# chsakell/aca-dotnet-workshop

Measured on AMD Instinct MI355X. Metric: tasks_e2e_per_sec, higher is better.
Workload: dtype n/a (JSON over HTTP)

## Files before the change

aca_dotnet_workshop_amd/native/build.py:

```python
from __future__ import annotations

import contextlib
import fcntl
import os
import subprocess
import sys
import sysconfig
from pathlib import Path

HERE = Path(__file__).resolve().parent
SRC = HERE / "src"


def ext_path(name: str) -> Path:
    suffix = sysconfig.get_config_var("EXT_SUFFIX") or ".so"
    return HERE / f"{name}{suffix}"


@contextlib.contextmanager
def build_lock(name: str):
    lock_dir = HERE / "bin"
    lock_dir.mkdir(exist_ok=True)
    with open(lock_dir / f".{name}.lock", "w") as fh:
        fcntl.flock(fh, fcntl.LOCK_EX)
        try:
            yield
        finally:
            fcntl.flock(fh, fcntl.LOCK_UN)


def _stale(target: Path, sources: list[Path]) -> bool:
    if not target.exists():
        return True
    t = target.stat().st_mtime
    return any(s.exists() and s.stat().st_mtime > t for s in sources)


def _newest(sources: list[Path]) -> float:
    return max((s.stat().st_mtime for s in sources if s.exists()), default=0.0)


def _install(tmp: Path, target: Path, stamp: float) -> None:
    os.replace(tmp, target)
    if stamp > 0:
        os.utime(target, (stamp, stamp))


def _run_compiler(cmd: list[str], tmp: Path) -> None:
    try:
        subprocess.run(cmd, check=True)
    except BaseException:
        tmp.unlink(missing_ok=True)
        raise


EXE_ONLY_HEADERS: set[str] = set()


def build_native(force: bool = False, verbose: bool = False) -> Path:
    target = ext_path("_ttnative")
    sources = sorted(h for h in SRC.glob("*.hpp") if h.name not in EXE_ONLY_HEADERS) + [SRC / "module.cpp"]
    if not force and not _stale(target, sources):
        return target
    with build_lock("ttnative"):
        if force or _stale(target, sources):
            _compile_native(target, verbose, _newest(sources))
    return target


def _compile_native(target: Path, verbose: bool, stamp: float = 0.0) -> None:
    import pybind11
    cxx = os.environ.get("CXX", "g++")
    tmp = target.with_suffix(f".tmp{os.getpid()}.so")
    cmd = [cxx, "-O3", "-std=c++17", "-shared", "-fPIC", "-Wall", "-Wno-unused-function", "-Wno-attributes",
           f"-I{pybind11.get_include()}", f"-I{sysconfig.get_paths()['include']}", str(SRC / "module.cpp"),
           "-o", str(tmp), "-lpthread", "-lssl", "-lcrypto"]
    if verbose:
        print(" ".join(cmd), file=sys.stderr)
    _run_compiler(cmd, tmp)
    _install(tmp, target, stamp)


DATAPLANE = HERE / "bin" / "ttsidecar-dataplane"


def build_dataplane(force: bool = False, verbose: bool = False) -> Path:
    sources = [SRC / "dataplane.cpp", SRC / "evhttp.hpp", SRC / "h2.hpp", SRC / "pb.hpp", SRC / "tls.hpp", SRC / "json.hpp", SRC / "httpparse.hpp",
               SRC / "textutil.hpp", SRC / "pcsample.hpp"]
    return _build_exe(DATAPLANE, SRC / "dataplane.cpp", sources, force, verbose)


def _build_exe(target: Path, main: Path, sources: list[Path], force: bool, verbose: bool,
               threads: bool = False) -> Path:
    if not force and not _stale(target, sources):
        return target
    with build_lock(target.name):
        if not force and not _stale(target, sources):
            return target
        cxx = os.environ.get("CXX", "g++")
        tmp = target.with_name(f".{target.name}.tmp{os.getpid()}")
        cmd = [cxx, "-O2", "-std=c++17", "-Wall", "-Wno-unused-function", "-rdynamic", str(main), "-o", str(tmp),
               "-lssl", "-lcrypto"] + (["-pthread"] if threads else [])
        if verbose:
            print(" ".join(cmd), file=sys.stderr)
        stamp = _newest(sources)
        _run_compiler(cmd, tmp)
        _install(tmp, target, stamp)
    return target


INGRESS = HERE / "bin" / "ttingress"


def build_ingress(force: bool = False, verbose: bool = False) -> Path:
    sources = [SRC / "ingress.cpp", SRC / "evhttp.hpp", SRC / "tls.hpp", SRC / "json.hpp", SRC / "httpparse.hpp",
               SRC / "textutil.hpp", SRC / "pcsample.hpp"]
    return _build_exe(INGRESS, SRC / "ingress.cpp", sources, force, verbose, threads=True)


LOADGEN = HERE / "bin" / "ttloadgen"


def build_loadgen(force: bool = False, verbose: bool = False) -> Path:
    sources = [SRC / "loadgen.cpp", SRC / "evhttp.hpp", SRC / "tls.hpp", SRC / "json.hpp", SRC / "httpparse.hpp"]
    return _build_exe(LOADGEN, SRC / "loadgen.cpp", sources, force, verbose, threads=True)


if __name__ == "__main__":
    print(build_native(force="--force" in sys.argv, verbose=True))
    print(build_dataplane(force="--force" in sys.argv, verbose=True))
    print(build_loadgen(force="--force" in sys.argv, verbose=True))
    print(build_ingress(force="--force" in sys.argv, verbose=True))
```

aca_dotnet_workshop_amd/native/src/dataplane.cpp:

```cpp
#include <signal.h>
#include <sys/prctl.h>
#include <sys/signalfd.h>
#include <sys/stat.h>
#include <dirent.h>

#include <cstdio>
#include <ctime>
#include <fstream>
#include <map>
#include <random>
#include <sstream>

#include "evhttp.hpp"
#include "daprpb.hpp"
#include "h2.hpp"
#include "json.hpp"
#include "pb.hpp"
#include "pcsample.hpp"
#include "textutil.hpp"

using namespace tt;
using ev::ClientResult;
using ev::Endpoint;
using ev::HeaderList;
using ev::Message;
using ev::Reply;
using namespace tt::text;

namespace {

std::mt19937_64& rng() {
  static std::mt19937_64 r{std::random_device{}() ^ ((uint64_t)getpid() << 32)};
  return r;
}

std::string hex_u64(uint64_t v, int digits = 16) {
  static const char* d = "0123456789abcdef";
  std::string s((size_t)digits, '0');
  for (int i = digits - 1; i >= 0; --i, v >>= 4) s[(size_t)i] = d[v & 15];
  return s;
}

std::string uuid4() {
  uint64_t a = rng()(), b = rng()();
  a = (a & 0xFFFFFFFFFFFF0FFFull) | 0x0000000000004000ull;
  b = (b & 0x3FFFFFFFFFFFFFFFull) | 0x8000000000000000ull;
  std::string h = hex_u64(a) + hex_u64(b);
  return h.substr(0, 8) + "-" + h.substr(8, 4) + "-" + h.substr(12, 4) + "-" + h.substr(16, 4) + "-" + h.substr(20);
}

std::string utc_now_iso() {
  timespec ts;
  clock_gettime(CLOCK_REALTIME, &ts);
  tm t;
  gmtime_r(&ts.tv_sec, &t);
  char buf[64];
  std::snprintf(buf, sizeof buf, "%04d-%02d-%02dT%02d:%02d:%02d.%06ldZ", t.tm_year + 1900, t.tm_mon + 1, t.tm_mday,
                t.tm_hour, t.tm_min, t.tm_sec, ts.tv_nsec / 1000);
  return buf;
}

double wall_now() {
  timespec ts;
  clock_gettime(CLOCK_REALTIME, &ts);
  return (double)ts.tv_sec + ts.tv_nsec / 1e9;
}

std::string error_json(std::string_view code, std::string_view msg) {
  return "{\"errorCode\":" + json_str(code) + ",\"message\":" + json_str(msg) + "}";
}


bool valid_json(std::string_view s) { return tt::valid(s); }

bool top_level_string(std::string_view json, std::string_view key, std::string& out) {
  const char* p = tt::ws_end(json.data(), json.data() + json.size());
  const char* e = json.data() + json.size();
  if (p >= e || *p != '{') return false;
  p = tt::ws_end(p + 1, e);
  while (p < e && *p == '"') {
    const char* k = p + 1;
    const char* q = tt::skip_value(p, e);
    std::string_view name(k, (size_t)(q - 1 - k));
    p = tt::ws_end(q, e);
    if (p >= e || *p != ':') return false;
    p = tt::ws_end(p + 1, e);
    const char* v = p;
    p = tt::skip_value(p, e);
    if (name.find('\\') != std::string_view::npos) {
      try {
        Value obj = parse(json);
        const Value* x = obj.get(key);
        if (!x || x->t != Value::String) return false;
        out = x->s;
        return true;
      } catch (const std::exception&) {
        return false;
      }
    }
    if (name == key) {
      if (*v != '"') return false;
      std::string_view lit(v + 1, (size_t)(p - 1 - (v + 1)));
      if (lit.find('\\') != std::string_view::npos) {
        try {
          out = parse(std::string_view(v, (size_t)(p - v))).s;
        } catch (const std::exception&) {
          return false;
        }
      } else {
        out.assign(lit);
      }
      return true;
    }
    p = tt::ws_end(p, e);
    if (p < e && *p == ',') p = tt::ws_end(p + 1, e);
  }
  return false;
}

std::string errno_text(int e) {
  switch (e) {
    case ETIMEDOUT: return "timeout";
    case ECONNREFUSED: return "connection refused";
    case ENOENT: return "no such socket";
    case ECONNRESET: return "connection closed";
    case EPROTO: return "malformed upstream response";
    default: return std::string(strerror(e));
  }
}

const std::string* opt_str(const Value& cfg, const char* k) {
  auto* v = cfg.get(k);
  return v && v->t == Value::String ? &v->s : nullptr;
}

void hex16(uint64_t v, char* out) {
  static const char* d = "0123456789abcdef";
  for (int i = 15; i >= 0; --i, v >>= 4) out[i] = d[v & 15];
}

struct SpanCtx {
  char trace_id[32], span_id[16], parent_id[16];
  bool has_parent = false, sampled = false;
  double start_wall = 0, t0 = 0;
  std::string_view tid() const { return {trace_id, 32}; }
  std::string_view sid() const { return {span_id, 16}; }
  std::string_view pid() const { return {parent_id, 16}; }
  std::string traceparent() const {
    std::string s;
    s.reserve(55);
    s.append("00-", 3).append(trace_id, 32).append(1, '-').append(span_id, 16).append(sampled ? "-01" : "-00", 3);
    return s;
  }
};

bool parse_traceparent(const std::string* v, SpanCtx& out) {
  if (!v) return false;
  std::string_view s(*v);
  if (s.size() < 55 || s[2] != '-' || s[35] != '-' || s[52] != '-') return false;
  bool tz = true, pz = true;
  for (size_t i = 3; i < 35; ++i) {
    if (hexv(s[i]) < 0) return false;
    tz = tz && s[i] == '0';
  }
  for (size_t i = 36; i < 52; ++i) {
    if (hexv(s[i]) < 0) return false;
    pz = pz && s[i] == '0';
  }
  if (tz || pz) return false;
  int f1 = hexv(s[53]), f2 = hexv(s[54]);
  if (f1 < 0 || f2 < 0) return false;
  std::memcpy(out.trace_id, s.data() + 3, 32);
  std::memcpy(out.parent_id, s.data() + 36, 16);
  out.has_parent = true;
  out.sampled = ((f1 * 16 + f2) & 1) != 0;
  return true;
}

class Tracer {
 public:
  void init(const Value& cfg) {
    if (auto* d = opt_str(cfg, "dir")) dir_ = *d;
    if (auto* r = cfg.get("sampleRate"); r && r->t == Value::Number) rate_ = r->n;
    if (auto* r = opt_str(cfg, "role")) role_ = *r;
    if (auto* i = opt_str(cfg, "instance")) instance_ = *i;
    if (auto* f = opt_str(cfg, "file")) path_ = *f;
    if (auto* fe = cfg.get("flushEach"); fe && fe->t == Value::Bool) flush_each_ = fe->b;
    if (!dir_.empty() && path_.empty()) {
      mkdir(dir_.c_str(), 0755);
      std::string safe = role_;
      for (auto& c : safe)
        if (c == '/') c = '_';
      stem_ = dir_ + "/spans-" + safe + "-" + std::to_string(getpid()) + "-";
      path_ = stem_;
    }
  }
  SpanCtx start(const std::string* traceparent) {
    SpanCtx s;
    if (!parse_traceparent(traceparent, s)) {
      hex16(rng()(), s.trace_id);
      hex16(rng()(), s.trace_id + 16);
      s.has_parent = false;
      s.sampled = rate_ >= 1.0 || std::uniform_real_distribution<double>(0, 1)(rng()) < rate_;
    }
    hex16(rng()(), s.span_id);
    if (s.sampled) s.start_wall = wall_now();
    s.t0 = ev::now_s();
    return s;
  }
  void end(const SpanCtx& s, const std::string& name, int status, const std::vector<std::pair<std::string, std::string>>& attrs) {
    if (!s.sampled || path_.empty()) return;
    char dur[32];
    std::snprintf(dur, sizeof dur, "%.3f", (ev::now_s() - s.t0) * 1000.0);
    char ts[32];
    std::snprintf(ts, sizeof ts, "%.6f", s.start_wall);
    std::string l = "{\"type\":\"span\",\"role\":" + json_str(role_) + ",\"instance\":" + json_str(instance_) +
                    ",\"name\":" + json_str(name) + ",\"kind\":\"server\",\"traceId\":\"" + std::string(s.tid()) +
                    "\",\"spanId\":\"" + std::string(s.sid()) + "\",\"parentId\":" +
                    (s.has_parent ? "\"" + std::string(s.pid()) + "\"" : std::string("null")) + ",\"ts\":" + ts +
                    ",\"durationMs\":" + dur + ",\"status\":\"" + (status >= 500 ? "error" : "ok") +
                    "\",\"attributes\":{\"http.status\":" + std::to_string(status);
    for (auto& a : attrs) l += "," + json_str(a.first) + ":" + json_str(a.second);
    l += "},\"plane\":\"native\"}\n";
    buf_ += l;
    if (flush_each_ || buf_.size() > 64 * 1024) flush();
  }
  void flush() {
    if (buf_.empty() || path_.empty()) return;
    std::string path = path_;
    if (!stem_.empty()) {
      time_t t = time(nullptr);
      struct tm g;
      gmtime_r(&t, &g);
      char day[16];
      std::strftime(day, sizeof day, "%Y%m%d", &g);
      path = stem_ + day + ".jsonl";
    }
    if (FILE* f = std::fopen(path.c_str(), "a")) {
      std::fwrite(buf_.data(), 1, buf_.size(), f);
      std::fclose(f);
    }
    buf_.clear();
  }

 private:
  std::string dir_, path_, stem_, role_ = "sidecar", instance_;
  double rate_ = 1.0;
  bool flush_each_ = false;
  std::string buf_;
};

class Resolver {
 public:
  std::string dir;
  std::vector<std::string> candidates(const std::string& app) {
    auto& e = cache_[app];
    double t = ev::now_s();
    if (t - e.at > 0.5) {
      e.eps.clear();
      e.at = t;
      std::string d = dir + "/" + app;
      if (DIR* dh = opendir(d.c_str())) {
        std::vector<std::string> files;
        while (dirent* de = readdir(dh)) {
          std::string n = de->d_name;
          if (n.size() > 5 && n[0] != '.' && n.compare(n.size() - 5, 5, ".json") == 0) files.push_back(n);
        }
        closedir(dh);
        std::sort(files.begin(), files.end());
        for (auto& f : files) {
          std::ifstream in(d + "/" + f);
          std::stringstream ss;
          ss << in.rdbuf();
          try {
            Value rec = parse(ss.str());
            auto* ep = rec.get("endpoint");
            auto* pid = rec.get("pid");
            if (!ep || ep->t != Value::String) continue;
            if (pid && pid->t == Value::Number && kill((pid_t)pid->n, 0) != 0 && errno == ESRCH) continue;
            e.eps.push_back(ep->s);
          } catch (const std::exception&) {
          }
        }
      }
    }
    if (e.eps.size() <= 1) return e.eps;
    size_t n = e.rr++ % e.eps.size();
    std::vector<std::string> out(e.eps.begin() + (long)n, e.eps.end());
    out.insert(out.end(), e.eps.begin(), e.eps.begin() + (long)n);
    return out;
  }
  void invalidate(const std::string& app) { cache_.erase(app); }

 private:
  struct Entry {
    double at = -1;
    std::vector<std::string> eps;
    size_t rr = 0;
  };
  std::map<std::string, Entry> cache_;
};

inline uint64_t fnv1a64(std::string_view s) {
  uint64_t h = 14695981039346656037ull;
  for (unsigned char c : s) {
    h ^= c;
    h *= 1099511628211ull;
  }
  return h;
}
struct Store {
  Endpoint backing;
  std::vector<Endpoint> shards;
  std::string coll_path;
  std::string prefix;
  HeaderList auth;
  size_t shard_of(std::string_view full_key) const { return shards.empty() ? 0 : fnv1a64(full_key) % shards.size(); }
  const Endpoint& ep(size_t shard) const { return shards.empty() ? backing : shards[shard]; }
};
struct Bus {
  Endpoint backing;
  std::vector<Endpoint> shards;
  std::string ns;
  HeaderList auth;
  const Endpoint& ep(std::string_view partition_key) const {
    return shards.empty() ? backing : shards[fnv1a64(partition_key) % shards.size()];
  }
};
inline std::vector<Endpoint> shard_list(const Value& s) {
  std::vector<Endpoint> out;
  if (auto* sh = s.get("shards"); sh && sh->t == Value::Array)
    for (auto& u : sh->items)
      if (u.t == Value::String) out.push_back(Endpoint::parse(u.s));
  if (out.size() == 1) out.clear();
  return out;
}

bool is_invoke_hop(const std::string& k) {
  return ev::is_hop_header(k) || k == "dapr-api-token" || k == "dapr-app-id" || k == "traceparent";
}

class DataPlane {
 public:
  DataPlane(ev::Loop& loop, const Value& cfg) : loop_(loop), client_(loop) {
    app_id_ = *opt_str(cfg, "appId");
    if (auto* a = opt_str(cfg, "app")) {
      app_ = Endpoint::parse(*a);
      has_app_ = true;
    }
    if (auto* t = opt_str(cfg, "appToken")) app_token_ = *t;
    if (auto* t = opt_str(cfg, "apiToken")) api_token_ = *t;
    if (auto* t = opt_str(cfg, "meshToken")) mesh_token_ = *t;
    if (auto* t = cfg.get("mtls"); t && t->t == Value::Object) {
      ev::TlsConfig tc;
      tc.cert = *opt_str(*t, "cert");
      tc.key = *opt_str(*t, "key");
      tc.ca = *opt_str(*t, "ca");
      mesh_server_tls = std::make_shared<ev::TlsContext>(tc, true);
      client_.set_tls(std::make_shared<ev::TlsContext>(tc, false));
    }
    if (auto* r = opt_str(cfg, "registryDir")) resolver_.dir = *r;
    fallback_ = Endpoint::parse(*opt_str(cfg, "fallback"));
    if (auto* v = cfg.get("invokeNative"); v && v->t == Value::Bool) invoke_native_ = v->b;
    if (auto* v = cfg.get("appTimeout"); v && v->t == Value::Number) app_timeout_ = v->n;
    if (auto* v = cfg.get("apiLogging"); v && v->t == Value::Bool) api_logging_ = v->b;
    if (auto* tr = cfg.get("trace")) tracer_.init(*tr);
    if (auto* st = cfg.get("stores"); st && st->t == Value::Object)
      for (size_t i = 0; i < st->keys.size(); ++i) {
        const Value& s = st->items[i];
        Store x;
        x.backing = Endpoint::parse(*opt_str(s, "backing"));
        x.coll_path = "/cosmos/" + quote_all(*opt_str(s, "account")) + "/" + quote_all(*opt_str(s, "db")) + "/" +
                      quote_all(*opt_str(s, "coll"));
        x.prefix = *opt_str(s, "prefix");
        x.auth = auth_headers(s);
        x.shards = shard_list(s);
        stores_[st->keys[i]] = std::move(x);
      }
    if (auto* ps = cfg.get("pubsubs"); ps && ps->t == Value::Object)
      for (size_t i = 0; i < ps->keys.size(); ++i) {
        const Value& s = ps->items[i];
        Bus b;
        b.backing = Endpoint::parse(*opt_str(s, "backing"));
        b.ns = *opt_str(s, "ns");
        b.auth = auth_headers(s);
        b.shards = shard_list(s);
        buses_[ps->keys[i]] = std::move(b);
      }
  }

  ev::Handler api_handler() {
    return [this](Message&& m, Reply r) { on_api(std::move(m), std::move(r)); };
  }
  ev::Handler internal_handler() {
    return [this](Message&& m, Reply r) { on_internal(std::move(m), std::move(r)); };
  }
  ev::Handler control_handler() {
    return [this](Message&& m, Reply r) { on_control(std::move(m), std::move(r)); };
  }
  void flush() {
    flush_api_log();
    tracer_.flush();
  }
  size_t inflight() const { return inflight_; }
  void tick(double now) {
    flush_api_log();
    for (auto& c : consumers_) c->tick(now);
  }
  void begin_stop() {
    for (auto& c : consumers_) c->stop();
  }
  bool drained() const {
    if (inflight_) return false;
    for (auto& c : consumers_)
      if (!c->drained()) return false;
    return true;
  }

 private:
  ev::Loop& loop_;
  ev::Client client_;
  Tracer tracer_;
  Resolver resolver_;
  std::string app_id_, app_token_, api_token_, mesh_token_;

 public:
  std::shared_ptr<ev::TlsContext> mesh_server_tls;
  const std::string& app_id() const { return app_id_; }

 private:
  Endpoint app_, fallback_;
  bool has_app_ = false, invoke_native_ = true, api_logging_ = false;
  double app_timeout_ = 300;
  std::map<std::string, Store> stores_;
  std::map<std::string, Bus> buses_;
  std::map<std::string, uint64_t> counters_;
  std::map<std::pair<std::string, int>, uint64_t> op_counts_;
  size_t inflight_ = 0;

  static HeaderList auth_headers(const Value& s) {
    HeaderList h;
    if (auto* i = opt_str(s, "identity"); i && !i->empty()) h.emplace_back("x-tt-identity", *i);
    if (auto* k = opt_str(s, "key"); k && !k->empty()) h.emplace_back("x-tt-key", *k);
    return h;
  }

  void api_log(const std::string& name, int status, const SpanCtx& span) {
    char buf[96];
    std::snprintf(buf, sizeof buf, " status=%d duration_ms=%.3f app_id=", status, (ev::now_s() - span.t0) * 1e3);
    auto sp = name.find(' ');
    std::string& msg = api_log_msg_;
    msg.assign("HTTP API Called method=");
    msg.append(name, 0, sp);
    msg += " path=";
    if (sp != std::string::npos) msg.append(name, sp + 1, std::string::npos);
    msg += buf;
    msg += app_id_;
    if (api_log_role_.empty()) api_log_role_ = json_str(app_id_ + ".sidecar");
    char ts[32];
    std::snprintf(ts, sizeof ts, "%.6f", wall_now());
    std::string& b = api_log_buf_;
    b += "{\"ts\":";
    b += ts;
    b += ",\"level\":\"INFO\",\"role\":";
    b += api_log_role_;
    b += ",\"category\":\"sidecar.http-info\",\"message\":";
    escape_to(b, msg);
    b += ",\"traceId\":\"";
    b += span.tid();
    b += "\",\"spanId\":\"";
    b += span.sid();
    b += "\",\"plane\":\"native\"}\n";
    if (b.size() >= 32768) flush_api_log();
  }
  std::string api_log_msg_, api_log_role_;
  void flush_api_log() {
    if (api_log_buf_.empty()) return;
    std::fwrite(api_log_buf_.data(), 1, api_log_buf_.size(), stderr);
    api_log_buf_.clear();
  }
  std::string api_log_buf_;

  void count(const std::string& op, int status) {
    op_counts_[{op, status}]++;
  }

  struct Done {
    DataPlane* dp;
    Reply rep;
    SpanCtx span;
    std::string name, op;
    std::vector<std::pair<std::string, std::string>> attrs;
    void send(int status, const HeaderList& h, std::string_view body) {
      rep.send(status, h, body);
      if (dp->api_logging_) dp->api_log(name, status, span);
      dp->tracer_.end(span, name, status, attrs);
      dp->count(op, status);
      dp->inflight_--;
    }
    void json(int status, std::string_view body) { send(status, {{"content-type", "application/json"}}, body); }
    void error(int status, std::string_view code, std::string_view msg) { json(status, error_json(code, msg)); }
  };
  std::shared_ptr<Done> begin(const Message& m, Reply&& r, std::string op, std::string_view path) {
    inflight_++;
    auto d = std::make_shared<Done>();
    d->dp = this;
    d->rep = std::move(r);
    d->span = tracer_.start(m.header("traceparent"));
    d->name = m.method + " " + std::string(path.substr(0, 80));
    d->op = std::move(op);
    return d;
  }

  static void split_target(const std::string& target, std::string& path, std::string& qs) {
    auto q = target.find('?');
    path = target.substr(0, q);
    qs = q == std::string::npos ? "" : target.substr(q + 1);
  }

  struct SubSpec {
    std::string name, pubsub, topic, route, entity, ns, dlt;
    Endpoint backing;
    HeaderList auth;
    int lock_ms = 60000, prefetch = 64, max_conc = 32, retry_delay_ms = 0;
    bool raw = false;
  };
  class Consumer {
   public:
    Consumer(DataPlane& dp, SubSpec s) : s_(std::move(s)), dp_(dp) { next_renew_ = ev::now_s() + renew_period(); }
    SubSpec s_;
    uint64_t delivered = 0, succeeded = 0, retried = 0, dropped = 0, errors = 0;

    void start() { pump(); }
    void stop() {
      stopping_ = true;
      while (!queued_.empty()) {
        abandon_.emplace_back(queued_.front().token, 0);
        locked_.erase(queued_.front().token);
        queued_.pop_front();
      }
      schedule_flush();
    }
    bool drained() const { return running_ == 0 && !settling_ && pending_empty(); }
    void tick(double now) {
      if (!stopping_ && !receiving_ && retry_at_ > 0 && now >= retry_at_) {
        retry_at_ = 0;
        pump();
      }
      if (now >= next_renew_) {
        next_renew_ = now + renew_period();
        if (!locked_.empty() && !stopping_) renew();
      }
    }
    std::string stats_json() const {
      return "{\"delivered\":" + std::to_string(delivered) + ",\"succeeded\":" + std::to_string(succeeded) +
             ",\"retried\":" + std::to_string(retried) + ",\"dropped\":" + std::to_string(dropped) +
             ",\"errors\":" + std::to_string(errors) + ",\"plane\":\"native\"}";
    }

   private:
    struct Msg {
      std::string token, id, body, ctype;
      long long delivery_count = 0;
    };
    DataPlane& dp_;
    std::deque<Msg> queued_;
    std::map<std::string, int> locked_;
    int running_ = 0;
    bool receiving_ = false, stopping_ = false, settling_ = false, flush_scheduled_ = false;
    double retry_at_ = 0, backoff_ = 0.1, next_renew_ = 0;
    std::vector<std::string> complete_;
    std::vector<std::pair<std::string, int>> abandon_;
    std::vector<std::pair<std::string, std::string>> deadletter_;

    double renew_period() const { return std::max(s_.lock_ms / 3000.0, 0.05); }
    bool pending_empty() const { return complete_.empty() && abandon_.empty() && deadletter_.empty(); }
    std::string sb_path(const std::string& tail) const { return "/servicebus/" + quote_all(s_.ns) + tail; }

    void pump() {
      if (stopping_ || receiving_) return;
      int room = s_.prefetch - (int)locked_.size();
      if (room <= 0) return;
      receiving_ = true;
      std::string q = "?entity=" + quote_all(s_.entity) + "&max=" + std::to_string(std::min(room, 256)) +
                      "&lockMs=" + std::to_string(s_.lock_ms) + "&waitMs=2000";
      dp_.client_.request(s_.backing, "POST", sb_path("/receive" + q), s_.auth, {}, 32.0,
                          [this](ClientResult&& res) { on_received(std::move(res)); });
    }

    void on_received(ClientResult&& res) {
      receiving_ = false;
      if (res.err || res.resp.status != 200) {
        if (!stopping_) {
          std::fprintf(stderr, "dataplane: %s: receive failed (%s); retrying in %.1fs\n", s_.name.c_str(),
                       res.err ? errno_text(res.err).c_str() : ("HTTP " + std::to_string(res.resp.status)).c_str(),
                       backoff_);
          retry_at_ = ev::now_s() + backoff_;
          backoff_ = std::min(backoff_ * 2, 5.0);
        }
        return;
      }
      backoff_ = 0.1;
      try {
        Value arr = parse(res.resp.body);
        for (auto& v : arr.items) {
          Msg m;
          if (auto* t = v.get("lockToken")) m.token = t->s;
          if (auto* t = v.get("id")) m.id = t->s;
          if (auto* t = v.get("contentType"); t && t->t == Value::String) m.ctype = t->s;
          if (auto* t = v.get("deliveryCount"); t && t->t == Value::Number) m.delivery_count = (long long)t->n;
          if (auto* b = v.get("bodyB64"); b && b->t == Value::String) m.body = unbase64(b->s);
          else if (auto* b = v.get("body"); b && b->t == Value::String) m.body = b->s;
          if (stopping_) {
            abandon_.emplace_back(m.token, 0);
            continue;
          }
          locked_[m.token] = 1;
          queued_.push_back(std::move(m));
        }
      } catch (const std::exception& e) {
        std::fprintf(stderr, "dataplane: %s: bad receive payload: %s\n", s_.name.c_str(), e.what());
      }
      start_deliveries();
      if (stopping_) schedule_flush();
      pump();
    }

    void start_deliveries() {
      while (!queued_.empty() && running_ < s_.max_conc) {
        Msg m = std::move(queued_.front());
        queued_.pop_front();
        running_++;
        delivered++;
        deliver(std::move(m));
      }
    }

    void deliver(Msg&& m) {
      std::string body = std::move(m.body);
      std::string ctype = m.ctype.empty() ? "application/json" : m.ctype;
      SpanCtx span;
      bool is_ce = false;
      std::string parent_tp;
      if (ctype.rfind("application/cloudevents", 0) == 0 && valid_json(body)) {
        is_ce = true;
        top_level_string(body, "traceparent", parent_tp);
      }
      if (!is_ce && !s_.raw) {
        std::string base = lower(ctype.substr(0, ctype.find(';')));
        std::string ce = "{\"specversion\":\"1.0\",\"id\":" + json_str(m.id.empty() ? uuid4() : m.id) +
                         ",\"source\":\"unknown\",\"type\":\"com.dapr.event.sent\",\"datacontenttype\":" +
                         json_str(base.empty() ? "application/json" : base) + ",\"topic\":" + json_str(s_.topic) +
                         ",\"pubsubname\":" + json_str(s_.pubsub) + ",\"time\":\"" + utc_now_iso() + "\"";
        if (base.find("json") != std::string::npos && !body.empty() && valid_json(body)) ce += ",\"data\":" + compact(body);
        else if (base.find("json") != std::string::npos && body.empty()) ce += ",\"data\":null";
        else if (base.rfind("text/", 0) == 0 || base.find("json") != std::string::npos || body.empty())
          ce += ",\"data\":" + json_str(body);
        else ce += ",\"data_base64\":\"" + base64(body) + "\"";
        ce += "}";
        body = std::move(ce);
        is_ce = true;
      }
      span = dp_.tracer_.start(parent_tp.empty() ? nullptr : &parent_tp);
      HeaderList h;
      h.emplace_back("content-type", is_ce && !s_.raw ? "application/cloudevents+json" : ctype);
      h.emplace_back("traceparent", span.traceparent());
      h.emplace_back("pubsubname", s_.pubsub);
      h.emplace_back("topic", s_.topic);
      std::string token = m.token;
      long long dc = m.delivery_count;
      std::string raw_body = body;
      std::string out_ct = h[0].second;
      dp_.call_app("POST", "/" + s_.route, std::move(h), std::move(body),
                   [this, token, span, dc, raw_body = std::move(raw_body), out_ct](ClientResult&& res) mutable {
                     int outcome = 1;
                     int status = res.err ? 0 : res.resp.status;
                     if (res.err) {
                       errors++;
                     } else if (status >= 200 && status < 300) {
                       outcome = 0;
                       auto* ct = res.resp.header("content-type");
                       if (!res.resp.body.empty() && ct && ct->find("json") != std::string::npos) {
                         try {
                           Value v = parse(res.resp.body);
                           if (auto* st = v.get("status"); st && st->t == Value::String) {
                             std::string u = st->s;
                             for (auto& c : u) c = (char)std::toupper((unsigned char)c);
                             outcome = u == "RETRY" ? 1 : u == "DROP" ? 2 : 0;
                           }
                         } catch (const std::exception&) {
                         }
                       }
                     } else if (status == 404) {
                       outcome = 2;
                     }
                     dp_.tracer_.end(span, "pubsub/" + s_.topic, outcome == 0 ? status : 500,
                                     {{"messaging.delivery_count", std::to_string(dc)}});
                     dp_.count("deliver", outcome == 0 ? 200 : outcome == 1 ? 503 : 404);
                     finish(token, outcome, raw_body, out_ct);
                   });
    }

    void finish(const std::string& token, int outcome, const std::string& body, const std::string& ctype) {
      running_--;
      if (outcome == 0) {
        succeeded++;
        complete_.push_back(token);
        locked_.erase(token);
      } else if (outcome == 1) {
        retried++;
        abandon_.emplace_back(token, s_.retry_delay_ms);
        locked_.erase(token);
      } else {
        dropped++;
        if (!s_.dlt.empty()) {
          forward_dead_letter(token, body, ctype);
        } else {
          deadletter_.emplace_back(token, "dropped by application");
          locked_.erase(token);
        }
      }
      schedule_flush();
      start_deliveries();
      pump();
    }

    void forward_dead_letter(const std::string& token, const std::string& body, const std::string& ctype) {
      HeaderList h = s_.auth;
      h.emplace_back("content-type", ctype);
      running_++;
      dp_.client_.request(s_.backing, "POST", sb_path("/topics/" + quote_all(s_.dlt) + "/messages"), h, body, 60,
                          [this, token](ClientResult&& res) {
                            running_--;
                            if (!res.err && res.resp.status < 300) complete_.push_back(token);
                            else deadletter_.emplace_back(token, "dropped by application");
                            locked_.erase(token);
                            schedule_flush();
                          });
    }

    void schedule_flush() {
      if (flush_scheduled_) return;
      flush_scheduled_ = true;
      dp_.loop_.defer([this] {
        flush_scheduled_ = false;
        flush();
      });
    }

    void flush() {
      if (settling_ || pending_empty()) return;
      std::string b = "{\"entity\":" + json_str(s_.entity) + ",\"complete\":[";
      for (size_t i = 0; i < complete_.size(); ++i) b += (i ? "," : "") + json_str(complete_[i]);
      b += "],\"abandon\":[";
      for (size_t i = 0; i < abandon_.size(); ++i)
        b += (i ? ",{\"token\":" : "{\"token\":") + json_str(abandon_[i].first) + ",\"delayMs\":" +
             std::to_string(abandon_[i].second) + "}";
      b += "],\"deadletter\":[";
      for (size_t i = 0; i < deadletter_.size(); ++i)
        b += (i ? ",{\"token\":" : "{\"token\":") + json_str(deadletter_[i].first) + ",\"reason\":" +
             json_str(deadletter_[i].second) + "}";
      b += "]}";
      complete_.clear();
      abandon_.clear();
      deadletter_.clear();
      settling_ = true;
      HeaderList h = s_.auth;
      h.emplace_back("content-type", "application/json");
      dp_.client_.request(s_.backing, "POST", sb_path("/settle"), h, b, 60, [this](ClientResult&& res) {
        settling_ = false;
        if (res.err || res.resp.status >= 300)
          std::fprintf(stderr, "dataplane: %s: settle failed\n", s_.name.c_str());
        if (!pending_empty()) flush();
      });
    }

    void renew() {
      std::string b = "{\"entity\":" + json_str(s_.entity) + ",\"renew\":[";
      size_t i = 0;
      for (auto& kv : locked_)
        b += (i++ ? ",{\"token\":" : "{\"token\":") + json_str(kv.first) + ",\"lockMs\":" + std::to_string(s_.lock_ms) + "}";
      b += "]}";
      HeaderList h = s_.auth;
      h.emplace_back("content-type", "application/json");
      dp_.client_.request(s_.backing, "POST", sb_path("/settle"), h, b, 60, [](ClientResult&&) {});
    }
  };
  std::vector<std::unique_ptr<Consumer>> consumers_;

  void on_control(Message&& m, Reply r) {
    std::string path, qs;
    split_target(m.target, path, qs);
    if (path == "/subscribe" && m.method == "POST") {
      try {
        Value v = parse(m.body);
        SubSpec s;
        auto str = [&](const char* k) { auto* x = opt_str(v, k); return x ? *x : std::string(); };
        auto num = [&](const char* k, int d) { auto* x = v.get(k); return x && x->t == Value::Number ? (int)x->n : d; };
        s.name = str("name");
        s.pubsub = str("pubsub");
        s.topic = str("topic");
        s.route = str("route");
        s.entity = str("entity");
        s.ns = str("ns");
        s.dlt = str("deadLetterTopic");
        s.backing = Endpoint::parse(str("backing"));
        s.auth = auth_headers(v);
        s.lock_ms = num("lockMs", 60000);
        s.prefetch = std::max(1, num("prefetch", 64));
        s.max_conc = std::max(1, num("maxConcurrent", 32));
        s.retry_delay_ms = num("retryDelayMs", 0);
        if (auto* x = v.get("raw"); x && x->t == Value::Bool) s.raw = x->b;
        consumers_.push_back(std::make_unique<Consumer>(*this, std::move(s)));
        consumers_.back()->start();
        r.empty(204);
      } catch (const std::exception& e) {
        r.json(400, error_json("ERR_MALFORMED_REQUEST", e.what()));
      }
      return;
    }
    if (path == "/stats" && m.method == "GET") {
      std::string b = "{\"consumers\":{";
      for (size_t i = 0; i < consumers_.size(); ++i)
        b += (i ? "," : "") + json_str(consumers_[i]->s_.name) + ":" + consumers_[i]->stats_json();
      b += "},\"inflight\":" + std::to_string(inflight_) + "}";
      r.json(200, b);
      return;
    }
    r.json(404, error_json("ERR_NOT_FOUND", "no such control route"));
  }

  void on_api(Message&& m, Reply r) {
    std::string path, qs;
    split_target(m.target, path, qs);
    if (!api_token_.empty() && path.rfind("/v1.0/healthz", 0) != 0) {
      auto* t = m.header("dapr-api-token");
      if (!t || *t != api_token_) {
        r.json(401, error_json("ERR_API_TOKEN", "invalid api token"));
        return;
      }
    }
    std::vector<std::string_view> seg;
    {
      std::string_view p(path);
      size_t i = 1;
      while (i <= p.size()) {
        size_t j = p.find('/', i);
        if (j == std::string_view::npos) j = p.size();
        seg.push_back(p.substr(i, j - i));
        i = j + 1;
      }
    }
    if (seg.size() == 4 && (lower(seg[0]) == "v1.0-alpha1" || lower(seg[0]) == "v1.0-beta1") &&
        lower(seg[1]) == "state" && lower(seg[3]) == "query" && (m.method == "POST" || m.method == "PUT")) {
      auto it = stores_.find(unquote(seg[2]));
      if (it != stores_.end()) {
        if (it->second.shards.empty()) state_query(std::move(m), std::move(r), it->second, path);
        else state_query_sharded(std::move(m), std::move(r), it->second, path);
        return;
      }
    }
    if (seg.size() >= 2 && lower(seg[0]) == "v1.0") {
      std::string s1 = lower(seg[1]);
      if (s1 == "invoke" && seg.size() >= 4 && lower(seg[3]) == "method" && invoke_native_) {
        size_t off = (size_t)(seg[3].data() + seg[3].size() + 1 - path.data());
        std::string method_path = off <= path.size() ? path.substr(off) : "";
        std::string target = unquote(seg[2]);
        target = target.substr(0, target.find('.'));
        invoke(std::move(m), std::move(r), target, method_path, qs, path);
        return;
      }
      if (s1 == "state" && seg.size() >= 3) {
        std::string store = unquote(seg[2]);
        auto it = stores_.find(store);
        if (it != stores_.end()) {
          if (seg.size() == 3 && (m.method == "POST" || m.method == "PUT")) {
            state_save(std::move(m), std::move(r), store, it->second, path);
            return;
          }
          if (seg.size() == 4 && m.method == "GET") {
            state_get(std::move(m), std::move(r), it->second, unquote(seg[3]), path);
            return;
          }
          if (seg.size() == 4 && (m.method == "POST" || m.method == "PUT") && lower(seg[3]) == "bulk") {
            state_bulk_get(std::move(m), std::move(r), it->second, path);
            return;
          }
          if (seg.size() == 4 && m.method == "DELETE") {
            state_delete(std::move(m), std::move(r), it->second, unquote(seg[3]), path);
            return;
          }
        }
      }
      if (s1 == "publish" && seg.size() >= 4 && (m.method == "POST" || m.method == "PUT")) {
        std::string name = unquote(seg[2]);
        size_t off = (size_t)(seg[3].data() - path.data());
        std::string topic = unquote(std::string_view(path).substr(off));
        auto it = buses_.find(name);
        if (it != buses_.end() && !topic.empty() && publish(m, r, name, topic, it->second, qs, path)) return;
      }
    }
    if (path == "/metrics" && m.method == "GET") {
      metrics(std::move(m), std::move(r));
      return;
    }
    forward_to_control_plane(std::move(m), std::move(r));
  }

  void forward_to_control_plane(Message&& m, Reply r, std::function<void(std::string&)> amend = nullptr) {
    HeaderList h;
    for (auto& kv : m.headers)
      if (!ev::is_hop_header(kv.first)) h.push_back(kv);
    client_.request(fallback_, m.method, m.target, h, m.body, 0,
                    [r, amend = std::move(amend)](ClientResult&& res) {
                      if (res.err) {
                        r.json(503, error_json("ERR_SIDECAR_CONTROL_PLANE", "control plane unreachable: " + errno_text(res.err)));
                        return;
                      }
                      if (amend) amend(res.resp.body);
                      r.send(res.resp.status, res.resp.headers, res.resp.body);
                    });
  }

  void metrics(Message&& m, Reply r) {
    std::string extra = "# HELP sidecar_native_requests_total requests served by the native data plane\n"
                        "# TYPE sidecar_native_requests_total counter\n";
    std::map<std::string, uint64_t> all = counters_;
    for (auto& kv : op_counts_)
      all["app=\"" + app_id_ + "\",op=\"" + kv.first.first + "\",status=\"" + std::to_string(kv.first.second) + "\""] +=
          kv.second;
    for (auto& kv : all) extra += "sidecar_native_requests_total{" + kv.first + "} " + std::to_string(kv.second) + "\n";
    extra += "# HELP sidecar_mtls_handshake_rejected_total mesh TLS handshakes this sidecar refused\n"
             "# TYPE sidecar_mtls_handshake_rejected_total counter\n"
             "sidecar_mtls_handshake_rejected_total{app=\"" + app_id_ + "\"} " +
             std::to_string(ev::tls_server_handshake_rejects.load(std::memory_order_relaxed)) + "\n";
    extra += "# HELP sidecar_pipelined_requests_total requests sent over pipelined local connections "
             "(store and broker calls to the backing's Unix socket)\n"
             "# TYPE sidecar_pipelined_requests_total counter\n"
             "sidecar_pipelined_requests_total{app=\"" + app_id_ + "\"} " + std::to_string(client_.pipelined()) + "\n";
    extra += "# HELP sidecar_client_connects_total outbound connections opened (the pools had none idle); "
             "tls: with a TLS handshake\n"
             "# TYPE sidecar_client_connects_total counter\n"
             "sidecar_client_connects_total{app=\"" + app_id_ + "\",transport=\"any\"} " +
             std::to_string(client_.connects()) + "\n" +
             "sidecar_client_connects_total{app=\"" + app_id_ + "\",transport=\"tls\"} " +
             std::to_string(client_.tls_connects()) + "\n";
    extra += "# HELP sidecar_partitioned_query_rows_total cross-partition state queries: sort-key entries the "
             "shards sent (phase keys) and documents fetched for the merged pages (phase documents)\n"
             "# TYPE sidecar_partitioned_query_rows_total counter\n"
             "sidecar_partitioned_query_rows_total{app=\"" + app_id_ + "\",phase=\"keys\"} " +
             std::to_string(keys_moved_) + "\nsidecar_partitioned_query_rows_total{app=\"" + app_id_ +
             "\",phase=\"documents\"} " + std::to_string(rows_fetched_) + "\n";
    forward_to_control_plane(std::move(m), std::move(r), [extra](std::string& body) { body += extra; });
  }

  HeaderList fwd_headers(Message& m, const std::string& traceparent, bool drop_mesh) {
    HeaderList h;
    h.reserve(m.headers.size() + 3);
    for (auto& kv : m.headers) {
      if (is_invoke_hop(kv.first)) continue;
      if (drop_mesh && kv.first == "tt-mesh-token") continue;
      h.push_back(std::move(kv));
    }
    h.emplace_back("traceparent", traceparent);
    return h;
  }

  static void relay(Done& d, ClientResult& res) {
    d.send(res.resp.status, res.resp.headers, res.resp.body);
  }

  void invoke(Message&& m, Reply&& r, const std::string& target, const std::string& method_path,
              const std::string& qs, const std::string& path) {
    auto d = begin(m, std::move(r), "invoke", path);
    d->attrs.emplace_back("invoke.target", target);
    HeaderList h = fwd_headers(m, d->span.traceparent(), false);
    h.emplace_back("dapr-caller-app-id", app_id_);
    std::string tgt = "/" + method_path + (qs.empty() ? "" : "?" + qs);
    if (target == app_id_) {
      call_app(m.method, tgt, std::move(h), std::move(m.body), [d, target](ClientResult&& res) {
        if (res.err) {
          d->error(500, "ERR_DIRECT_INVOKE", "failed to invoke, id: " + target + ", err: " + errno_text(res.err));
          return;
        }
        relay(*d, res);
      });
      return;
    }
    auto cands = resolver_.candidates(target);
    if (cands.empty()) {
      resolver_.invalidate(target);
      cands = resolver_.candidates(target);
    }
    if (cands.empty()) {
      d->error(500, "ERR_DIRECT_INVOKE", "failed to resolve address for app-id '" + target + "'");
      return;
    }
    if (!mesh_token_.empty()) h.emplace_back("tt-mesh-token", mesh_token_);
    if (cands.size() > 3) cands.resize(3);
    call_peer(std::make_shared<PeerCall>(PeerCall{d, target, m.method, tgt, std::move(h), std::move(m.body),
                                                  std::move(cands), 0}));
  }

  struct PeerCall {
    std::shared_ptr<Done> d;
    std::string target, method, path;
    HeaderList headers;
    std::string body;
    std::vector<std::string> cands;
    size_t i;
  };
  void call_peer(std::shared_ptr<PeerCall> pc) {
    Endpoint ep = Endpoint::parse(pc->cands[pc->i]);
    client_.request(ep, pc->method, pc->path, pc->headers, pc->body, app_timeout_, [this, pc](ClientResult&& res) {
      if (res.err == ECONNREFUSED || res.err == ENOENT || res.err == ECONNRESET) {
        resolver_.invalidate(pc->target);
        if (++pc->i < pc->cands.size()) {
          call_peer(pc);
          return;
        }
      }
      if (res.err) {
        pc->d->error(500, "ERR_DIRECT_INVOKE", "failed to invoke, id: " + pc->target + ", err: " + errno_text(res.err));
        return;
      }
      relay(*pc->d, res);
    });
  }

  void call_app(const std::string& method, const std::string& target, HeaderList&& h, std::string&& body,
                ev::ClientCallback cb) {
    if (!has_app_) {
      loop_.defer([cb = std::move(cb)]() mutable {
        ClientResult r;
        r.err = ECONNREFUSED;
        cb(std::move(r));
      });
      return;
    }
    if (!app_token_.empty()) h.emplace_back("dapr-api-token", app_token_);
    client_.request(app_, method, target, h, body, app_timeout_, std::move(cb));
  }

  void on_internal(Message&& m, Reply r) {
    if (mesh_server_tls) {
      auto* c = m.header("dapr-caller-app-id");
      if (!m.tls || (c && !(m.tls_peer && names_include(*m.tls_peer, *c)))) {
        r.json(403, error_json("ERR_MESH_AUTH", "caller identity not proven by its mTLS certificate"));
        return;
      }
    }
    if (!mesh_token_.empty()) {
      auto* t = m.header("tt-mesh-token");
      if (!t || *t != mesh_token_) {
        r.json(403, error_json("ERR_MESH_AUTH", "sidecar-to-sidecar call not authenticated"));
        return;
      }
    }
    std::string path, qs;
    split_target(m.target, path, qs);
    auto d = begin(m, std::move(r), "internal", path);
    if (auto* c = m.header("dapr-caller-app-id")) d->attrs.emplace_back("caller", *c);
    HeaderList h = fwd_headers(m, d->span.traceparent(), true);
    std::string app_id = app_id_;
    call_app(m.method, m.target, std::move(h), std::move(m.body), [d, app_id](ClientResult&& res) {
      if (res.err) {
        d->error(502, "ERR_APP_CHANNEL", "app " + app_id + " unreachable: " + errno_text(res.err));
        return;
      }
      relay(*d, res);
    });
  }

  static bool names_include(const std::string& csv, const std::string& name) {
    size_t p = 0;
    while (p <= csv.size()) {
      size_t e = csv.find(',', p);
      if (e == std::string::npos) e = csv.size();
      if (csv.compare(p, e - p, name) == 0) return true;
      p = e + 1;
    }
    return false;
  }

  struct Item {
    std::string key, value, etag;
    bool first_write = false;
    long long ttl_ms = 0;
  };

  static bool parse_items(const std::string& body, std::vector<Item>& items, std::string& err) {
    if (!valid_json(body)) {
      err = "request body is not valid JSON";
      return false;
    }
    const char* p = ws_end(body.data(), body.data() + body.size());
    const char* e = body.data() + body.size();
    if (p >= e || *p != '[') {
      err = "request body must be an array of state items";
      return false;
    }
    ++p;
    while (true) {
      p = ws_end(p, e);
      if (p < e && *p == ']') break;
      if (p >= e || *p != '{') {
        err = "state item without key";
        return false;
      }
      Item it;
      bool have_value = false;
      ++p;
      while (true) {
        p = ws_end(p, e);
        if (*p == '}') {
          ++p;
          break;
        }
        const char* ks = p;
        p = skip_value(p, e);
        std::string_view ktok(ks, (size_t)(p - ks));
        std::string k = ktok.size() >= 2 && ktok.find('\\') == std::string_view::npos
                            ? std::string(ktok.substr(1, ktok.size() - 2))
                            : parse(ktok).s;
        p = ws_end(p, e) + 1;
        p = ws_end(p, e);
        const char* vs = p;
        p = skip_value(p, e);
        std::string_view raw(vs, (size_t)(p - vs));
        if (k == "key") {
          if (raw.size() >= 2 && raw.front() == '"' && raw.find('\\') == std::string_view::npos) {
            it.key.assign(raw.data() + 1, raw.size() - 2);
          } else {
            Value v = parse(raw);
            if (v.t == Value::String) it.key = v.s;
          }
        } else if (k == "value") {
          it.value = compact(raw);
          have_value = true;
        } else if (k == "etag") {
          Value v = parse(raw);
          if (v.t == Value::String) it.etag = v.s;
          else if (auto* x = v.get("value"); x && x->t == Value::String) it.etag = x->s;
        } else if (k == "options") {
          Value v = parse(raw);
          if (auto* c = v.get("concurrency"); c && c->t == Value::String) it.first_write = c->s == "first-write";
        } else if (k == "metadata") {
          Value v = parse(raw);
          if (auto* t = v.get("ttlInSeconds")) {
            double s = t->t == Value::Number ? t->n : t->t == Value::String ? std::atof(t->s.c_str()) : 0.0;
            it.ttl_ms = (long long)(s * 1000);
          }
        }
        p = ws_end(p, e);
        if (*p == ',') ++p;
      }
      if (it.key.empty()) {
        err = "state item without key";
        return false;
      }
      if (!have_value) it.value = "null";
      items.push_back(std::move(it));
      p = ws_end(p, e);
      if (*p == ',') ++p;
    }
    return true;
  }

  struct StoreCall {
    Endpoint ep;
    std::string method, target, body;
    HeaderList headers;
    ev::ClientCallback cb;
    int attempt = 0;
    double waited = 0.0;
    bool pipeline = true;
  };

  void store_request(const Endpoint& ep, std::string method, std::string target, HeaderList h, std::string body,
                     ev::ClientCallback cb, bool pipeline = true) {
    auto c = std::make_shared<StoreCall>();
    c->pipeline = pipeline;
    c->ep = ep;
    c->method = std::move(method);
    c->target = std::move(target);
    c->headers = std::move(h);
    c->body = std::move(body);
    c->cb = std::move(cb);
    store_send(std::move(c));
  }

  void store_send(std::shared_ptr<StoreCall> c) {
    StoreCall& k = *c;
    auto on_done = [this, c](ClientResult&& res) {
      if (!res.err && res.resp.status == 429 && c->attempt < 9) {
        const std::string* ra = res.resp.header("x-ms-retry-after-ms");
        double delay = ra ? std::strtod(ra->c_str(), nullptr) / 1000.0 : 0.1;
        delay = std::min(std::max(delay, 0.001), 5.0);
        if (c->waited + delay <= 30.0) {
          count("state.throttled_retry", 429);
          c->attempt++;
          c->waited += delay;
          auto& hs = c->headers;
          hs.erase(std::remove_if(hs.begin(), hs.end(), [](const auto& h) { return h.first == "x-tt-ru-ticket"; }),
                   hs.end());
          if (const std::string* t = res.resp.header("x-tt-ru-ticket")) hs.emplace_back("x-tt-ru-ticket", *t);
          loop_.call_later(delay, [this, c] { store_send(c); });
          return;
        }
      }
      c->cb(std::move(res));
    };
    if (k.pipeline) client_.request_pipelined(k.ep, k.method, k.target, k.headers, k.body, 60, std::move(on_done));
    else client_.request(k.ep, k.method, k.target, k.headers, k.body, 60, std::move(on_done));
  }

  void state_save(Message&& m, Reply&& r, const std::string& name, const Store& s, const std::string& path) {
    auto d = begin(m, std::move(r), "state.save", path);
    std::vector<Item> items;
    std::string err;
    if (!parse_items(m.body, items, err)) {
      d->error(400, "ERR_MALFORMED_REQUEST", err);
      return;
    }
    auto done = [d, name](ClientResult&& res) {
      if (!res.err && (res.resp.status == 409 || res.resp.status == 412)) {
        d->error(409, "ERR_STATE_SAVE", "failed saving state in state store " + name + ": state save: HTTP " +
                                            std::to_string(res.resp.status) + " " + res.resp.body.substr(0, 200));
        return;
      }
      if (res.err || res.resp.status >= 300) {
        d->error(500, "ERR_STATE_SAVE", "failed saving state in state store " + name + ": " +
                                            (res.err ? errno_text(res.err) : "HTTP " + std::to_string(res.resp.status)));
        return;
      }
      d->send(204, {}, {});
    };
    if (items.empty()) {
      d->send(204, {}, {});
      return;
    }
    HeaderList h = s.auth;
    h.emplace_back("content-type", "application/json");
    if (s.shards.empty()) {
      save_on(s, 0, h, items, std::move(done));
      return;
    }
    std::map<size_t, std::vector<Item>> by_shard;
    for (auto& it : items) by_shard[s.shard_of(full_key(s, it.key))].push_back(std::move(it));
    if (by_shard.size() == 1) {
      save_on(s, by_shard.begin()->first, h, by_shard.begin()->second, std::move(done));
      return;
    }
    struct Join {
      size_t left;
      ClientResult worst;
      bool have = false;
      ev::ClientCallback done;
    };
    auto j = std::make_shared<Join>();
    j->left = by_shard.size();
    j->done = std::move(done);
    for (auto& kv : by_shard)
      save_on(s, kv.first, h, kv.second, [j](ClientResult&& res) {
        auto rank = [](const ClientResult& r) {
          return r.err ? 3 : (r.resp.status == 409 || r.resp.status == 412) ? 2 : r.resp.status >= 300 ? 1 : 0;
        };
        if (!j->have || rank(res) > rank(j->worst)) {
          j->worst = std::move(res);
          j->have = true;
        }
        if (--j->left == 0) j->done(std::move(j->worst));
      });
  }

  void save_on(const Store& s, size_t shard, HeaderList h, std::vector<Item>& items, ev::ClientCallback done) {
    if (items.size() == 1) {
      Item& it = items[0];
      if (!it.etag.empty()) h.emplace_back("if-match", it.etag);
      if (it.first_write) h.emplace_back("x-tt-first-write", "1");
      if (it.ttl_ms) h.emplace_back("x-tt-ttl-ms", std::to_string(it.ttl_ms));
      store_request(s.ep(shard), "PUT", s.coll_path + "/docs/" + quote_all(full_key(s, it.key)), std::move(h), it.value,
                    std::move(done));
      return;
    }
    std::string body = "[";
    for (size_t i = 0; i < items.size(); ++i) {
      auto& it = items[i];
      if (i) body += ',';
      const bool as_text = it.value.empty() || it.value[0] == '"';
      body += "{\"key\":" + json_str(full_key(s, it.key)) + ",\"value\":" + (as_text ? json_str(it.value) : it.value) +
              ",\"etag\":" + (it.etag.empty() ? std::string("null") : json_str(it.etag)) +
              ",\"firstWrite\":" + (it.first_write ? "true" : "false") + ",\"ttlMs\":" + std::to_string(it.ttl_ms) + "}";
    }
    body += "]";
    store_request(s.ep(shard), "POST", s.coll_path + "/bulkset", std::move(h), std::move(body), std::move(done), false);
  }

  static std::string full_key(const Store& s, const std::string& key) {
    if (s.prefix.empty() && key.find("||") != std::string::npos) return key;
    return s.prefix + key;
  }

  void state_get(Message&& m, Reply&& r, const Store& s, const std::string& key, const std::string& path) {
    auto d = begin(m, std::move(r), "state.get", path);
    const std::string fk = full_key(s, key);
    store_request(s.ep(s.shard_of(fk)), "GET", s.coll_path + "/docs/" + quote_all(fk), s.auth, {},
                    [d](ClientResult&& res) {
                      if (res.err || (res.resp.status != 200 && res.resp.status != 404)) {
                        d->error(500, "ERR_STATE_GET", "state get: " + (res.err ? errno_text(res.err)
                                                                               : "HTTP " + std::to_string(res.resp.status)));
                        return;
                      }
                      if (res.resp.status == 404) {
                        d->send(204, {}, {});
                        return;
                      }
                      const std::string* et = res.resp.header("etag");
                      d->send(200, {{"etag", et ? *et : ""}, {"content-type", "application/json"}}, res.resp.body);
                    });
  }

  struct BulkGet {
    std::vector<std::string> keys, full;
    std::vector<std::string> bodies;
    std::unordered_map<std::string, std::pair<std::string_view, std::string>> found;
    size_t left = 0;
    bool failed = false;
    std::string error;
  };

  static bool scan_bulkget(const std::string& body, BulkGet& bg) {
    const char* p = tt::ws_end(body.data(), body.data() + body.size());
    const char* e = body.data() + body.size();
    if (p >= e || *p != '[') return false;
    ++p;
    while (true) {
      p = tt::ws_end(p, e);
      if (p < e && *p == ']') return true;
      if (p >= e || *p != '{') return false;
      ++p;
      std::string key, etag;
      std::string_view data;
      while (true) {
        p = tt::ws_end(p, e);
        if (p < e && *p == '}') {
          ++p;
          break;
        }
        const char* ks = p;
        p = tt::skip_value(p, e);
        std::string_view name(ks, (size_t)(p - ks));
        p = tt::ws_end(p, e);
        if (p >= e || *p != ':') return false;
        const char* vs = tt::ws_end(p + 1, e);
        p = tt::skip_value(vs, e);
        std::string_view val(vs, (size_t)(p - vs));
        try {
          if (name == "\"key\"") key = tt::parse(val).s;
          else if (name == "\"etag\"") etag = tt::parse(val).s;
          else if (name == "\"data\"") data = val;
        } catch (const std::exception&) {
          return false;
        }
        p = tt::ws_end(p, e);
        if (p < e && *p == ',') ++p;
      }
      if (!data.empty()) bg.found[key] = {data, std::move(etag)};
      p = tt::ws_end(p, e);
      if (p < e && *p == ',') ++p;
    }
  }

  void fetch_docs(const Store& s, const std::shared_ptr<BulkGet>& bg, std::function<void()> done) {
    std::map<size_t, std::vector<size_t>> by_shard;
    for (size_t i = 0; i < bg->full.size(); ++i) by_shard[s.shards.empty() ? 0 : s.shard_of(bg->full[i])].push_back(i);
    if (by_shard.empty()) {
      done();
      return;
    }
    bg->left = by_shard.size();
    bg->bodies.resize(by_shard.size());
    auto fin = std::make_shared<std::function<void()>>(std::move(done));
    HeaderList h = s.auth;
    h.emplace_back("content-type", "application/json");
    size_t slot = 0;
    for (auto& kv : by_shard) {
      std::string body = "{\"keys\":[";
      for (size_t j = 0; j < kv.second.size(); ++j) body += (j ? "," : "") + json_str(bg->full[kv.second[j]]);
      body += "]}";
      store_request(s.ep(kv.first), "POST", s.coll_path + "/bulkget", h, std::move(body),
                    [bg, slot, fin](ClientResult&& res) {
                      if (res.err || res.resp.status != 200) {
                        bg->failed = true;
                        if (bg->error.empty())
                          bg->error = res.err ? errno_text(res.err) : "HTTP " + std::to_string(res.resp.status);
                      } else {
                        bg->bodies[slot] = std::move(res.resp.body);
                        if (!scan_bulkget(bg->bodies[slot], *bg)) bg->failed = true, bg->error = "unreadable bulkget";
                      }
                      if (--bg->left == 0) (*fin)();
                    },
                    bg->keys.size() <= 16);
      ++slot;
    }
  }

  void state_bulk_get(Message&& m, Reply&& r, const Store& s, const std::string& path) {
    auto d = begin(m, std::move(r), "state.bulkget", path);
    auto bg = std::make_shared<BulkGet>();
    try {
      Value v = parse(m.body.empty() ? std::string("{}") : m.body);
      const Value* ks = v.get("keys");
      if (ks && ks->t == Value::Array)
        for (auto& k : ks->items) {
          if (k.t != Value::String) throw std::runtime_error("keys must be strings");
          bg->keys.push_back(k.s);
          bg->full.push_back(full_key(s, k.s));
        }
    } catch (const std::exception& ex) {
      d->error(400, "ERR_MALFORMED_REQUEST", std::string("bulk get: ") + ex.what());
      return;
    }
    fetch_docs(s, bg, [d, bg] {
      if (bg->failed) {
        d->error(500, "ERR_STATE_BULK_GET", "bulk get: " + bg->error);
        return;
      }
      std::string out = "[";
      for (size_t i = 0; i < bg->keys.size(); ++i) {
        out += i ? ",{\"key\":" : "{\"key\":";
        out += json_str(bg->keys[i]);
        auto it = bg->found.find(bg->full[i]);
        if (it != bg->found.end()) {
          out += ",\"data\":";
          out.append(it->second.first);
          out += ",\"etag\":" + json_str(it->second.second);
        }
        out += '}';
      }
      out += ']';
      d->send(200, {{"content-type", "application/json"}}, out);
    });
  }

  struct ShardPage {
    std::vector<std::string> keys;
    std::vector<std::vector<Value>> sort;
    bool more = false;
// ... 130 lines not shown
            x->error = std::string("unreadable shard page: ") + ex.what();
          }
        }
        if (--x->left == 0) merge_and_fetch(d, x, s);
      }, false);
    }
  }

  void merge_and_fetch(const std::shared_ptr<Done>& d, const std::shared_ptr<XQuery>& x, const Store& s) {
    if (x->failed) {
      d->error(x->fail_status, "ERR_STATE_QUERY", "state query: " + x->error);
      return;
    }
    const size_t n = x->pages.size();
    std::vector<size_t> pos(n, 0), used(n, 0);
    static const Value kNull;
    auto less = [&](size_t a, size_t b) {
      const auto& va = x->pages[a].sort[pos[a]];
      const auto& vb = x->pages[b].sort[pos[b]];
      for (size_t k = 0; k < x->sort.size(); ++k) {
        int c = compare(k < va.size() ? va[k] : kNull, k < vb.size() ? vb[k] : kNull);
        if (c) return x->sort[k].second ? c > 0 : c < 0;
      }
      return a < b;
    };
    auto bg = std::make_shared<BulkGet>();
    std::vector<size_t> order_shard;
    auto starved = [&] {
      for (size_t i = 0; i < n; ++i)
        if (x->pages[i].more && pos[i] >= x->pages[i].keys.size()) return true;
      return false;
    };
    while ((!x->limit || bg->full.size() < x->limit) && !starved()) {
      size_t best = n;
      for (size_t i = 0; i < n; ++i) {
        if (pos[i] >= x->pages[i].keys.size()) continue;
        if (x->sort.empty()) {
          best = i;
          break;
        }
        if (best == n || less(i, best)) best = i;
      }
      if (best == n) break;
      bg->keys.push_back(x->pages[best].keys[pos[best]]);
      bg->full.push_back(full_key(s, bg->keys.back()));
      ++pos[best];
      ++used[best];
    }
    std::string tok;
    if (x->limit) {
      bool any = false;
      std::string arr = "[";
      for (size_t i = 0; i < n; ++i) {
        if (i) arr += ',';
        const ShardPage& pg = x->pages[i];
        if (!pg.present || (!pg.more && used[i] == pg.keys.size())) {
          arr += "null";
        } else {
          bool all = used[i] == pg.keys.size();
          arr += std::to_string(all && pg.next >= 0 ? pg.next : x->offsets[i] + (long long)used[i]);
          any = true;
        }
      }
      arr += ']';
      if (any) tok = "p1." + b64url(arr);
    }
    rows_fetched_ += bg->full.size();
    fetch_docs(s, bg, [d, bg, tok] {
      if (bg->failed) {
        d->error(500, "ERR_STATE_QUERY", "state query: " + bg->error);
        return;
      }
      std::string out = "{\"results\":[";
      bool first = true;
      for (size_t i = 0; i < bg->keys.size(); ++i) {
        auto it = bg->found.find(bg->full[i]);
        if (it == bg->found.end()) continue;
        out += first ? "{\"key\":" : ",{\"key\":";
        first = false;
        out += json_str(bg->keys[i]);
        out += ",\"data\":";
        out.append(it->second.first);
        out += ",\"etag\":" + json_str(it->second.second);
        out += '}';
      }
      out += ']';
      if (!tok.empty()) out += ",\"token\":" + json_str(tok);
      out += '}';
      d->send(200, {{"content-type", "application/json"}}, out);
    });
  }
  uint64_t keys_moved_ = 0, rows_fetched_ = 0;

  void state_query(Message&& m, Reply&& r, const Store& s, const std::string& path) {
    auto d = begin(m, std::move(r), "state.query", path);
    std::string target = s.coll_path + "/query";
    if (!s.prefix.empty()) target += "?prefix=" + quote_all(s.prefix);
    HeaderList h = s.auth;
    h.emplace_back("content-type", "application/json");
    if (d->span.sampled) {
      h.emplace_back("traceparent", d->span.traceparent());
      char t[32];
      std::snprintf(t, sizeof t, "%.6f", ev::now_s());
      h.emplace_back("x-tt-sent-mono", t);
    }
    store_request(s.backing, "POST", target, h, m.body.empty() ? std::string("{}") : m.body,
                    [d](ClientResult&& res) {
                      if (!res.err && res.resp.status == 200) {
                        if (d->span.sampled) {
                          const double now = ev::now_s();
                          for (auto [attr, hdr] : {std::pair{"store_handler_end_to_sidecar_ms", "x-tt-handler-end-mono"},
                                                   std::pair{"store_front_rx_to_sidecar_ms", "x-tt-front-rx-mono"}})
                            if (const std::string* t = res.resp.header(hdr)) {
                              char b[32];
                              std::snprintf(b, sizeof b, "%.3f", (now - std::strtod(t->c_str(), nullptr)) * 1e3);
                              d->attrs.emplace_back(attr, b);
                            }
                        }
                        d->send(200, {{"content-type", "application/json"}}, res.resp.body);
                        return;
                      }
                      int status = (!res.err && res.resp.status == 400) ? 400 : 500;
                      d->error(status, "ERR_STATE_QUERY",
                               "state query: " + (res.err ? errno_text(res.err)
                                                          : "HTTP " + std::to_string(res.resp.status) + " " +
                                                                res.resp.body.substr(0, 300)));
                    },
                    false);
  }

  void state_delete(Message&& m, Reply&& r, const Store& s, const std::string& key, const std::string& path) {
    auto d = begin(m, std::move(r), "state.delete", path);
    HeaderList h = s.auth;
    if (auto* im = m.header("if-match"); im && !im->empty()) h.emplace_back("if-match", *im);
    const std::string fk = full_key(s, key);
    store_request(s.ep(s.shard_of(fk)), "DELETE", s.coll_path + "/docs/" + quote_all(fk), h, {},
                    [d](ClientResult&& res) {
                      if (!res.err && (res.resp.status == 409 || res.resp.status == 412)) {
                        d->error(409, "ERR_STATE_DELETE", "state delete: HTTP " + std::to_string(res.resp.status) +
                                                              " " + res.resp.body.substr(0, 200));
                        return;
                      }
                      if (res.err || (res.resp.status != 204 && res.resp.status != 404)) {
                        d->error(500, "ERR_STATE_DELETE", "state delete: " + (res.err ? errno_text(res.err)
                                                                                     : "HTTP " + std::to_string(res.resp.status)));
                        return;
                      }
                      d->send(204, {}, {});
                    });
  }

  bool publish(Message& m, Reply& r, const std::string& name, const std::string& topic, const Bus& b,
               const std::string& qs, const std::string& path) {
    std::map<std::string, std::string> meta;
    for (size_t i = 0; i <= qs.size() && !qs.empty();) {
      size_t j = qs.find('&', i);
      if (j == std::string::npos) j = qs.size();
      std::string_view kv(qs.data() + i, j - i);
      size_t eq = kv.find('=');
      std::string k = unquote(kv.substr(0, eq), true);
      std::string v = eq == std::string_view::npos ? "" : unquote(kv.substr(eq + 1), true);
      if (k.rfind("metadata.", 0) == 0) meta[k.substr(9)] = v;
      i = j + 1;
    }
    const std::string* ct = m.header("content-type");
    std::string ctype = ct && !ct->empty() ? *ct : "application/json";
    std::string base = lower(ctype.substr(0, ctype.find(';')));
    while (!base.empty() && base.back() == ' ') base.pop_back();
    while (!base.empty() && base.front() == ' ') base.erase(0, 1);
    bool raw = lower(meta.count("rawPayload") ? meta["rawPayload"] : "") == "true";
    if (!raw && base == "application/cloudevents+json") return false;
    bool is_json = base.find("json") != std::string::npos;
    bool json_body = is_json && !m.body.empty() && valid_json(m.body);
    bool as_string = !json_body && (is_json || base.rfind("text/", 0) == 0 || m.body.empty());
    if (!raw && as_string && !valid_utf8(m.body)) return false;
    auto d = begin(m, std::move(r), "publish", path);
    d->attrs.emplace_back("topic", topic);
    std::string body, out_ct, event_id;
    if (raw) {
      body = std::move(m.body);
      out_ct = ctype;
    } else {
      std::string tp = d->span.traceparent();
      event_id = uuid4();
      body = "{\"specversion\":\"1.0\",\"id\":\"" + event_id + "\",\"source\":" + json_str(app_id_) +
             ",\"type\":\"com.dapr.event.sent\",\"datacontenttype\":" + json_str(base.empty() ? "application/json" : base) +
             ",\"topic\":" + json_str(topic) + ",\"pubsubname\":" + json_str(name) + ",\"time\":\"" + utc_now_iso() + "\"";
      if (is_json) {
        if (m.body.empty()) body += ",\"data\":null";
        else if (json_body) body += ",\"data\":" + compact(m.body);
        else body += ",\"data\":" + json_str(m.body);
      } else if (base.rfind("text/", 0) == 0 || m.body.empty()) {
        body += ",\"data\":" + json_str(m.body);
      } else {
        body += ",\"data_base64\":\"" + base64(m.body) + "\"";
      }
      body += ",\"traceparent\":\"" + tp + "\",\"traceid\":\"" + tp + "\"}";
      out_ct = "application/cloudevents+json";
    }
    HeaderList h = b.auth;
    h.emplace_back("content-type", out_ct);
    std::string props;
    for (auto& kv : meta) {
      if (kv.first == "ttlInSeconds" || kv.first == "rawPayload") continue;
      props += (props.empty() ? "{" : ",") + json_str(kv.first) + ":" + json_str(kv.second);
    }
    if (!props.empty()) h.emplace_back("x-tt-props", props + "}");
    if (meta.count("ttlInSeconds")) {
      long long ttl = (long long)(std::atof(meta["ttlInSeconds"].c_str()) * 1000);
      if (ttl) h.emplace_back("x-tt-ttl-ms", std::to_string(ttl));
    }
    const std::string pkey = meta.count("partitionKey") && !meta["partitionKey"].empty() ? meta["partitionKey"]
                             : event_id.empty()                                          ? uuid4()
                                                                                         : event_id;
    client_.request_pipelined(b.ep(pkey), "POST", "/servicebus/" + quote_all(b.ns) + "/topics/" + quote_all(topic) + "/messages", h,
                    body, 60, [d, name, topic](ClientResult&& res) {
                      if (res.err || res.resp.status >= 300) {
                        d->error(500, "ERR_PUBSUB_PUBLISH_MESSAGE",
                                 "error when publish to topic " + topic + " in pubsub " + name + ": " +
                                     (res.err ? errno_text(res.err)
                                              : "publish: HTTP " + std::to_string(res.resp.status) + " " +
                                                    res.resp.body.substr(0, 200)));
                        return;
                      }
                      d->send(204, {}, {});
                    });
    return true;
  }

 public:
  h2::GrpcHandler grpc_handler() {
    return [this](h2::GrpcCall&& c, h2::GrpcReply r) { on_grpc(std::move(c), std::move(r)); };
  }

 private:
  static int grpc_code(int http) {
    switch (http) {
      case 400: return 3;
      case 401: return 16;
      case 403: return 7;
      case 404: return 5;
      case 405: case 501: return 12;
      case 409: return 10;
      case 429: return 8;
      case 500: return 13;
      case 502: case 503: return 14;
      case 504: return 4;
      default: return http >= 400 ? 2 : 0;
    }
  }
  static void grpc_fail(const h2::GrpcReply& r, int status, std::string_view body, const std::string& what) {
    std::string msg;
    try {
      Value js = parse(body);
      if (js.t == Value::Object) {
        const Value* c = js.get("errorCode");
        const Value* m = js.get("message");
        msg = (c && c->t == Value::String ? c->s : std::string()) + ": " +
              (m && m->t == Value::String ? m->s : dump(js));
      } else {
        msg = dump(js);
      }
    } catch (const std::exception&) {
      msg = std::string(body.substr(0, 500));
    }
    r.error(grpc_code(status), what + ": " + msg, {{"dapr-http-status", std::to_string(status)}});
  }
  static std::string json_or_text(std::string_view raw) {
    if (raw.empty()) return "null";
    if (valid_json(raw)) return compact(raw);
    if (valid_utf8(raw)) return json_str(raw);
    return json_str(base64(raw));
  }
  static std::string meta_qs(const std::vector<std::pair<std::string, std::string>>& meta) {
    std::string qs;
    for (auto& kv : meta) qs += (qs.empty() ? "?" : "&") + quote_all("metadata." + kv.first) + "=" + quote_all(kv.second);
    return qs;
  }
  static std::string quote_path(std::string_view s) {
    std::string o;
    size_t i = 0;
    while (true) {
      size_t j = s.find('/', i);
      o += quote_all(s.substr(i, j == std::string_view::npos ? std::string_view::npos : j - i));
      if (j == std::string_view::npos) break;
      o += '/';
      i = j + 1;
    }
    return o;
  }
  using HttpDone = std::function<void(int, const HeaderList&, std::string_view)>;
  void grpc_http(const h2::GrpcCall& c, std::string method, std::string target, std::string body,
                 std::string ctype, HeaderList extra, HttpDone done) {
    Message m;
    m.method = std::move(method);
    m.target = std::move(target);
    for (auto& kv : c.metadata)
      if (kv.first == "dapr-api-token" || kv.first == "traceparent" || kv.first == "tracestate" ||
          kv.first.rfind("dapr-", 0) == 0)
        m.headers.push_back(kv);
    if (!ctype.empty()) m.headers.emplace_back("content-type", std::move(ctype));
    for (auto& kv : extra) m.headers.push_back(std::move(kv));
    m.headers.emplace_back("content-length", std::to_string(body.size()));
    m.body = std::move(body);
    on_api(std::move(m), Reply(std::move(done)));
  }

  struct StateItemPb {
    std::string key, value, etag;
    bool has_etag = false;
    std::vector<std::pair<std::string, std::string>> meta;
    uint64_t concurrency = 0, consistency = 0;
  };
  static bool decode_state_item(std::string_view s, StateItemPb& it) {
    pb::Reader r(s);
    uint32_t f, wt;
    std::string_view v;
    while (r.next(f, wt)) {
      if (f == 1 && wt == pb::LEN && r.bytes(v)) it.key.assign(v);
      else if (f == 2 && wt == pb::LEN && r.bytes(v)) it.value.assign(v);
      else if (f == 3 && wt == pb::LEN && r.bytes(v)) {
        it.has_etag = true;
        pb::Reader er(v);
        uint32_t ef, ewt;
        std::string_view ev;
        while (er.next(ef, ewt))
          if (ef == 1 && ewt == pb::LEN && er.bytes(ev)) it.etag.assign(ev);
          else if (!er.skip(ewt)) break;
        if (!er.ok) return false;
      } else if (f == 4 && wt == pb::LEN && r.bytes(v)) {
        std::string k, val;
        if (!pb::map_entry(v, k, val)) return false;
        it.meta.emplace_back(std::move(k), std::move(val));
      } else if (f == 5 && wt == pb::LEN && r.bytes(v)) {
        pb::Reader orr(v);
        uint32_t of, owt;
        uint64_t x;
        while (orr.next(of, owt))
          if ((of == 1 || of == 2) && owt == pb::VARINT && orr.varint(x)) (of == 1 ? it.concurrency : it.consistency) = x;
          else if (!orr.skip(owt)) break;
        if (!orr.ok) return false;
      } else if (!r.skip(wt)) {
        break;
      }
    }
    return r.ok;
  }
  static std::string state_item_json(const StateItemPb& it) {
    std::string o = "{\"key\":" + json_str(it.key) + ",\"value\":" + json_or_text(it.value);
    if (it.has_etag) o += ",\"etag\":" + json_str(it.etag);
    if (!it.meta.empty()) {
      o += ",\"metadata\":{";
      for (size_t i = 0; i < it.meta.size(); ++i)
        o += (i ? "," : "") + json_str(it.meta[i].first) + ":" + json_str(it.meta[i].second);
      o += "}";
    }
    std::string opts;
    if (it.concurrency == 1 || it.concurrency == 2)
      opts += std::string("\"concurrency\":\"") + (it.concurrency == 1 ? "first-write" : "last-write") + "\"";
    if (it.consistency == 1 || it.consistency == 2)
      opts += std::string(opts.empty() ? "" : ",") + "\"consistency\":\"" +
              (it.consistency == 1 ? "eventual" : "strong") + "\"";
    if (!opts.empty()) o += ",\"options\":{" + opts + "}";
    return o + "}";
  }

  void on_grpc(h2::GrpcCall&& c, h2::GrpcReply r) {
    static constexpr std::string_view kSvc = "/dapr.proto.runtime.v1.Dapr/";
    if (c.path.compare(0, kSvc.size(), kSvc) != 0) {
      r.error(12, "unknown service: " + c.path);
      return;
    }
    std::string rpc = c.path.substr(kSvc.size());
    counters_["app=\"" + app_id_ + "\",op=\"grpc." + rpc + "\",status=\"call\""]++;
    pb::Reader rd(c.message);
    uint32_t f, wt;
    std::string_view v;
    auto fail_decode = [&] { r.error(3, rpc + ": malformed request message"); };
    auto empty_ok = [r, rpc](int status, const HeaderList&, std::string_view body) {
      if (status >= 300) grpc_fail(r, status, body, rpc);
      else r.ok({});
    };

    if (rpc == "SaveState") {
      std::string store, items = "[";
      bool first = true;
      while (rd.next(f, wt)) {
        if (f == 1 && wt == pb::LEN && rd.bytes(v)) store.assign(v);
        else if (f == 2 && wt == pb::LEN && rd.bytes(v)) {
          StateItemPb it;
          if (!decode_state_item(v, it)) return fail_decode();
          items += (first ? "" : ",") + state_item_json(it);
          first = false;
        } else if (!rd.skip(wt)) break;
      }
      if (!rd.ok) return fail_decode();
      grpc_http(c, "POST", "/v1.0/state/" + quote_all(store), items + "]", "application/json", {}, empty_ok);
      return;
    }
    if (rpc == "GetState") {
      std::string store, key;
      std::vector<std::pair<std::string, std::string>> meta;
      while (rd.next(f, wt)) {
        if (f == 1 && wt == pb::LEN && rd.bytes(v)) store.assign(v);
        else if (f == 2 && wt == pb::LEN && rd.bytes(v)) key.assign(v);
        else if (f == 4 && wt == pb::LEN && rd.bytes(v)) {
          std::string k, val;
          if (!pb::map_entry(v, k, val)) return fail_decode();
          meta.emplace_back(std::move(k), std::move(val));
        } else if (!rd.skip(wt)) break;
      }
      if (!rd.ok) return fail_decode();
      grpc_http(c, "GET", "/v1.0/state/" + quote_all(store) + "/" + quote_all(key) + meta_qs(meta), {}, {}, {},
                [r, rpc](int status, const HeaderList& h, std::string_view body) {
                  if (status >= 300) return grpc_fail(r, status, body, rpc);
                  pb::Writer w;
                  if (status == 200) {
                    w.str(1, body);
                    for (auto& kv : h)
                      if (kv.first == "etag") w.str(2, kv.second);
                  }
                  r.ok(w.s);
                });
      return;
    }
    if (rpc == "DeleteState") {
      std::string store, key, etag;
      std::vector<std::pair<std::string, std::string>> meta;
      while (rd.next(f, wt)) {
        if (f == 1 && wt == pb::LEN && rd.bytes(v)) store.assign(v);
        else if (f == 2 && wt == pb::LEN && rd.bytes(v)) key.assign(v);
        else if (f == 3 && wt == pb::LEN && rd.bytes(v)) {
          pb::Reader er(v);
          uint32_t ef, ewt;
          std::string_view ev;
          while (er.next(ef, ewt))
            if (ef == 1 && ewt == pb::LEN && er.bytes(ev)) etag.assign(ev);
            else if (!er.skip(ewt)) break;
          if (!er.ok) return fail_decode();
        } else if (f == 5 && wt == pb::LEN && rd.bytes(v)) {
          std::string k, val;
          if (!pb::map_entry(v, k, val)) return fail_decode();
          meta.emplace_back(std::move(k), std::move(val));
        } else if (!rd.skip(wt)) break;
      }
      if (!rd.ok) return fail_decode();
      HeaderList extra;
      if (!etag.empty()) extra.emplace_back("if-match", etag);
      grpc_http(c, "DELETE", "/v1.0/state/" + quote_all(store) + "/" + quote_all(key) + meta_qs(meta), {}, {},
                std::move(extra), empty_ok);
      return;
    }
    if (rpc == "QueryStateAlpha1") {
      std::string store, query;
      std::vector<std::pair<std::string, std::string>> meta;
      while (rd.next(f, wt)) {
        if (f == 1 && wt == pb::LEN && rd.bytes(v)) store.assign(v);
        else if (f == 2 && wt == pb::LEN && rd.bytes(v)) query.assign(v);
        else if (f == 3 && wt == pb::LEN && rd.bytes(v)) {
          std::string k, val;
          if (!pb::map_entry(v, k, val)) return fail_decode();
          meta.emplace_back(std::move(k), std::move(val));
        } else if (!rd.skip(wt)) break;
      }
      if (!rd.ok) return fail_decode();
      grpc_http(c, "POST", "/v1.0-alpha1/state/" + quote_all(store) + "/query" + meta_qs(meta), std::move(query),
                "application/json", {}, [r, rpc](int status, const HeaderList&, std::string_view body) {
                  if (status >= 300) return grpc_fail(r, status, body, rpc);
                  std::string fast;
                  if (tt::daprpb::query_response_pb(body, fast)) return r.ok(fast);
                  pb::Writer w;
                  try {
                    Value js = body.empty() ? Value() : parse(body);
                    if (const Value* res = js.get("results"); res && res->t == Value::Array)
                      for (auto& it : res->items) {
                        pb::Writer e;
                        auto sv = [&](const char* k) -> std::string {
                          const Value* x = it.get(k);
                          return x && x->t == Value::String ? x->s : std::string();
                        };
                        e.str(1, sv("key"));
                        if (const Value* d = it.get("data"); d && d->t != Value::Null) e.str(2, dump(*d));
                        e.str(3, sv("etag"));
                        e.str(4, sv("error"));
                        w.len_field(1, e.s);
                      }
                    if (const Value* t = js.get("token"); t && t->t == Value::String) w.str(2, t->s);
                    if (const Value* md = js.get("metadata"); md && md->t == Value::Object)
                      for (size_t i = 0; i < md->keys.size(); ++i)
                        w.map_entry(3, md->keys[i], md->items[i].t == Value::String ? md->items[i].s : dump(md->items[i]));
                  } catch (const std::exception& ex) {
                    return r.error(13, rpc + ": malformed query response: " + ex.what());
                  }
                  r.ok(w.s);
                });
      return;
    }
    if (rpc == "GetBulkState") {
      std::string store, body = "{\"keys\":[";
      uint64_t parallelism = 0;
      bool first = true;
      std::vector<std::pair<std::string, std::string>> meta;
      while (rd.next(f, wt)) {
        if (f == 1 && wt == pb::LEN && rd.bytes(v)) store.assign(v);
        else if (f == 2 && wt == pb::LEN && rd.bytes(v)) {
          body += first ? "" : ",";
          body += json_str(v);
          first = false;
        } else if (f == 3 && wt == pb::VARINT && rd.varint(parallelism)) {
        } else if (f == 4 && wt == pb::LEN && rd.bytes(v)) {
          std::string k, val;
          if (!pb::map_entry(v, k, val)) return fail_decode();
          meta.emplace_back(std::move(k), std::move(val));
        } else if (!rd.skip(wt)) break;
      }
      if (!rd.ok) return fail_decode();
      body += "],\"parallelism\":" + std::to_string(parallelism ? parallelism : 10) + "}";
      grpc_http(c, "POST", "/v1.0/state/" + quote_all(store) + "/bulk" + meta_qs(meta), std::move(body),
                "application/json", {}, [r, rpc](int status, const HeaderList&, std::string_view res) {
                  if (status >= 300) return grpc_fail(r, status, res, rpc);
                  pb::Writer w;
                  try {
                    Value js = res.empty() ? Value() : parse(res);
                    if (js.t == Value::Array)
                      for (auto& it : js.items) {
                        pb::Writer e;
                        auto sv = [&](const char* k) -> std::string {
// ... 221 lines not shown
```

aca_dotnet_workshop_amd/native/src/evhttp.hpp:

```cpp
#pragma once

#include <arpa/inet.h>
#include <fcntl.h>
#include <netinet/in.h>
#include <netinet/tcp.h>
#include <sys/epoll.h>
#include <sys/socket.h>
#include <sys/un.h>
#include <unistd.h>

#include <cerrno>
#include <chrono>
#include <cstdio>
#include <cstdlib>
#include <sys/resource.h>
#include <cstring>
#include <deque>
#include <functional>
#include <map>
#include <memory>
#include <string>
#include <string_view>
#include <unordered_map>
#include <utility>
// ... 850 lines not shown
      ::close(fd);
      throw std::runtime_error("bind " + ep.key() + ": " + strerror(e));
    }
    socklen_t len = sizeof a;
    getsockname(fd, (sockaddr*)&a, &len);
    port = ntohs(a.sin_port);
  }
  if (::listen(fd, 1024) != 0) {
    int e = errno;
    ::close(fd);
    throw std::runtime_error(std::string("listen: ") + strerror(e));
  }
  return fd;
}

inline int listen_on(Loop& loop, const Endpoint& ep, Handler& h, bool reuseport = false,
                     std::shared_ptr<IoObj>* listener_out = nullptr, std::shared_ptr<TlsContext> tls = nullptr,
                     bool record_peer = false) {
  int port = 0;
  int fd = bind_listen(ep, reuseport, port);
  auto l = std::make_shared<Listener>(loop, fd, h, std::move(tls), record_peer);
  loop.add(l, EPOLLIN);
  if (listener_out) *listener_out = l;
  return port;
}

struct ClientResult {
  int err = 0;
  Message resp;
};
using ClientCallback = std::function<void(ClientResult&&)>;

class Client;

class ClientConn : public IoObj {
 public:
  ClientConn(Loop& loop, Client& owner, std::string key) : loop_(loop), owner_(owner), key_(std::move(key)), parser_(false) {}
  bool reused = false;
  bool connecting = false;

  void start(std::string&& wire, bool head, double deadline, ClientCallback&& cb) {
    out_ = std::move(wire);
    out_off_ = 0;
    cb_ = std::move(cb);
    deadline_ = deadline;
    got_bytes_ = false;
    busy_ = true;
    if (head) parser_.expect_no_body();
    if (!connecting) flush();
  }
  void on_event(uint32_t ev) override;
  void on_tick(double now) override {
    if (busy_ && deadline_ > 0 && now > deadline_) fail(ETIMEDOUT);
    else if (!busy_ && now - idle_since_ > 30.0) loop_.remove(this);
  }
  bool busy() const { return busy_; }
  std::string wire_copy;
  bool peer_gone() const {
    char b;
    ssize_t n = ::recv(fd, &b, 1, MSG_PEEK | MSG_DONTWAIT);
    return n == 0 || (n < 0 && errno != EAGAIN && errno != EWOULDBLOCK && errno != EINTR);
  }
  bool head_req = false;
  std::unique_ptr<TlsIo> tls_;

  ssize_t io_recv(char* buf, size_t n) { return tls_ ? tls_->recv(buf, n) : ::recv(fd, buf, n, 0); }
  ssize_t io_send(const char* p, size_t n) { return tls_ ? tls_->send(p, n) : ::send(fd, p, n, MSG_NOSIGNAL); }
  bool short_read(size_t n, size_t cap) const { return read_done(tls_.get(), n, cap); }

 private:
  friend class Client;
  Loop& loop_;
  Client& owner_;
  std::string key_;
  MsgParser parser_;
  std::string in_;
  size_t in_off_ = 0;
  std::string out_;
  size_t out_off_ = 0;
  ClientCallback cb_;
  double deadline_ = 0;
  double idle_since_ = 0;
  bool busy_ = false;
  bool got_bytes_ = false;
  bool want_out_ = false;

  void flush();
  void fail(int err);
  void finish(Message&& m, bool keep);
};

class PipeConn : public IoObj {
 public:
  PipeConn(Loop& loop, Client& owner, std::string key) : loop_(loop), owner_(owner), key_(std::move(key)), parser_(false) {}
  size_t inflight() const { return q_.size(); }
  double idle_since() const { return q_.empty() ? idle_since_ : 0.0; }
  void send(std::string&& wire, double deadline, ClientCallback&& cb) {
    if (out_off_ == out_.size()) {
      out_ = std::move(wire);
      out_off_ = 0;
    } else {
      out_ += wire;
    }
    q_.push_back(Pending{std::move(cb), deadline});
    loop_.want_flush(this);
  }
  bool peer_gone() const {
    char b;
    ssize_t n = ::recv(fd, &b, 1, MSG_PEEK | MSG_DONTWAIT);
    return n == 0 || (n < 0 && errno != EAGAIN && errno != EWOULDBLOCK && errno != EINTR);
  }
  void on_event(uint32_t ev) override;
  void on_flush() override;
  void on_tick(double now) override {
    for (auto& p : q_)
      if (p.deadline > 0 && now > p.deadline) {
        fail_all(ETIMEDOUT);
        return;
      }
    if (q_.empty() && now - idle_since_ > 30.0) fail_all(0);
  }

 private:
  struct Pending {
    ClientCallback cb;
    double deadline;
  };
  Loop& loop_;
  Client& owner_;
  std::string key_;
  MsgParser parser_;
  std::string in_, out_;
  size_t in_off_ = 0, out_off_ = 0;
  std::deque<Pending> q_;
  double idle_since_ = now_s();
  bool want_out_ = false;
  void fail_all(int err);
};

class Client {
 public:
  explicit Client(Loop& loop) : loop_(loop) {}

  void set_tls(std::shared_ptr<TlsContext> mesh) { mesh_tls_ = std::move(mesh); }

  void request(const Endpoint& ep, std::string_view method, std::string_view target, const HeaderList& headers,
               std::string_view body, double timeout_s, ClientCallback cb, bool retry_stale = true) {
    std::string w;
    w.reserve(body.size() + 512);
    w.append(method);
    w += ' ';
    w.append(target);
    w += " HTTP/1.1\r\nhost: ";
    w += ep.unix_socket ? "localhost" : ep.host + ":" + std::to_string(ep.port);
    w += "\r\n";
    for (auto& h : headers) {
      if (is_hop_header(h.first)) continue;
      w += h.first;
      w += ": ";
      w += h.second;
      w += "\r\n";
    }
    w += "content-length: ";
    w += std::to_string(body.size());
    w += "\r\n\r\n";
    w.append(body);
    dispatch(ep, std::move(w), method == "HEAD", timeout_s, std::move(cb), retry_stale);
  }

  void request_pipelined(const Endpoint& ep, std::string_view method, std::string_view target,
                         const HeaderList& headers, std::string_view body, double timeout_s, ClientCallback cb) {
    static const bool enabled = [] {
      const char* v = std::getenv("TT_PIPELINE");
      return !(v && v[0] == '0');
    }();
    if (!enabled || !ep.unix_socket || ep.tls || method == "HEAD") {
      request(ep, method, target, headers, body, timeout_s, std::move(cb), false);
      return;
    }
    std::string w;
    w.reserve(body.size() + 256 + target.size());
    w.append(method);
    w += ' ';
    w.append(target);
    w += " HTTP/1.1\r\nhost: localhost\r\n";
    for (auto& h : headers) {
      if (is_hop_header(h.first)) continue;
      w += h.first;
      w += ": ";
      w += h.second;
      w += "\r\n";
    }
    w += "content-length: ";
    w += std::to_string(body.size());
    w += "\r\n\r\n";
    w.append(body);
    double deadline = timeout_s > 0 ? now_s() + timeout_s : 0;
    auto c = pipe_for(ep);
    if (!c) {
      dispatch(ep, std::move(w), false, timeout_s, std::move(cb), false);
      return;
    }
    c->send(std::move(w), deadline, std::move(cb));
    ++pipelined_;
  }
  void pipe_flushed(const std::string& key) {
    auto it = pipes_.find(key);
    if (it != pipes_.end()) it->second.cur = (it->second.cur + 1) % kPipeConns;
  }
  void pipe_closed(PipeConn* c, const std::string& key) {
    auto it = pipes_.find(key);
    if (it == pipes_.end()) return;
    for (auto& p : it->second.conns)
      if (p.get() == c) p.reset();
  }
  uint64_t pipelined() const { return pipelined_; }
  uint64_t connects() const { return connects_; }
  uint64_t tls_connects() const { return tls_connects_; }

  void release(const std::shared_ptr<ClientConn>& c) {
    auto& v = idle_[c->key_];
    if (v.size() < 256) {
      c->idle_since_ = now_s();
      v.push_back(c);
    } else {
      loop_.remove(c.get());
    }
  }
  void forget(ClientConn* c) {
    auto it = idle_.find(c->key_);
    if (it == idle_.end()) return;
    auto& v = it->second;
    for (size_t i = 0; i < v.size(); ++i)
      if (v[i].get() == c) {
        v.erase(v.begin() + (long)i);
        break;
      }
  }
  Loop& loop() { return loop_; }

  void dispatch(const Endpoint& ep, std::string&& wire, bool head, double timeout_s, ClientCallback&& cb,
                bool allow_retry) {
    std::string key = ep.key();
    std::shared_ptr<ClientConn> c;
    auto& v = idle_[key];
    while (!v.empty()) {
      c = v.back();
      v.pop_back();
      if (!c->dead && (allow_retry || !c->peer_gone())) break;
      loop_.remove(c.get());
      c.reset();
    }
    double deadline = timeout_s > 0 ? now_s() + timeout_s : 0;
    if (c) {
      c->reused = true;
    } else {
      int err = 0;
      double tc = stall_log() ? now_s() : 0;
      c = connect(ep, key, err);
      if (tc > 0 && now_s() - tc > 0.02) stall_note("client-connect-slow", (now_s() - tc) * 1e3, err);
      if (!c && err == EAGAIN && (deadline == 0 || now_s() < deadline)) {
        auto ep_copy = ep;
        loop_.call_later(0.0005, [this, ep_copy, wire = std::move(wire), head, timeout_s, cb = std::move(cb),
                                  allow_retry, deadline]() mutable {
          double left = deadline > 0 ? deadline - now_s() : 0;
          dispatch(ep_copy, std::move(wire), head, deadline > 0 ? std::max(left, 1e-3) : timeout_s, std::move(cb),
                   allow_retry);
        });
        return;
      }
      if (!c) {
        loop_.defer([cb = std::move(cb), err]() mutable {
          ClientResult r;
          r.err = err;
          cb(std::move(r));
        });
        return;
      }
    }
    if (allow_retry && c->reused) {
      auto ep_copy = ep;
      auto wire_copy = wire;
      ClientCallback inner = [this, ep_copy, wire_copy = std::move(wire_copy), head, timeout_s,
                              cb = std::move(cb)](ClientResult&& r) mutable {
        if (r.err == ECONNRESET || r.err == EPIPE) {
          dispatch(ep_copy, std::move(wire_copy), head, timeout_s, std::move(cb), false);
          return;
        }
        cb(std::move(r));
      };
      double ts = stall_log() ? now_s() : 0;
      c->start(std::move(wire), head, deadline, std::move(inner));
      if (ts > 0 && now_s() - ts > 0.02) stall_note("client-start-slow", (now_s() - ts) * 1e3, 1);
    } else {
      double ts = stall_log() ? now_s() : 0;
      c->start(std::move(wire), head, deadline, std::move(cb));
      if (ts > 0 && now_s() - ts > 0.02) stall_note("client-start-slow", (now_s() - ts) * 1e3, 0);
    }
  }

 private:
  Loop& loop_;
  std::unordered_map<std::string, std::vector<std::shared_ptr<ClientConn>>> idle_;
  std::shared_ptr<TlsContext> mesh_tls_, insecure_tls_, system_tls_;
  static constexpr size_t kPipeConns = 4, kPipeDepth = 64;
  struct PipeGroup {
    std::shared_ptr<PipeConn> conns[kPipeConns];
    size_t cur = 0;
  };
  std::unordered_map<std::string, PipeGroup> pipes_;
  uint64_t pipelined_ = 0, connects_ = 0, tls_connects_ = 0;

  std::shared_ptr<PipeConn> pipe_for(const Endpoint& ep) {
    std::string key = ep.key();
    auto& g = pipes_[key];
    for (size_t tries = 0; tries < kPipeConns; ++tries) {
      auto& c = g.conns[g.cur];
      if (c && (c->dead || (c->idle_since() > 0 && now_s() - c->idle_since() > 1.0 && c->peer_gone()))) {
        auto gone = c;
        c.reset();
        if (!gone->dead) loop_.remove(gone.get());
      }
      if (!c) {
        int fd = ::socket(AF_UNIX, SOCK_STREAM | SOCK_NONBLOCK | SOCK_CLOEXEC, 0);
        if (fd < 0) return nullptr;
        widen_local_sndbuf(fd);
        sockaddr_un a{};
        a.sun_family = AF_UNIX;
        std::strncpy(a.sun_path, ep.path.c_str(), sizeof a.sun_path - 1);
        if (::connect(fd, (sockaddr*)&a, sizeof a) != 0) {
          ::close(fd);
          return nullptr;
        }
        c = std::make_shared<PipeConn>(loop_, *this, key);
        c->fd = fd;
        loop_.add(c, EPOLLIN);
      }
      if (c->inflight() < kPipeDepth) return c;
      g.cur = (g.cur + 1) % kPipeConns;
    }
    return nullptr;
  }

  const TlsContext* tls_for(const Endpoint& ep) {
    if (ep.tls == 1) return mesh_tls_.get();
    if (ep.tls == 2 && mesh_tls_) return mesh_tls_.get();
    if (ep.tls == 2) {
      if (!system_tls_) {
        TlsConfig c;
        c.verify_peer = false;
        system_tls_ = std::make_shared<TlsContext>(c, false);
      }
      return system_tls_.get();
    }
    if (!insecure_tls_) {
      TlsConfig c;
      c.verify_peer = false;
// ... 270 lines not shown
```

aca_dotnet_workshop_amd/native/src/json.hpp:

```cpp
#pragma once

#include <emmintrin.h>

#include <cctype>
#include <cmath>
#include <cstdio>
#include <cstdint>
#include <cstring>
#include <stdexcept>
#include <string>
#include <string_view>
#include <vector>

namespace tt {

struct Value {
  enum Type : uint8_t { Null = 0, Bool = 1, Number = 2, String = 3, Array = 4, Object = 5 };
  Type t = Null;
  bool b = false;
  double n = 0.0;
  std::string s;
  std::vector<Value> items;
  std::vector<std::string> keys;

// ... 87 lines not shown
  void num(Value& v) {
    const char* s = p_;
    if (p_ < e_ && (*p_ == '-' || *p_ == '+')) ++p_;
    const char* d0 = p_;
    while (p_ < e_ && *p_ >= '0' && *p_ <= '9') ++p_;
    const char* d1 = p_;
    while (p_ < e_ && ((*p_ >= '0' && *p_ <= '9') || *p_ == '.' || *p_ == 'e' || *p_ == 'E' || *p_ == '-' || *p_ == '+')) ++p_;
    if (p_ == s) fail("invalid JSON token");
    v.t = Value::Number;
    if (p_ == d1 && d1 > d0 && d1 - d0 <= 15) {
      int64_t x = 0;
      for (const char* q = d0; q < d1; ++q) x = x * 10 + (*q - '0');
      v.n = *s == '-' ? -(double)x : (double)x;
      return;
    }
    char buf[64];
    std::string big;
    const size_t n = (size_t)(p_ - s);
    const char* c;
    if (n < sizeof buf) {
      std::memcpy(buf, s, n);
      buf[n] = 0;
      c = buf;
    } else {
      big.assign(s, n);
      c = big.c_str();
    }
    char* end = nullptr;
    v.n = std::strtod(c, &end);
    if (end != c + n) fail("invalid number");
  }
  static void utf8(std::string& out, uint32_t cp) {
    if (cp < 0x80) out += (char)cp;
    else if (cp < 0x800) { out += (char)(0xC0 | (cp >> 6)); out += (char)(0x80 | (cp & 0x3F)); }
    else if (cp < 0x10000) { out += (char)(0xE0 | (cp >> 12)); out += (char)(0x80 | ((cp >> 6) & 0x3F)); out += (char)(0x80 | (cp & 0x3F)); }
    else { out += (char)(0xF0 | (cp >> 18)); out += (char)(0x80 | ((cp >> 12) & 0x3F)); out += (char)(0x80 | ((cp >> 6) & 0x3F)); out += (char)(0x80 | (cp & 0x3F)); }
  }
  uint32_t hex4() {
    if (e_ - p_ < 4) fail("bad \\u escape");
    uint32_t v = 0;
    for (int i = 0; i < 4; ++i) {
      char c = *p_++;
      v <<= 4;
      if (c >= '0' && c <= '9') v |= c - '0';
      else if (c >= 'a' && c <= 'f') v |= c - 'a' + 10;
      else if (c >= 'A' && c <= 'F') v |= c - 'A' + 10;
      else fail("bad hex digit");
    }
    return v;
  }
  const char* stop(const char* p) const {
    const __m128i q = _mm_set1_epi8('"'), bs = _mm_set1_epi8('\\'), ctl = _mm_set1_epi8(0x1F);
    while (e_ - p >= 16) {
      __m128i x = _mm_loadu_si128(reinterpret_cast<const __m128i*>(p));
      __m128i hit = _mm_or_si128(_mm_cmpeq_epi8(x, q), _mm_cmpeq_epi8(x, bs));
      if (strict_) hit = _mm_or_si128(hit, _mm_cmpeq_epi8(_mm_max_epu8(x, ctl), ctl));
      int m = _mm_movemask_epi8(hit);
      if (m) return p + __builtin_ctz((unsigned)m);
      p += 16;
    }
    while (p < e_ && *p != '"' && *p != '\\' && !(strict_ && (unsigned char)*p < 0x20)) ++p;
    return p;
  }
  void str(std::string& out) {
    ++p_;
    const char* run = p_;
    while (true) {
      p_ = stop(p_);
      if (p_ >= e_) fail("unterminated string");
      char c = *p_;
      if (c == '"') { out.append(run, p_); ++p_; return; }
      if (c != '\\') fail("control character in string");
      out.append(run, p_);
      ++p_;
      if (p_ >= e_) fail("bad escape");
      char x = *p_++;
      switch (x) {
        case '"': out += '"'; break;
        case '\\': out += '\\'; break;
        case '/': out += '/'; break;
        case 'b': out += '\b'; break;
        case 'f': out += '\f'; break;
        case 'n': out += '\n'; break;
        case 'r': out += '\r'; break;
        case 't': out += '\t'; break;
        case 'u': {
          uint32_t cp = hex4();
          if (cp >= 0xD800 && cp < 0xDC00 && e_ - p_ >= 6 && p_[0] == '\\' && p_[1] == 'u') {
            p_ += 2;
            uint32_t lo = hex4();
            cp = 0x10000 + ((cp - 0xD800) << 10) + (lo - 0xDC00);
          }
          utf8(out, cp);
          break;
        }
        default: fail("bad escape");
      }
      run = p_;
    }
  }
  void array(Value& v, int depth) {
    ++p_;
    v.t = Value::Array;
    ws();
    if (p_ < e_ && *p_ == ']') { ++p_; return; }
    v.items.reserve(4);
    while (true) {
      v.items.emplace_back();
      value(v.items.back(), depth + 1);
      ws();
      if (p_ >= e_) fail("unterminated array");
      if (*p_ == ',') { ++p_; continue; }
      if (*p_ == ']') { ++p_; return; }
      fail("expected , or ]");
    }
  }
  void object(Value& v, int depth) {
    ++p_;
    v.t = Value::Object;
    ws();
    if (p_ < e_ && *p_ == '}') { ++p_; return; }
    v.keys.reserve(8);
    v.items.reserve(8);
    while (true) {
      ws();
      if (p_ >= e_ || *p_ != '"') fail("expected object key");
      v.keys.emplace_back();
      str(v.keys.back());
      ws();
      if (p_ >= e_ || *p_ != ':') fail("expected :");
      ++p_;
      v.items.emplace_back();
      value(v.items.back(), depth + 1);
      ws();
      if (p_ >= e_) fail("unterminated object");
      if (*p_ == ',') { ++p_; continue; }
      if (*p_ == '}') { ++p_; return; }
      fail("expected , or }");
    }
  }
};

inline Value parse(std::string_view s) { return Parser(s).parse(); }
inline Value parse_strict(std::string_view s) { return Parser(s, true).parse(); }

class Validator {
 public:
  explicit Validator(std::string_view s) : p_(s.data()), e_(s.data() + s.size()) {}
  bool ok() {
    if (!value(0)) return false;
    ws();
    return p_ == e_;
  }

 private:
  const char* p_;
  const char* e_;
  void ws() { while (p_ < e_ && (*p_ == ' ' || *p_ == '\n' || *p_ == '\r' || *p_ == '\t')) ++p_; }
  bool value(int depth) {
    if (depth > 256) return false;
    ws();
    if (p_ >= e_) return false;
    switch (*p_) {
      case '{': return object(depth);
      case '[': return array(depth);
      case '"': return str();
      case 't': return lit("true", 4);
      case 'f': return lit("false", 5);
      case 'n': return lit("null", 4);
      default: return num();
    }
  }
  bool lit(const char* w, size_t n) {
    if ((size_t)(e_ - p_) < n || std::memcmp(p_, w, n) != 0) return false;
    p_ += n;
    return true;
  }
  bool num() {
    const char* s = p_;
    if (p_ < e_ && (*p_ == '-' || *p_ == '+')) ++p_;
    const char* d0 = p_;
    while (p_ < e_ && *p_ >= '0' && *p_ <= '9') ++p_;
    const char* d1 = p_;
    while (p_ < e_ && ((*p_ >= '0' && *p_ <= '9') || *p_ == '.' || *p_ == 'e' || *p_ == 'E' || *p_ == '-' || *p_ == '+')) ++p_;
    if (p_ == s) return false;
    if (p_ == d1 && d1 > d0) return true;
    char buf[64];
    std::string big;
    const size_t n = (size_t)(p_ - s);
    const char* c;
    if (n < sizeof buf) {
      std::memcpy(buf, s, n);
      buf[n] = 0;
      c = buf;
    } else {
      big.assign(s, n);
      c = big.c_str();
    }
    char* end = nullptr;
    std::strtod(c, &end);
    return end == c + n;
  }
  bool str() {
    ++p_;
    const __m128i q = _mm_set1_epi8('"'), bs = _mm_set1_epi8('\\');
    while (true) {
      while (e_ - p_ >= 16) {
        __m128i x = _mm_loadu_si128(reinterpret_cast<const __m128i*>(p_));
        int m = _mm_movemask_epi8(_mm_or_si128(_mm_cmpeq_epi8(x, q), _mm_cmpeq_epi8(x, bs)));
        if (m) {
          p_ += __builtin_ctz((unsigned)m);
          break;
        }
        p_ += 16;
      }
      while (p_ < e_ && *p_ != '"' && *p_ != '\\') ++p_;
      if (p_ >= e_) return false;
      if (*p_ == '"') {
        ++p_;
        return true;
      }
      ++p_;
      if (p_ >= e_) return false;
      char x = *p_++;
      switch (x) {
        case '"': case '\\': case '/': case 'b': case 'f': case 'n': case 'r': case 't': break;
        case 'u': {
          if (!hex4()) return false;
          break;
        }
        default: return false;
      }
    }
  }
  bool hex4() {
    if (e_ - p_ < 4) return false;
    uint32_t cp = 0;
    for (int i = 0; i < 4; ++i) {
      char c = *p_++;
      cp <<= 4;
      if (c >= '0' && c <= '9') cp |= c - '0';
      else if (c >= 'a' && c <= 'f') cp |= c - 'a' + 10;
      else if (c >= 'A' && c <= 'F') cp |= c - 'A' + 10;
      else return false;
    }
    if (cp >= 0xD800 && cp < 0xDC00 && e_ - p_ >= 6 && p_[0] == '\\' && p_[1] == 'u') {
      p_ += 2;
      for (int i = 0; i < 4; ++i) {
        char c = *p_++;
        if (!((c >= '0' && c <= '9') || (c >= 'a' && c <= 'f') || (c >= 'A' && c <= 'F'))) return false;
      }
    }
    return true;
  }
  bool array(int depth) {
    ++p_;
    ws();
    if (p_ < e_ && *p_ == ']') { ++p_; return true; }
    while (true) {
      if (!value(depth + 1)) return false;
      ws();
      if (p_ >= e_) return false;
      if (*p_ == ',') { ++p_; continue; }
      if (*p_ == ']') { ++p_; return true; }
      return false;
    }
  }
  bool object(int depth) {
    ++p_;
    ws();
    if (p_ < e_ && *p_ == '}') { ++p_; return true; }
    while (true) {
      ws();
      if (p_ >= e_ || *p_ != '"' || !str()) return false;
      ws();
      if (p_ >= e_ || *p_ != ':') return false;
      ++p_;
      if (!value(depth + 1)) return false;
      ws();
      if (p_ >= e_) return false;
      if (*p_ == ',') { ++p_; continue; }
      if (*p_ == '}') { ++p_; return true; }
      return false;
    }
  }
};

inline bool valid(std::string_view s) { return Validator(s).ok(); }

inline const char* ws_end(const char* p, const char* e) {
  while (p < e && (*p == ' ' || *p == '\n' || *p == '\r' || *p == '\t')) ++p;
  return p;
}

inline const char* skip_value(const char* p, const char* e) {
  p = ws_end(p, e);
  if (p >= e) return p;
  if (*p == '"') {
    ++p;
    while (p < e && *p != '"') p += (*p == '\\') ? 2 : 1;
    return p + 1;
  }
  if (*p == '{' || *p == '[') {
    int depth = 0;
    while (p < e) {
      char c = *p;
      if (c == '"') {
        p = skip_value(p, e);
        continue;
      }
      if (c == '{' || c == '[') ++depth;
      if (c == '}' || c == ']') {
        if (--depth == 0) return p + 1;
      }
      ++p;
    }
    return p;
  }
  while (p < e && *p != ',' && *p != '}' && *p != ']' && *p != ' ' && *p != '\n' && *p != '\r' && *p != '\t') ++p;
  return p;
}

inline std::string compact(std::string_view s) {
  std::string o;
  o.reserve(s.size());
  const char* p = s.data();
  const char* e = p + s.size();
  bool in_str = false;
  const __m128i q = _mm_set1_epi8('"'), bs = _mm_set1_epi8('\\'), sp = _mm_set1_epi8(' '), nl = _mm_set1_epi8('\n'),
                cr = _mm_set1_epi8('\r'), tb = _mm_set1_epi8('\t');
  while (p < e) {
    if (e - p >= 16) {
      __m128i x = _mm_loadu_si128(reinterpret_cast<const __m128i*>(p));
      __m128i hit = _mm_or_si128(_mm_cmpeq_epi8(x, q), _mm_cmpeq_epi8(x, bs));
      if (!in_str)
        hit = _mm_or_si128(hit, _mm_or_si128(_mm_or_si128(_mm_cmpeq_epi8(x, sp), _mm_cmpeq_epi8(x, nl)),
                                             _mm_or_si128(_mm_cmpeq_epi8(x, cr), _mm_cmpeq_epi8(x, tb))));
      int m = _mm_movemask_epi8(hit);
      if (m == 0) {
        o.append(p, 16);
        p += 16;
        continue;
      }
      int k = __builtin_ctz((unsigned)m);
      o.append(p, (size_t)k);
      p += k;
    }
    char c = *p++;
    if (in_str) {
      o += c;
      if (c == '\\' && p < e) o += *p++;
      else if (c == '"') in_str = false;
    } else if (c == '"') {
      in_str = true;
      o += c;
    } else if (c != ' ' && c != '\n' && c != '\r' && c != '\t') {
      o += c;
    }
  }
  return o;
}

inline void escape_to(std::string& out, std::string_view s) {
  out += '"';
  const char* run = s.data();
  const char* e = s.data() + s.size();
  for (const char* p = run; p < e; ++p) {
    const unsigned char c = (unsigned char)*p;
    if (c >= 0x20 && c != '"' && c != '\\') continue;
    out.append(run, (size_t)(p - run));
    run = p + 1;
    switch (c) {
      case '"': out += "\\\""; break;
      case '\\': out += "\\\\"; break;
      case '\n': out += "\\n"; break;
      case '\r': out += "\\r"; break;
      case '\t': out += "\\t"; break;
      case '\b': out += "\\b"; break;
      case '\f': out += "\\f"; break;
      default:
        char buf[8];
        std::snprintf(buf, sizeof buf, "\\u%04x", c);
        out += buf;
    }
  }
  out.append(run, (size_t)(e - run));
  out += '"';
}

inline void number_to(std::string& out, double d) {
  if (std::isfinite(d) && d == std::floor(d) && std::fabs(d) < 9.007199254740992e15) {
    char buf[32];
    std::snprintf(buf, sizeof buf, "%lld", (long long)d);
    out += buf;
  } else if (!std::isfinite(d)) {
    out += "null";
  } else {
    char buf[32];
    std::snprintf(buf, sizeof buf, "%.17g", d);
    out += buf;
  }
}

inline void dump_to(std::string& out, const Value& v) {
  switch (v.t) {
    case Value::Null: out += "null"; break;
    case Value::Bool: out += v.b ? "true" : "false"; break;
    case Value::Number: number_to(out, v.n); break;
    case Value::String: escape_to(out, v.s); break;
    case Value::Array:
      out += '[';
      for (size_t i = 0; i < v.items.size(); ++i) { if (i) out += ','; dump_to(out, v.items[i]); }
      out += ']';
      break;
    case Value::Object:
      out += '{';
      for (size_t i = 0; i < v.items.size(); ++i) {
        if (i) out += ',';
        escape_to(out, v.keys[i]);
        out += ':';
        dump_to(out, v.items[i]);
      }
      out += '}';
      break;
  }
}

inline std::string dump(const Value& v) { std::string o; dump_to(o, v); return o; }

inline int compare(const Value& a, const Value& b) {
  if (a.t != b.t) return a.t < b.t ? -1 : 1;
  switch (a.t) {
    case Value::Null: return 0;
    case Value::Bool: return (int)a.b - (int)b.b;
    case Value::Number: return a.n < b.n ? -1 : (a.n > b.n ? 1 : 0);
    case Value::String: { int c = a.s.compare(b.s); return c < 0 ? -1 : (c > 0 ? 1 : 0); }
    case Value::Array: {
      size_t n = std::min(a.items.size(), b.items.size());
      for (size_t i = 0; i < n; ++i) { int c = compare(a.items[i], b.items[i]); if (c) return c; }
      return a.items.size() < b.items.size() ? -1 : (a.items.size() > b.items.size() ? 1 : 0);
    }
    case Value::Object: { std::string x = dump(a), y = dump(b); int c = x.compare(y); return c < 0 ? -1 : (c > 0 ? 1 : 0); }
  }
  return 0;
}

inline bool equals(const Value& a, const Value& b) { return compare(a, b) == 0; }

inline std::string index_key(const Value& v) {
  std::string k;
  k += (char)('0' + v.t);
  switch (v.t) {
    case Value::Bool: k += v.b ? '1' : '0'; break;
    case Value::Number: number_to(k, v.n); break;
    case Value::String: k += v.s; break;
    case Value::Null: break;
    default: dump_to(k, v); break;
  }
  return k;
}

}
```

aca_dotnet_workshop_amd/native/src/module.cpp:

```cpp
#include <unistd.h>

#include <pybind11/pybind11.h>
#include <pybind11/numpy.h>
#include <pybind11/stl.h>

#include "apphost.hpp"
#include "daprpb.hpp"
#include "backingfront.hpp"
#include "broker.hpp"
#include "cpuscan.hpp"
#include "docstore.hpp"
#include "dutycycle.hpp"
#include "httpparse.hpp"
#include "taskcodec.hpp"
#include "sweepcodec.hpp"
#include "pcsample.hpp"
#include "formcodec.hpp"
#include "strrank.hpp"

namespace py = pybind11;
using namespace tt;

template <class List>
static py::dict headers_dict(const List& headers) {
// ... 422 lines not shown
    const taskcodec::Update* up = nullptr;
    if (!update.is_none()) {
      auto t = update.cast<py::tuple>();
      u.name = t[0].cast<std::string>();
      u.assigned_to = t[1].cast<std::string>();
      u.due = t[2].cast<std::string>();
      up = &u;
    }
    std::string out, id, old;
    if (!taskcodec::edit_task(view(stored), up, complete, out, id, old)) return py::none();
    return py::make_tuple(py::bytes(out), py::str(id), py::str(old));
  });
  m.def("task_json", [view](py::bytes stored) -> py::object {
    std::string out;
    if (!taskcodec::task_json(view(stored), out)) return py::none();
    return py::bytes(out);
  });
  m.def("ascii_ieq", [](const std::string& a, const std::string& b) -> py::object {
    int r = taskcodec::ascii_ieq(a, b);
    if (r < 0) return py::none();
    return py::bool_(r == 1);
  });

  m.def("tasks_conditional_mark", [](py::bytes got) -> py::object {
    char* p;
    Py_ssize_t n;
    if (PyBytes_AsStringAndSize(got.ptr(), &p, &n) != 0) throw py::error_already_set();
    std::vector<std::string> ids;
    std::string bulk;
    size_t skipped = 0;
    if (!taskcodec::conditional_mark(std::string_view(p, (size_t)n), bulk, ids, skipped)) return py::none();
    py::list l(ids.size());
    for (size_t i = 0; i < ids.size(); ++i) l[i] = py::str(ids[i]);
    return py::make_tuple(l, py::bytes(bulk), skipped);
  });

  m.def("tasks_overdue_filter", [](py::bytes body, const std::string& run_day) -> py::object {
    char* p;
    Py_ssize_t n;
    if (PyBytes_AsStringAndSize(body.ptr(), &p, &n) != 0) throw py::error_already_set();
    size_t retrieved = 0, kept = 0;
    std::string out;
    if (!taskcodec::overdue_filter(std::string_view(p, (size_t)n), run_day, retrieved, kept, out)) return py::none();
    return py::make_tuple(retrieved, kept, py::bytes(out));
  });

  m.def("tasks_overdue_filter_chunks", [](py::bytes body, const std::string& run_day, size_t chunk) -> py::object {
    char* p;
    Py_ssize_t n;
    if (PyBytes_AsStringAndSize(body.ptr(), &p, &n) != 0) throw py::error_already_set();
    if (chunk == 0) return py::none();
    size_t retrieved = 0, kept = 0;
    std::string out;
    std::vector<size_t> starts;
    if (!taskcodec::overdue_filter(std::string_view(p, (size_t)n), run_day, retrieved, kept, out, &starts))
      return py::none();
    py::list parts;
    const size_t body_end = out.size() - 1;
    for (size_t a = 0; a < starts.size(); a += chunk) {
      const size_t b = std::min(starts.size(), a + chunk);
      const size_t from = starts[a], to = b < starts.size() ? starts[b] - 1 : body_end;
      std::string part;
      part.reserve(to - from + 2);
      part += '[';
      part.append(out, from, to - from);
      part += ']';
      parts.append(py::bytes(part));
    }
    return py::make_tuple(retrieved, kept, parts);
  });

  m.def("frontend_create_form", [](py::bytes body, py::bytes cookie, py::bytes key) -> py::object {
    char *pb, *pc, *pk;
    Py_ssize_t nb, nc, nk;
    if (PyBytes_AsStringAndSize(body.ptr(), &pb, &nb) != 0 || PyBytes_AsStringAndSize(cookie.ptr(), &pc, &nc) != 0 ||
        PyBytes_AsStringAndSize(key.ptr(), &pk, &nk) != 0)
      throw py::error_already_set();
    std::string json;
    auto v = formcodec::create_task(std::string_view(pb, (size_t)nb), std::string_view(pc, (size_t)nc),
                                    std::string_view(pk, (size_t)nk), ".AspNetCore.Antiforgery", "TasksCreatedByCookie",
                                    json);
    if (v == formcodec::Verdict::kDecline) return py::none();
    if (v == formcodec::Verdict::kBadToken) return py::make_tuple(false, py::bytes(""));
    return py::make_tuple(true, py::bytes(json));
  });

  m.def("frontend_edit_form", [view](py::bytes body, py::bytes cookie, py::bytes key, const std::string& path_id)
            -> py::object {
    std::string json, id;
    auto v = formcodec::edit_task(view(body), view(cookie), view(key), ".AspNetCore.Antiforgery", path_id, json, id);
    if (v == formcodec::Verdict::kDecline) return py::none();
    if (v == formcodec::Verdict::kBadToken) return py::make_tuple(false, py::bytes(""), py::str(""));
    return py::make_tuple(true, py::bytes(json), py::str(id));
  });
  m.def("frontend_index_form", [view](py::bytes body, py::bytes cookie, py::bytes key) -> py::object {
    auto v = formcodec::index_post(view(body), view(cookie), view(key), ".AspNetCore.Antiforgery");
    if (v == formcodec::Verdict::kDecline) return py::none();
    return py::bool_(v == formcodec::Verdict::kOk);
  });

  m.def("tasks_from_query", [](py::bytes body, bool by_created, bool descending) -> py::object {
    char* p;
    Py_ssize_t n;
    if (PyBytes_AsStringAndSize(body.ptr(), &p, &n) != 0) throw py::error_already_set();
    std::string out;
    size_t count = 0;
    bool more = false;
    if (!taskcodec::query_tasks(std::string_view(p, (size_t)n), out, count, by_created, &more, descending))
      return py::none();
    return py::make_tuple(count, py::bytes(out), more);
  }, py::arg("body"), py::arg("by_created") = false, py::arg("descending") = false);
  m.def("tasks_query_in_store_layout", [](py::bytes body) {
    std::string_view b = body.cast<std::string_view>();
    std::string buf;
    std::vector<taskcodec::TaskRow> rows;
    bool token = false;
    return taskcodec::valid_utf8(b) && taskcodec::fast_query_tasks(b, buf, rows, token);
  });

  m.def("json_array_chunks", [](py::bytes body, long n) -> py::object {
    char* pb;
    Py_ssize_t nb;
    if (PyBytes_AsStringAndSize(body.ptr(), &pb, &nb) != 0) throw py::error_already_set();
    std::string_view s(pb, (size_t)nb);
    if (n < 1 || !tt::valid(s)) return py::none();
    const char* p = tt::ws_end(s.data(), s.data() + s.size());
    const char* e = s.data() + s.size();
    if (p >= e || *p != '[') return py::none();
    ++p;
    py::list out;
    std::string cur = "[";
    long in_cur = 0;
    while (true) {
      p = tt::ws_end(p, e);
      if (p < e && *p == ']') break;
      const char* vs = p;
      p = tt::skip_value(p, e);
      if (in_cur) cur += ',';
      cur.append(vs, (size_t)(p - vs));
      if (++in_cur == n) {
        cur += ']';
        out.append(py::bytes(cur));
        cur = "[";
        in_cur = 0;
      }
      p = tt::ws_end(p, e);
      if (p < e && *p == ',') ++p;
    }
    if (in_cur) {
      cur += ']';
      out.append(py::bytes(cur));
    }
    return out;
  });

  m.def("task_model_name", [](py::bytes body) -> py::object {
    char* p;
    Py_ssize_t n;
    if (PyBytes_AsStringAndSize(body.ptr(), &p, &n) != 0) throw py::error_already_set();
    std::string name;
    if (!taskcodec::task_model_name(std::string_view(p, (size_t)n), name)) return py::none();
    return py::str(name);
  });

  m.def("scan_select",
        [](py::list columns, py::array_t<uint16_t, py::array::c_style> live, int64_t nrows,
           py::array_t<int32_t, py::array::c_style> code, py::array_t<uint32_t, py::array::c_style> bitmaps,
           int threads, bool simd) {
          std::vector<cpuscan::Col> cols;
          std::vector<py::array> keep;
          const int64_t padded = (nrows + 63) / 64 * 64;
          for (auto item : columns) {
            auto t = item.cast<py::tuple>();
            py::array a = t[0].cast<py::array>();
            int w = t[1].cast<int>();
            if (w != 0 && w != 1 && w != 2 && w != 4) throw py::value_error("column width must be 0 (2 bits), 1, 2 or 4");
            if (!(a.flags() & py::array::c_style)) throw py::value_error("columns must be contiguous");
            if ((int64_t)a.nbytes() < (w == 0 ? padded / 4 : padded * w))
              throw py::value_error("column shorter than the padded row count");
            cols.push_back({static_cast<const uint8_t*>(a.data()), w});
            keep.push_back(a);
          }
          if ((int64_t)live.size() * 16 < padded) throw py::value_error("liveness shorter than the padded row count");
          if (code.ndim() != 2 || code.shape(1) != 4) throw py::value_error("code must be [L, 4]");
          cpuscan::Program pg;
          pg.code.assign(code.data(), code.data() + code.size());
          pg.bitmaps.assign(bitmaps.data(), bitmaps.data() + bitmaps.size());
          cpuscan::Selection sel(cols, live.data(), nrows, pg, std::max(1, threads), simd);
          int64_t total;
          {
            py::gil_scoped_release rel;
            total = sel.count();
          }
          int32_t* dst = static_cast<int32_t*>(cpuscan::huge_alloc((size_t)std::max<int64_t>(total, 1) * sizeof(int32_t)));
          py::capsule owner(dst, [](void* p) { std::free(p); });
          {
            py::gil_scoped_release rel;
            sel.write(dst);
          }
          return py::array_t<int32_t>({(py::ssize_t)total}, {(py::ssize_t)sizeof(int32_t)}, dst, owner);
        },
        py::arg("columns"), py::arg("live"), py::arg("nrows"), py::arg("code"), py::arg("bitmaps"), py::arg("threads"),
        py::arg("simd") = true);

  py::class_<TxOp>(m, "TxOp")
      .def(py::init([](bool is_delete, std::string key, std::string value, std::optional<std::string> etag,
                       bool first_write, int64_t ttl_ms) {
             TxOp op;
             op.is_delete = is_delete;
             op.key = std::move(key);
             op.value = std::move(value);
             op.etag = std::move(etag);
             op.first_write = first_write;
             op.ttl_ms = ttl_ms;
             return op;
           }),
           py::arg("is_delete"), py::arg("key"), py::arg("value") = "", py::arg("etag") = std::nullopt,
           py::arg("first_write") = false, py::arg("ttl_ms") = 0)
      .def_readonly("is_delete", &TxOp::is_delete)
      .def_readonly("key", &TxOp::key)
      .def_readonly("value", &TxOp::value)
      .def_readonly("ttl_ms", &TxOp::ttl_ms);

  py::class_<StrRanker>(m, "StrRanker")
      .def(py::init<>())
      .def_property_readonly("size", &StrRanker::size)
      .def(
          "extend",
          [](StrRanker& r, py::list values, py::array_t<int64_t, py::array::c_style> ranks) -> int64_t {
            const size_t n0 = r.size(), n = (size_t)PyList_GET_SIZE(values.ptr());
            if (n < n0) return -1;
            if ((size_t)ranks.size() < n || !ranks.writeable()) throw std::invalid_argument("rank buffer too small");
            std::vector<std::string_view> vs;
            vs.reserve(n - n0);
            for (size_t i = n0; i < n; ++i) {
              PyObject* o = PyList_GET_ITEM(values.ptr(), (Py_ssize_t)i);
              if (!PyUnicode_Check(o)) return -1;
              Py_ssize_t len = 0;
              const char* p = PyUnicode_AsUTF8AndSize(o, &len);
              if (!p) {
                PyErr_Clear();
                return -1;
              }
              vs.emplace_back(p, (size_t)len);
            }
            int64_t* out = ranks.mutable_data();
            return (int64_t)r.extend(vs.size(), [&](size_t i) { return vs[i]; }, out);
          },
          py::arg("values"), py::arg("ranks"));

  py::class_<DocStore>(m, "DocStore")
      .def(py::init<const std::string&, int, size_t>(), py::arg("path") = "", py::arg("fsync_mode") = 0,
           py::arg("index_threshold") = 256)
      .def("set",
           [](DocStore& s, const std::string& key, const std::string& value, const std::optional<std::string>& etag,
              bool first_write, int64_t ttl_ms) {
             std::string e = s.set(key, value, etag, first_write, ttl_ms);
             s.wait_durable();
             return e;
           },
           py::arg("key"), py::arg("value"), py::arg("etag") = std::nullopt, py::arg("first_write") = false,
           py::arg("ttl_ms") = 0, py::call_guard<py::gil_scoped_release>())
      .def("get", &DocStore::get, py::arg("key"))
      .def("delete",
           [](DocStore& s, const std::string& key, const std::optional<std::string>& etag) {
             bool ok = s.del(key, etag);
             s.wait_durable();
             return ok;
           },
           py::arg("key"), py::arg("etag") = std::nullopt, py::call_guard<py::gil_scoped_release>())
      .def("transact",
           [](DocStore& s, const std::vector<TxOp>& ops) {
             s.transact(ops);
             s.wait_durable();
           },
           py::arg("ops"), py::call_guard<py::gil_scoped_release>())
      .def("group_commit", &DocStore::group_commit)
      .def("wait_durable", &DocStore::wait_durable, py::call_guard<py::gil_scoped_release>())
      .def("commit_stats",
           [](DocStore& s) {
             auto c = s.commit_stats();
             py::dict d;
             d["syncs"] = c.syncs;
             d["acks"] = c.acks;
             d["written_bytes"] = c.written;
             d["synced_bytes"] = c.synced;
             d["sync_ms_total"] = c.sync_ms_total;
             d["sync_ms_max"] = c.sync_ms_max;
             return d;
           })
      .def("query", &DocStore::query, py::arg("query"), py::arg("prefix") = "", py::arg("sort_keys") = false,
           py::call_guard<py::gil_scoped_release>())
      .def("keys", &DocStore::keys, py::arg("prefix") = "", py::arg("limit") = 0)
      .def("encode_columns",
           [](DocStore& s, const std::string& prefix, const std::vector<std::string>& paths) {
             DocStore::Encoded e;
             {
               py::gil_scoped_release r;
               e = s.encode_columns(prefix, paths);
             }
             py::list cols;
             for (auto& c : e.cols) {
               py::array_t<int32_t> ids((py::ssize_t)c.ids.size());
               std::memcpy(ids.mutable_data(), c.ids.data(), c.ids.size() * sizeof(int32_t));
               cols.append(py::make_tuple(py::cast(c.values), ids));
             }
// ... 306 lines not shown
```

aca_dotnet_workshop_amd/native/src/textutil.hpp:

```cpp
#pragma once

#include <cctype>
#include <cstdint>
#include <string>
#include <string_view>

#include "json.hpp"

namespace tt::text {

inline int hexv(char c) {
  if (c >= '0' && c <= '9') return c - '0';
  if (c >= 'a' && c <= 'f') return c - 'a' + 10;
  if (c >= 'A' && c <= 'F') return c - 'A' + 10;
  return -1;
}

inline std::string unquote(std::string_view s, bool plus_space = false) {
  std::string o;
  o.reserve(s.size());
  for (size_t i = 0; i < s.size(); ++i) {
    if (s[i] == '%' && i + 2 < s.size() && hexv(s[i + 1]) >= 0 && hexv(s[i + 2]) >= 0) {
      o += (char)(hexv(s[i + 1]) * 16 + hexv(s[i + 2]));
      i += 2;
    } else if (plus_space && s[i] == '+') {
      o += ' ';
    } else {
      o += s[i];
    }
  }
  return o;
}

inline std::string quote_all(std::string_view s) {
  static const char* d = "0123456789ABCDEF";
  std::string o;
  for (unsigned char c : s) {
    if (std::isalnum(c) || c == '_' || c == '.' || c == '-' || c == '~') {
      o += (char)c;
    } else {
      o += '%';
      o += d[c >> 4];
      o += d[c & 15];
    }
  }
  return o;
}

inline std::string lower(std::string_view s) {
  std::string o(s);
  for (auto& c : o) c = (char)std::tolower((unsigned char)c);
  return o;
}

inline std::string json_str(std::string_view s) {
  std::string o;
  escape_to(o, s);
  return o;
}

inline bool valid_utf8(std::string_view s) {
  for (size_t i = 0; i < s.size();) {
    unsigned char c = (unsigned char)s[i];
    size_t n = c < 0x80 ? 0 : (c >> 5) == 6 ? 1 : (c >> 4) == 14 ? 2 : (c >> 3) == 30 ? 3 : 99;
    if (n == 99 || i + n >= s.size() + (n == 0)) return n == 0;
    for (size_t k = 1; k <= n; ++k)
      if (((unsigned char)s[i + k] >> 6) != 2) return false;
    i += n + 1;
  }
  return true;
}

inline std::string base64(std::string_view in) {
  static const char* t = "ABCDEFGHIJKLMNOPQRSTUVWXYZabcdefghijklmnopqrstuvwxyz0123456789+/";
  std::string o;
  size_t i = 0;
  for (; i + 2 < in.size(); i += 3) {
    uint32_t v = ((uint8_t)in[i] << 16) | ((uint8_t)in[i + 1] << 8) | (uint8_t)in[i + 2];
    o += t[v >> 18];
    o += t[(v >> 12) & 63];
    o += t[(v >> 6) & 63];
    o += t[v & 63];
  }
  if (i + 1 == in.size()) {
    uint32_t v = (uint8_t)in[i] << 16;
    o += t[v >> 18];
    o += t[(v >> 12) & 63];
    o += "==";
  } else if (i + 2 == in.size()) {
    uint32_t v = ((uint8_t)in[i] << 16) | ((uint8_t)in[i + 1] << 8);
    o += t[v >> 18];
    o += t[(v >> 12) & 63];
    o += t[(v >> 6) & 63];
    o += '=';
  }
  return o;
}

inline std::string unbase64(std::string_view in) {
  std::string o;
  uint32_t acc = 0;
  int bits = 0;
  for (char c : in) {
    int v = c >= 'A' && c <= 'Z' ? c - 'A' : c >= 'a' && c <= 'z' ? c - 'a' + 26 : c >= '0' && c <= '9' ? c - '0' + 52
            : c == '+' ? 62 : c == '/' ? 63 : -1;
    if (v < 0) continue;
    acc = (acc << 6) | (uint32_t)v;
    bits += 6;
    if (bits >= 8) {
      bits -= 8;
      o += (char)((acc >> bits) & 0xFF);
    }
  }
  return o;
}

}
```

Measured before the change: 96850.

## Cut allocations in dataplane hot paths and add native gRPC save/publish handling

```diff
diff --git a/aca_dotnet_workshop_amd/native/build.py b/aca_dotnet_workshop_amd/native/build.py
--- a/aca_dotnet_workshop_amd/native/build.py
+++ b/aca_dotnet_workshop_amd/native/build.py
@@ -85,8 +85,8 @@
 
 
 def build_dataplane(force: bool = False, verbose: bool = False) -> Path:
-    sources = [SRC / "dataplane.cpp", SRC / "evhttp.hpp", SRC / "h2.hpp", SRC / "pb.hpp", SRC / "tls.hpp", SRC / "json.hpp", SRC / "httpparse.hpp",
-               SRC / "textutil.hpp", SRC / "pcsample.hpp"]
+    sources = [SRC / "dataplane.cpp", SRC / "apireq.hpp", SRC / "evhttp.hpp", SRC / "h2.hpp", SRC / "pb.hpp", SRC / "tls.hpp",
+               SRC / "json.hpp", SRC / "httpparse.hpp", SRC / "textutil.hpp", SRC / "pcsample.hpp", SRC / "daprpb.hpp"]
     return _build_exe(DATAPLANE, SRC / "dataplane.cpp", sources, force, verbose)
 
 
diff --git a/aca_dotnet_workshop_amd/native/src/apireq.hpp b/aca_dotnet_workshop_amd/native/src/apireq.hpp
--- /dev/null
+++ b/aca_dotnet_workshop_amd/native/src/apireq.hpp
@@ -0,0 +1,145 @@
+#pragma once
+
+#include <cstdlib>
+#include <string>
+#include <string_view>
+#include <utility>
+#include <vector>
+
+#include "json.hpp"
+#include "pb.hpp"
+#include "textutil.hpp"
+
+namespace tt::apireq {
+
+struct SaveItem {
+  std::string_view key, value, etag;
+  bool raw_value = false;
+  bool first_write = false;
+  long long ttl_ms = 0;
+};
+
+struct SaveReq {
+  std::string_view store;
+  std::vector<SaveItem> items;
+};
+
+using MetaList = std::vector<std::pair<std::string_view, std::string_view>>;
+
+struct PublishReq {
+  std::string_view pubsub, topic, data, ctype;
+  MetaList meta;
+};
+
+inline void json_or_text_to(std::string& out, std::string_view raw) {
+  if (raw.empty()) out += "null";
+  else if (compact_to(out, raw)) return;
+  else if (text::valid_utf8(raw)) escape_to(out, raw);
+  else escape_to(out, text::base64(raw));
+}
+
+inline long long ttl_ms_of(std::string_view seconds) {
+  char buf[64];
+  std::string big;
+  const char* c;
+  if (seconds.size() < sizeof buf) {
+    if (!seconds.empty()) std::memcpy(buf, seconds.data(), seconds.size());
+    buf[seconds.size()] = 0;
+    c = buf;
+  } else {
+    big.assign(seconds);
+    c = big.c_str();
+  }
+  return (long long)(std::atof(c) * 1000);
+}
+
+inline bool map_entry_view(std::string_view entry, std::string_view& k, std::string_view& v) {
+  pb::Reader r(entry);
+  uint32_t f, wt;
+  k = {};
+  v = {};
+  while (r.next(f, wt)) {
+    std::string_view s;
+    if ((f == 1 || f == 2) && wt == pb::LEN) {
+      if (!r.bytes(s)) break;
+      (f == 1 ? k : v) = s;
+    } else if (!r.skip(wt)) {
+      break;
+    }
+  }
+  return r.ok;
+}
+
+inline bool decode_state_item(std::string_view s, SaveItem& it) {
+  pb::Reader r(s);
+  uint32_t f, wt;
+  std::string_view v;
+  bool have_ttl = false;
+  it.raw_value = true;
+  while (r.next(f, wt)) {
+    if (f == 1 && wt == pb::LEN && r.bytes(v)) it.key = v;
+    else if (f == 2 && wt == pb::LEN && r.bytes(v)) it.value = v;
+    else if (f == 3 && wt == pb::LEN && r.bytes(v)) {
+      pb::Reader er(v);
+      uint32_t ef, ewt;
+      std::string_view ev;
+      while (er.next(ef, ewt))
+        if (ef == 1 && ewt == pb::LEN && er.bytes(ev)) it.etag = ev;
+        else if (!er.skip(ewt)) break;
+      if (!er.ok) return false;
+    } else if (f == 4 && wt == pb::LEN && r.bytes(v)) {
+      std::string_view k, val;
+      if (!map_entry_view(v, k, val)) return false;
+      if (k == "ttlInSeconds" && !have_ttl) {
+        have_ttl = true;
+        it.ttl_ms = ttl_ms_of(val);
+      }
+    } else if (f == 5 && wt == pb::LEN && r.bytes(v)) {
+      pb::Reader orr(v);
+      uint32_t of, owt;
+      uint64_t x;
+      while (orr.next(of, owt))
+        if ((of == 1 || of == 2) && owt == pb::VARINT && orr.varint(x)) {
+          if (of == 1) it.first_write = x == 1;
+        } else if (!orr.skip(owt)) break;
+      if (!orr.ok) return false;
+    } else if (!r.skip(wt)) {
+      break;
+    }
+  }
+  return r.ok;
+}
+
+inline bool decode_save(std::string_view msg, SaveReq& out) {
+  pb::Reader rd(msg);
+  uint32_t f, wt;
+  std::string_view v;
+  while (rd.next(f, wt)) {
+    if (f == 1 && wt == pb::LEN && rd.bytes(v)) out.store = v;
+    else if (f == 2 && wt == pb::LEN && rd.bytes(v)) {
+      out.items.emplace_back();
+      if (!decode_state_item(v, out.items.back())) return false;
+    } else if (!rd.skip(wt)) break;
+  }
+  return rd.ok;
+}
+
+inline bool decode_publish(std::string_view msg, PublishReq& out) {
+  pb::Reader rd(msg);
+  uint32_t f, wt;
+  std::string_view v;
+  while (rd.next(f, wt)) {
+    if (f == 1 && wt == pb::LEN && rd.bytes(v)) out.pubsub = v;
+    else if (f == 2 && wt == pb::LEN && rd.bytes(v)) out.topic = v;
+    else if (f == 3 && wt == pb::LEN && rd.bytes(v)) out.data = v;
+    else if (f == 4 && wt == pb::LEN && rd.bytes(v)) out.ctype = v;
+    else if (f == 5 && wt == pb::LEN && rd.bytes(v)) {
+      std::string_view k, val;
+      if (!map_entry_view(v, k, val)) return false;
+      out.meta.emplace_back(k, val);
+    } else if (!rd.skip(wt)) break;
+  }
+  return rd.ok;
+}
+
+}
diff --git a/aca_dotnet_workshop_amd/native/src/dataplane.cpp b/aca_dotnet_workshop_amd/native/src/dataplane.cpp
--- a/aca_dotnet_workshop_amd/native/src/dataplane.cpp
+++ b/aca_dotnet_workshop_amd/native/src/dataplane.cpp
@@ -11,6 +11,7 @@
 #include <random>
 #include <sstream>
 
+#include "apireq.hpp"
 #include "evhttp.hpp"
 #include "daprpb.hpp"
 #include "h2.hpp"
@@ -34,30 +35,49 @@
   return r;
 }
 
-std::string hex_u64(uint64_t v, int digits = 16) {
+struct Uuid {
+  char s[36];
+  std::string_view view() const { return {s, 36}; }
+};
+Uuid uuid4() {
   static const char* d = "0123456789abcdef";
-  std::string s((size_t)digits, '0');
-  for (int i = digits - 1; i >= 0; --i, v >>= 4) s[(size_t)i] = d[v & 15];
-  return s;
-}
-
-std::string uuid4() {
   uint64_t a = rng()(), b = rng()();
   a = (a & 0xFFFFFFFFFFFF0FFFull) | 0x0000000000004000ull;
   b = (b & 0x3FFFFFFFFFFFFFFFull) | 0x8000000000000000ull;
-  std::string h = hex_u64(a) + hex_u64(b);
-  return h.substr(0, 8) + "-" + h.substr(8, 4) + "-" + h.substr(12, 4) + "-" + h.substr(16, 4) + "-" + h.substr(20);
+  Uuid u;
+  char* o = u.s;
+  for (int i = 0; i < 32; ++i) {
+    if (i == 8 || i == 12 || i == 16 || i == 20) *o++ = '-';
+    const uint64_t w = i < 16 ? a : b;
+    *o++ = d[(w >> (60 - 4 * (i & 15))) & 15];
+  }
+  return u;
 }
 
-std::string utc_now_iso() {
+struct IsoTime {
+  char s[27];
+  std::string_view view() const { return {s, 27}; }
+};
+IsoTime utc_now_iso() {
+  static thread_local time_t cached_sec = -1;
+  static thread_local char cached[20];
   timespec ts;
   clock_gettime(CLOCK_REALTIME, &ts);
-  tm t;
-  gmtime_r(&ts.tv_sec, &t);
-  char buf[64];
-  std::snprintf(buf, sizeof buf, "%04d-%02d-%02dT%02d:%02d:%02d.%06ldZ", t.tm_year + 1900, t.tm_mon + 1, t.tm_mday,
-                t.tm_hour, t.tm_min, t.tm_sec, ts.tv_nsec / 1000);
-  return buf;
+  if (ts.tv_sec != cached_sec) {
+    tm t;
+    gmtime_r(&ts.tv_sec, &t);
+    char buf[64];
+    std::snprintf(buf, sizeof buf, "%04d-%02d-%02dT%02d:%02d:%02d.", t.tm_year + 1900, t.tm_mon + 1, t.tm_mday,
+                  t.tm_hour, t.tm_min, t.tm_sec);
+    std::memcpy(cached, buf, 20);
+    cached_sec = ts.tv_sec;
+  }
+  IsoTime o;
+  std::memcpy(o.s, cached, 20);
+  long us = ts.tv_nsec / 1000;
+  for (int i = 25; i >= 20; --i, us /= 10) o.s[i] = (char)('0' + us % 10);
+  o.s[26] = 'Z';
+  return o;
 }
 
 double wall_now() {
@@ -147,10 +167,16 @@
   std::string_view sid() const { return {span_id, 16}; }
   std::string_view pid() const { return {parent_id, 16}; }
   std::string traceparent() const {
-    std::string s;
-    s.reserve(55);
-    s.append("00-", 3).append(trace_id, 32).append(1, '-').append(span_id, 16).append(sampled ? "-01" : "-00", 3);
-    return s;
+    char b[55];
+    traceparent_to(b);
+    return std::string(b, 55);
+  }
+  void traceparent_to(char (&b)[55]) const {
+    std::memcpy(b, "00-", 3);
+    std::memcpy(b + 3, trace_id, 32);
+    b[35] = '-';
+    std::memcpy(b + 36, span_id, 16);
+    std::memcpy(b + 52, sampled ? "-01" : "-00", 3);
   }
 };
 
@@ -301,30 +327,68 @@
   std::map<std::string, Entry> cache_;
 };
 
-inline uint64_t fnv1a64(std::string_view s) {
-  uint64_t h = 14695981039346656037ull;
+inline uint64_t fnv1a64(std::string_view s, uint64_t h = 14695981039346656037ull) {
   for (unsigned char c : s) {
     h ^= c;
     h *= 1099511628211ull;
   }
   return h;
 }
+inline std::string header_lines(const HeaderList& headers) {
+  std::string o;
+  for (auto& h : headers) {
+    if (ev::is_hop_header(h.first)) continue;
+    o += h.first + ": " + h.second + "\r\n";
+  }
+  return o;
+}
+inline std::vector<std::string> head_tails(const Endpoint& backing, const std::vector<Endpoint>& shards,
+                                           const std::string& lines) {
+  std::vector<std::string> out;
+  auto one = [&](const Endpoint& ep) { out.push_back(" HTTP/1.1\r\nhost: " + ev::Client::host_of(ep) + "\r\n" + lines); };
+  if (shards.empty()) one(backing);
+  for (auto& ep : shards) one(ep);
+  return out;
+}
+
 struct Store {
   Endpoint backing;
   std::vector<Endpoint> shards;
+  std::string name;
   std::string coll_path;
   std::string prefix;
   HeaderList auth;
+  std::string put_line, bulkset_line;
+  std::vector<std::string> save_tail;
+  std::string grpc_save_name;
   size_t shard_of(std::string_view full_key) const { return shards.empty() ? 0 : fnv1a64(full_key) % shards.size(); }
   const Endpoint& ep(size_t shard) const { return shards.empty() ? backing : shards[shard]; }
+  void prerender() {
+    put_line = "PUT " + coll_path + "/docs/";
+    bulkset_line = "POST " + coll_path + "/bulkset";
+    HeaderList h = auth;
+    h.emplace_back("content-type", "application/json");
+    save_tail = head_tails(backing, shards, header_lines(h));
+    grpc_save_name = "POST " + ("/v1.0/state/" + quote_all(name)).substr(0, 80);
+  }
 };
 struct Bus {
   Endpoint backing;
   std::vector<Endpoint> shards;
+  std::string name;
   std::string ns;
   HeaderList auth;
-  const Endpoint& ep(std::string_view partition_key) const {
-    return shards.empty() ? backing : shards[fnv1a64(partition_key) % shards.size()];
+  std::string post_line;
+  std::vector<std::string> auth_tail;
+  std::string grpc_publish_prefix;
+  size_t shard_of(std::string_view partition_key) const {
+    return shards.empty() ? 0 : fnv1a64(partition_key) % shards.size();
+  }
+  const Endpoint& ep(size_t shard) const { return shards.empty() ? backing : shards[shard]; }
+  void prerender() {
+    post_line = "POST /servicebus/" + quote_all(ns) + "/topics/";
+    auth_tail = head_tails(backing, shards, header_lines(auth));
+    grpc_publish_prefix = "/v1.0/publish/" + quote_all(name) + "/";
   }
 };
 inline std::vector<Endpoint> shard_list(const Value& s) {
@@ -344,6 +408,7 @@
  public:
   DataPlane(ev::Loop& loop, const Value& cfg) : loop_(loop), client_(loop) {
     app_id_ = *opt_str(cfg, "appId");
+    ce_head_ = "\",\"source\":" + json_str(app_id_) + ",\"type\":\"com.dapr.event.sent\",\"datacontenttype\":";
     if (auto* a = opt_str(cfg, "app")) {
       app_ = Endpoint::parse(*a);
       has_app_ = true;
@@ -375,6 +440,8 @@
         x.prefix = *opt_str(s, "prefix");
         x.auth = auth_headers(s);
         x.shards = shard_list(s);
+        x.name = st->keys[i];
+        x.prerender();
         stores_[st->keys[i]] = std::move(x);
       }
     if (auto* ps = cfg.get("pubsubs"); ps && ps->t == Value::Object)
@@ -385,6 +452,8 @@
         b.ns = *opt_str(s, "ns");
         b.auth = auth_headers(s);
         b.shards = shard_list(s);
+        b.name = ps->keys[i];
+        b.prerender();
         buses_[ps->keys[i]] = std::move(b);
       }
   }
@@ -432,10 +501,10 @@
   Endpoint app_, fallback_;
   bool has_app_ = false, invoke_native_ = true, api_logging_ = false;
   double app_timeout_ = 300;
-  std::map<std::string, Store> stores_;
-  std::map<std::string, Bus> buses_;
-  std::map<std::string, uint64_t> counters_;
-  std::map<std::pair<std::string, int>, uint64_t> op_counts_;
+  std::map<std::string, Store, std::less<>> stores_;
+  std::map<std::string, Bus, std::less<>> buses_;
+  std::map<std::string, uint64_t, std::less<>> grpc_calls_;
+  std::map<std::pair<std::string_view, int>, uint64_t> op_counts_;
   size_t inflight_ = 0;
 
   static HeaderList auth_headers(const Value& s) {
@@ -481,18 +550,21 @@
   }
   std::string api_log_buf_;
 
-  void count(const std::string& op, int status) {
-    op_counts_[{op, status}]++;
-  }
+  void count(const char* op, int status) { op_counts_[{std::string_view(op), status}]++; }
 
   struct Done {
     DataPlane* dp;
     Reply rep;
     SpanCtx span;
-    std::string name, op;
+    std::string name;
+    const char* op = "";
     std::vector<std::pair<std::string, std::string>> attrs;
+    const char* grpc_rpc = nullptr;
+    h2::GrpcReply grpc_rep;
     void send(int status, const HeaderList& h, std::string_view body) {
-      rep.send(status, h, body);
+      if (!grpc_rpc) rep.send(status, h, body);
+      else if (status >= 300) grpc_fail(grpc_rep, status, body, grpc_rpc);
+      else grpc_rep.ok({});
       if (dp->api_logging_) dp->api_log(name, status, span);
       dp->tracer_.end(span, name, status, attrs);
       dp->count(op, status);
@@ -501,14 +573,32 @@
     void json(int status, std::string_view body) { send(status, {{"content-type", "application/json"}}, body); }
     void error(int status, std::string_view code, std::string_view msg) { json(status, error_json(code, msg)); }
   };
-  std::shared_ptr<Done> begin(const Message& m, Reply&& r, std::string op, std::string_view path) {
+  std::shared_ptr<Done> begin(const Message& m, Reply&& r, const char* op, std::string_view path) {
     inflight_++;
     auto d = std::make_shared<Done>();
     d->dp = this;
     d->rep = std::move(r);
     d->span = tracer_.start(m.header("traceparent"));
     d->name = m.method + " " + std::string(path.substr(0, 80));
-    d->op = std::move(op);
+    d->op = op;
+    return d;
+  }
+  std::shared_ptr<Done> begin_grpc(const h2::GrpcCall& c, h2::GrpcReply&& r, const char* rpc, const char* op,
+                                   std::string_view name) {
+    inflight_++;
+    auto d = std::make_shared<Done>();
+    d->dp = this;
+    d->grpc_rpc = rpc;
+    d->grpc_rep = std::move(r);
+    const std::string* tp = nullptr;
+    for (auto& kv : c.metadata)
+      if (kv.first == "traceparent") {
+        tp = &kv.second;
+        break;
+      }
+    d->span = tracer_.start(tp);
+    d->name.assign(name);
+    d->op = op;
     return d;
   }
 
@@ -648,10 +738,10 @@
       }
       if (!is_ce && !s_.raw) {
         std::string base = lower(ctype.substr(0, ctype.find(';')));
-        std::string ce = "{\"specversion\":\"1.0\",\"id\":" + json_str(m.id.empty() ? uuid4() : m.id) +
+        std::string ce = "{\"specversion\":\"1.0\",\"id\":" + json_str(m.id.empty() ? std::string(uuid4().view()) : m.id) +
                          ",\"source\":\"unknown\",\"type\":\"com.dapr.event.sent\",\"datacontenttype\":" +
                          json_str(base.empty() ? "application/json" : base) + ",\"topic\":" + json_str(s_.topic) +
-                         ",\"pubsubname\":" + json_str(s_.pubsub) + ",\"time\":\"" + utc_now_iso() + "\"";
+                         ",\"pubsubname\":" + json_str(s_.pubsub) + ",\"time\":\"" + std::string(utc_now_iso().view()) + "\"";
         if (base.find("json") != std::string::npos && !body.empty() && valid_json(body)) ce += ",\"data\":" + compact(body);
         else if (base.find("json") != std::string::npos && body.empty()) ce += ",\"data\":null";
         else if (base.rfind("text/", 0) == 0 || base.find("json") != std::string::npos || body.empty())
@@ -875,7 +965,7 @@
         auto it = stores_.find(store);
         if (it != stores_.end()) {
           if (seg.size() == 3 && (m.method == "POST" || m.method == "PUT")) {
-            state_save(std::move(m), std::move(r), store, it->second, path);
+            state_save(std::move(m), std::move(r), it->second, path);
             return;
           }
           if (seg.size() == 4 && m.method == "GET") {
@@ -925,10 +1015,11 @@
   void metrics(Message&& m, Reply r) {
     std::string extra = "# HELP sidecar_native_requests_total requests served by the native data plane\n"
                         "# TYPE sidecar_native_requests_total counter\n";
-    std::map<std::string, uint64_t> all = counters_;
+    std::map<std::string, uint64_t> all;
+    for (auto& kv : grpc_calls_) all["app=\"" + app_id_ + "\",op=\"grpc." + kv.first + "\",status=\"call\""] += kv.second;
     for (auto& kv : op_counts_)
-      all["app=\"" + app_id_ + "\",op=\"" + kv.first.first + "\",status=\"" + std::to_string(kv.first.second) + "\""] +=
-          kv.second;
+      all["app=\"" + app_id_ + "\",op=\"" + std::string(kv.first.first) + "\",status=\"" +
+          std::to_string(kv.first.second) + "\""] += kv.second;
     for (auto& kv : all) extra += "sidecar_native_requests_total{" + kv.first + "} " + std::to_string(kv.second) + "\n";
     extra += "# HELP sidecar_mtls_handshake_rejected_total mesh TLS handshakes this sidecar refused\n"
              "# TYPE sidecar_mtls_handshake_rejected_total counter\n"
@@ -1083,88 +1174,127 @@
     return false;
   }
 
-  struct Item {
-    std::string key, value, etag;
-    bool first_write = false;
-    long long ttl_ms = 0;
+  struct SavePart {
+    size_t shard = 0, first = 0, count = 0;
+    int attempt = 0;
+    double waited = 0.0;
+    std::string ticket;
   };
-
-  static bool parse_items(const std::string& body, std::vector<Item>& items, std::string& err) {
-    if (!valid_json(body)) {
-      err = "request body is not valid JSON";
-      return false;
-    }
-    const char* p = ws_end(body.data(), body.data() + body.size());
+  struct SaveCall {
+    std::shared_ptr<Done> d;
+    const Store* s = nullptr;
+    std::string src;
+    std::deque<std::string> owned;
+    apireq::SaveReq req;
+    std::vector<SavePart> parts;
+    size_t left = 0;
+    ClientResult worst;
+    bool have = false;
+  };
+
+  static bool parse_items(SaveCall& c, std::string& err) {
+    const char* why = scan_items(c);
+    if (!why) return true;
+    err = valid_json(c.src) ? why : "request body is not valid JSON";
+    return false;
+  }
+  static const char* scan_items(SaveCall& c) {
+    static const char* const kBad = "request body is not valid JSON";
+    const std::string& body = c.src;
     const char* e = body.data() + body.size();
-    if (p >= e || *p != '[') {
-      err = "request body must be an array of state items";
-      return false;
-    }
-    ++p;
+    const char* p = ws_end(body.data(), e);
+    if (p >= e || *p != '[') return "request body must be an array of state items";
+    p = ws_end(p + 1, e);
+    bool first_item = true;
     while (true) {
-      p = ws_end(p, e);
-      if (p < e && *p == ']') break;
-      if (p >= e || *p != '{') {
-        err = "state item without key";
-        return false;
-      }
-      Item it;
+      if (p >= e) return kBad;
+      if (first_item && *p == ']') break;
+      if (*p != '{') return "state item without key";
+      apireq::SaveItem it;
       bool have_value = false;
-      ++p;
+      p = ws_end(p + 1, e);
+      bool first_member = true;
       while (true) {
-        p = ws_end(p, e);
-        if (*p == '}') {
+        if (p >= e) return kBad;
+        if (first_member && *p == '}') {
           ++p;
           break;
         }
+        if (*p != '"') return kBad;
         const char* ks = p;
-        p = skip_value(p, e);
+        p = Validator(std::string_view(ks, (size_t)(e - ks))).prefix(2);
+        if (!p) return kBad;
         std::string_view ktok(ks, (size_t)(p - ks));
-        std::string k = ktok.size() >= 2 && ktok.find('\\') == std::string_view::npos
-                            ? std::string(ktok.substr(1, ktok.size() - 2))
-                            : parse(ktok).s;
-        p = ws_end(p, e) + 1;
+        std::string kbuf;
+        std::string_view k = ktok.substr(1, ktok.size() - 2);
+        if (ktok.find('\\') != std::string_view::npos) k = kbuf = parse(ktok).s;
         p = ws_end(p, e);
+        if (p >= e || *p != ':') return kBad;
+        p = ws_end(p + 1, e);
         const char* vs = p;
-        p = skip_value(p, e);
-        std::string_view raw(vs, (size_t)(p - vs));
-        if (k == "key") {
-          if (raw.size() >= 2 && raw.front() == '"' && raw.find('\\') == std::string_view::npos) {
-            it.key.assign(raw.data() + 1, raw.size() - 2);
-          } else {
+        if (k == "value") {
+          c.owned.emplace_back();
+          p = Compactor(c.owned.back(), std::string_view(vs, (size_t)(e - vs))).prefix(2);
+          if (!p) return kBad;
+          it.value = c.owned.back();
+          have_value = true;
+        } else {
+          p = Validator(std::string_view(vs, (size_t)(e - vs))).prefix(2);
+          if (!p) return kBad;
+          std::string_view raw(vs, (size_t)(p - vs));
+          auto keep = [&c](std::string& s) -> std::string_view {
+            c.owned.push_back(std::move(s));
+            return c.owned.back();
+          };
+          if (k == "key") {
+            if (raw.size() >= 2 && raw.front() == '"' && raw.find('\\') == std::string_view::npos) {
+              it.key = raw.substr(1, raw.size() - 2);
+            } else {
+              Value v = parse(raw);
+              if (v.t == Value::String) it.key = keep(v.s);
+            }
+          } else if (k == "etag") {
             Value v = parse(raw);
-            if (v.t == Value::String) it.key = v.s;
-          }
-        } else if (k == "value") {
-          it.value = compact(raw);
-          have_value = true;
-        } else if (k == "etag") {
-          Value v = parse(raw);
-          if (v.t == Value::String) it.etag = v.s;
-          else if (auto* x = v.get("value"); x && x->t == Value::String) it.etag = x->s;
-        } else if (k == "options") {
-          Value v = parse(raw);
-          if (auto* c = v.get("concurrency"); c && c->t == Value::String) it.first_write = c->s == "first-write";
-        } else if (k == "metadata") {
-          Value v = parse(raw);
-          if (auto* t = v.get("ttlInSeconds")) {
-            double s = t->t == Value::Number ? t->n : t->t == Value::String ? std::atof(t->s.c_str()) : 0.0;
-            it.ttl_ms = (long long)(s * 1000);
+            if (v.t == Value::String) it.etag = keep(v.s);
+            else if (auto* x = v.get("value"); x && x->t == Value::String) it.etag = keep(const_cast<Value*>(x)->s);
+          } else if (k == "options") {
+            Value v = parse(raw);
+            if (auto* o = v.get("concurrency"); o && o->t == Value::String) it.first_write = o->s == "first-write";
+          } else if (k == "metadata") {
+            Value v = parse(raw);
+            if (auto* t = v.get("ttlInSeconds")) {
+              double s = t->t == Value::Number ? t->n : t->t == Value::String ? std::atof(t->s.c_str()) : 0.0;
+              it.ttl_ms = (long long)(s * 1000);
+            }
           }
         }
+        first_member = false;
         p = ws_end(p, e);
-        if (*p == ',') ++p;
-      }
-      if (it.key.empty()) {
-        err = "state item without key";
-        return false;
-      }
+        if (p >= e) return kBad;
+        if (*p == ',') {
+          p = ws_end(p + 1, e);
+          if (p < e && *p == '}') return kBad;
+          continue;
+        }
+        if (*p != '}') return kBad;
+        ++p;
+        break;
+      }
+      if (it.key.empty()) return "state item without key";
       if (!have_value) it.value = "null";
-      items.push_back(std::move(it));
+      c.req.items.push_back(it);
+      first_item = false;
       p = ws_end(p, e);
-      if (*p == ',') ++p;
-    }
-    return true;
+      if (p >= e) return kBad;
+      if (*p == ',') {
+        p = ws_end(p + 1, e);
+        if (p < e && *p == ']') return kBad;
+        continue;
+      }
+      if (*p != ']') return kBad;
+      break;
+    }
+    return ws_end(p + 1, e) == e ? nullptr : kBad;
   }
 
   struct StoreCall {
@@ -1190,24 +1320,29 @@
     store_send(std::move(c));
   }
 
+  bool throttled_retry(const ClientResult& res, int& attempt, double& waited, double& delay) {
+    if (res.err || res.resp.status != 429 || attempt >= 9) return false;
+    const std::string* ra = res.resp.header("x-ms-retry-after-ms");
+    delay = ra ? std::strtod(ra->c_str(), nullptr) / 1000.0 : 0.1;
+    delay = std::min(std::max(delay, 0.001), 5.0);
+    if (waited + delay > 30.0) return false;
+    count("state.throttled_retry", 429);
+    attempt++;
+    waited += delay;
+    return true;
+  }
+
   void store_send(std::shared_ptr<StoreCall> c) {
     StoreCall& k = *c;
     auto on_done = [this, c](ClientResult&& res) {
-      if (!res.err && res.resp.status == 429 && c->attempt < 9) {
-        const std::string* ra = res.resp.header("x-ms-retry-after-ms");
-        double delay = ra ? std::strtod(ra->c_str(), nullptr) / 1000.0 : 0.1;
-        delay = std::min(std::max(delay, 0.001), 5.0);
-        if (c->waited + delay <= 30.0) {
-          count("state.throttled_retry", 429);
-          c->attempt++;
-          c->waited += delay;
-          auto& hs = c->headers;
-          hs.erase(std::remove_if(hs.begin(), hs.end(), [](const auto& h) { return h.first == "x-tt-ru-ticket"; }),
-                   hs.end());
-          if (const std::string* t = res.resp.header("x-tt-ru-ticket")) hs.emplace_back("x-tt-ru-ticket", *t);
-          loop_.call_later(delay, [this, c] { store_send(c); });
-          return;
-        }
+      double delay;
+      if (throttled_retry(res, c->attempt, c->waited, delay)) {
+        auto& hs = c->headers;
+        hs.erase(std::remove_if(hs.begin(), hs.end(), [](const auto& h) { return h.first == "x-tt-ru-ticket"; }),
+                 hs.end());
+        if (const std::string* t = res.resp.header("x-tt-ru-ticket")) hs.emplace_back("x-tt-ru-ticket", *t);
+        loop_.call_later(delay, [this, c] { store_send(c); });
+        return;
       }
       c->cb(std::move(res));
     };
@@ -1215,86 +1350,156 @@
     else client_.request(k.ep, k.method, k.target, k.headers, k.body, 60, std::move(on_done));
   }
 
-  void state_save(Message&& m, Reply&& r, const std::string& name, const Store& s, const std::string& path) {
-    auto d = begin(m, std::move(r), "state.save", path);
-    std::vector<Item> items;
+  void state_save(Message&& m, Reply&& r, const Store& s, const std::string& path) {
+    auto c = std::make_shared<SaveCall>();
+    c->d = begin(m, std::move(r), "state.save", path);
+    c->s = &s;
+    c->src = std::move(m.body);
     std::string err;
-    if (!parse_items(m.body, items, err)) {
-      d->error(400, "ERR_MALFORMED_REQUEST", err);
+    if (!parse_items(*c, err)) {
+      c->d->error(400, "ERR_MALFORMED_REQUEST", err);
       return;
     }
-    auto done = [d, name](ClientResult&& res) {
-      if (!res.err && (res.resp.status == 409 || res.resp.status == 412)) {
-        d->error(409, "ERR_STATE_SAVE", "failed saving state in state store " + name + ": state save: HTTP " +
-                                            std::to_string(res.resp.status) + " " + res.resp.body.substr(0, 200));
+    save_core(c);
+  }
+
+  static size_t body_begin(std::string& w) {
+    w += "content-length:           \r\n\r\n";
+    return w.size();
+  }
+  static void body_done(std::string& w, size_t body_at) {
+    size_t n = w.size() - body_at;
+    char* q = &w[body_at - 5];
+    do {
+      *q-- = (char)('0' + n % 10);
+      n /= 10;
+    } while (n);
+  }
+
+  void save_core(const std::shared_ptr<SaveCall>& c) {
+    Done& d = *c->d;
+    const Store& s = *c->s;
+    auto& items = c->req.items;
+    for (auto& it : items)
+      if (it.key.empty()) {
+        d.error(400, "ERR_MALFORMED_REQUEST", "state item without key");
         return;
       }
-      if (res.err || res.resp.status >= 300) {
-        d->error(500, "ERR_STATE_SAVE", "failed saving state in state store " + name + ": " +
-                                            (res.err ? errno_text(res.err) : "HTTP " + std::to_string(res.resp.status)));
-        return;
-      }
-      d->send(204, {}, {});
+    if (items.empty()) {
+      d.send(204, {}, {});
+      return;
+    }
+    auto shard_of = [&s](std::string_view key) {
+      return s.shards.empty() ? (size_t)0 : (size_t)(fnv1a64(key, fnv1a64(s.prefix)) % s.shards.size());
     };
-    if (items.empty()) {
-      d->send(204, {}, {});
+    if (items.size() == 1 || s.shards.empty()) {
+      c->parts.emplace_back();
+      c->parts[0].shard = shard_of(items[0].key);
+      c->parts[0].count = items.size();
+    } else {
+      std::vector<std::pair<size_t, apireq::SaveItem>> by;
+      for (auto& it : items) by.emplace_back(shard_of(it.key), it);
+      std::stable_sort(by.begin(), by.end(), [](const auto& a, const auto& b) { return a.first < b.first; });
+      for (size_t i = 0; i < by.size(); ++i) {
+        items[i] = by[i].second;
+        if (i == 0 || by[i].first != by[i - 1].first) {
+          c->parts.emplace_back();
+          c->parts.back().shard = by[i].first;
+          c->parts.back().first = i;
+        }
+        c->parts.back().count++;
+      }
+    }
+    c->left = c->parts.size();
+    for (size_t i = 0; i < c->parts.size(); ++i) save_send(c, i);
+  }
+
+  void save_send(const std::shared_ptr<SaveCall>& c, size_t pi) {
+    const SavePart& p = c->parts[pi];
+    const Store& s = *c->s;
+    const apireq::SaveItem* it = &c->req.items[p.first];
+    const bool bulk = p.count > 1;
+    std::string w;
+    size_t body_at;
+    if (!bulk) {
+      w.reserve(s.put_line.size() + 3 * (s.prefix.size() + it->key.size()) + s.save_tail[p.shard].size() +
+                it->etag.size() + p.ticket.size() + it->value.size() + 160);
+      w += s.put_line;
+      quote_all_to(w, s.prefix);
+      quote_all_to(w, it->key);
+      w += s.save_tail[p.shard];
+      if (!it->etag.empty()) w.append("if-match: ").append(it->etag).append("\r\n");
+      if (it->first_write) w += "x-tt-first-write: 1\r\n";
+      if (it->ttl_ms) w.append("x-tt-ttl-ms: ").append(std::to_string(it->ttl_ms)).append("\r\n");
+      if (!p.ticket.empty()) w.append("x-tt-ru-ticket: ").append(p.ticket).append("\r\n");
+      body_at = body_begin(w);
+      if (it->raw_value) apireq::json_or_text_to(w, it->value);
+      else w += it->value;
+    } else {
+      w += s.bulkset_line;
+      w += s.save_tail[p.shard];
+      if (!p.ticket.empty()) w.append("x-tt-ru-ticket: ").append(p.ticket).append("\r\n");
+      body_at = body_begin(w);
+      w += '[';
+      std::string val;
+      for (size_t i = 0; i < p.count; ++i, ++it) {
+        if (i) w += ',';
+        val.clear();
+        if (it->raw_value) apireq::json_or_text_to(val, it->value);
+        else val = it->value;
+        const bool as_text = val.empty() || val[0] == '"';
+        w += "{\"key\":";
+        escape_to(w, s.prefix + std::string(it->key));
+        w += ",\"value\":";
+        if (as_text) escape_to(w, val);
+        else w += val;
+        w += ",\"etag\":";
+        if (it->etag.empty()) w += "null";
+        else escape_to(w, it->etag);
+        w += it->first_write ? ",\"firstWrite\":true,\"ttlMs\":" : ",\"firstWrite\":false,\"ttlMs\":";
+        w += std::to_string(it->ttl_ms);
+        w += '}';
+      }
+      w += ']';
+    }
+    body_done(w, body_at);
+    client_.send_wire(s.ep(p.shard), std::move(w), 60, [this, c, pi](ClientResult&& res) { save_answer(c, pi, std::move(res)); },
+                      !bulk);
+  }
+
+  void save_answer(const std::shared_ptr<SaveCall>& c, size_t pi, ClientResult&& res) {
+    SavePart& p = c->parts[pi];
+    double delay;
+    if (throttled_retry(res, p.attempt, p.waited, delay)) {
+      const std::string* t = res.resp.header("x-tt-ru-ticket");
+      p.ticket = t ? *t : std::string();
+      loop_.call_later(delay, [this, c, pi] { save_send(c, pi); });
       return;
     }
-    HeaderList h = s.auth;
-    h.emplace_back("content-type", "application/json");
-    if (s.shards.empty()) {
-      save_on(s, 0, h, items, std::move(done));
+    if (c->parts.size() > 1) {
+      auto rank = [](const ClientResult& r) {
+        return r.err ? 3 : (r.resp.status == 409 || r.resp.status == 412) ? 2 : r.resp.status >= 300 ? 1 : 0;
+      };
+      if (!c->have || rank(res) > rank(c->worst)) {
+        c->worst = std::move(res);
+        c->have = true;
+      }
+      if (--c->left) return;
+      res = std::move(c->worst);
+    }
+    Done& d = *c->d;
+    const std::string& name = c->s->name;
+    if (!res.err && (res.resp.status == 409 || res.resp.status == 412)) {
+      d.error(409, "ERR_STATE_SAVE", "failed saving state in state store " + name + ": state save: HTTP " +
+                                         std::to_string(res.resp.status) + " " + res.resp.body.substr(0, 200));
       return;
     }
-    std::map<size_t, std::vector<Item>> by_shard;
-    for (auto& it : items) by_shard[s.shard_of(full_key(s, it.key))].push_back(std::move(it));
-    if (by_shard.size() == 1) {
-      save_on(s, by_shard.begin()->first, h, by_shard.begin()->second, std::move(done));
+    if (res.err || res.resp.status >= 300) {
+      d.error(500, "ERR_STATE_SAVE", "failed saving state in state store " + name + ": " +
+                                         (res.err ? errno_text(res.err) : "HTTP " + std::to_string(res.resp.status)));
       return;
     }
-    struct Join {
-      size_t left;
-      ClientResult worst;
-      bool have = false;
-      ev::ClientCallback done;
-    };
-    auto j = std::make_shared<Join>();
-    j->left = by_shard.size();
-    j->done = std::move(done);
-    for (auto& kv : by_shard)
-      save_on(s, kv.first, h, kv.second, [j](ClientResult&& res) {
-        auto rank = [](const ClientResult& r) {
-          return r.err ? 3 : (r.resp.status == 409 || r.resp.status == 412) ? 2 : r.resp.status >= 300 ? 1 : 0;
-        };
-        if (!j->have || rank(res) > rank(j->worst)) {
-          j->worst = std::move(res);
-          j->have = true;
-        }
-        if (--j->left == 0) j->done(std::move(j->worst));
-      });
-  }
-
-  void save_on(const Store& s, size_t shard, HeaderList h, std::vector<Item>& items, ev::ClientCallback done) {
-    if (items.size() == 1) {
-      Item& it = items[0];
-      if (!it.etag.empty()) h.emplace_back("if-match", it.etag);
-      if (it.first_write) h.emplace_back("x-tt-first-write", "1");
-      if (it.ttl_ms) h.emplace_back("x-tt-ttl-ms", std::to_string(it.ttl_ms));
-      store_request(s.ep(shard), "PUT", s.coll_path + "/docs/" + quote_all(full_key(s, it.key)), std::move(h), it.value,
-                    std::move(done));
-      return;
-    }
-    std::string body = "[";
-    for (size_t i = 0; i < items.size(); ++i) {
-      auto& it = items[i];
-      if (i) body += ',';
-      const bool as_text = it.value.empty() || it.value[0] == '"';
-      body += "{\"key\":" + json_str(full_key(s, it.key)) + ",\"value\":" + (as_text ? json_str(it.value) : it.value) +
-              ",\"etag\":" + (it.etag.empty() ? std::string("null") : json_str(it.etag)) +
-              ",\"firstWrite\":" + (it.first_write ? "true" : "false") + ",\"ttlMs\":" + std::to_string(it.ttl_ms) + "}";
-    }
-    body += "]";
-    store_request(s.ep(shard), "POST", s.coll_path + "/bulkset", std::move(h), std::move(body), std::move(done), false);
+    d.send(204, {}, {});
   }
 
   static std::string full_key(const Store& s, const std::string& key) {
@@ -1731,81 +1936,141 @@
 
   bool publish(Message& m, Reply& r, const std::string& name, const std::string& topic, const Bus& b,
                const std::string& qs, const std::string& path) {
-    std::map<std::string, std::string> meta;
+    apireq::PublishReq q;
+    std::deque<std::string> owned;
     for (size_t i = 0; i <= qs.size() && !qs.empty();) {
       size_t j = qs.find('&', i);
       if (j == std::string::npos) j = qs.size();
       std::string_view kv(qs.data() + i, j - i);
       size_t eq = kv.find('=');
       std::string k = unquote(kv.substr(0, eq), true);
-      std::string v = eq == std::string_view::npos ? "" : unquote(kv.substr(eq + 1), true);
-      if (k.rfind("metadata.", 0) == 0) meta[k.substr(9)] = v;
+      if (k.rfind("metadata.", 0) == 0) {
+        owned.push_back(k.substr(9));
+        owned.push_back(eq == std::string_view::npos ? "" : unquote(kv.substr(eq + 1), true));
+        q.meta.emplace_back(owned[owned.size() - 2], owned.back());
+      }
       i = j + 1;
     }
-    const std::string* ct = m.header("content-type");
-    std::string ctype = ct && !ct->empty() ? *ct : "application/json";
-    std::string base = lower(ctype.substr(0, ctype.find(';')));
-    while (!base.empty() && base.back() == ' ') base.pop_back();
-    while (!base.empty() && base.front() == ' ') base.erase(0, 1);
-    bool raw = lower(meta.count("rawPayload") ? meta["rawPayload"] : "") == "true";
+    q.pubsub = name;
+    q.topic = topic;
+    q.data = m.body;
+    if (const std::string* ct = m.header("content-type")) q.ctype = *ct;
+    return publish_core(q, b, [&] { return begin(m, std::move(r), "publish", path); });
+  }
+
+  static bool ascii_ieq(std::string_view a, std::string_view b) {
+    if (a.size() != b.size()) return false;
+    for (size_t i = 0; i < a.size(); ++i)
+      if (std::tolower((unsigned char)a[i]) != std::tolower((unsigned char)b[i])) return false;
+    return true;
+  }
+
+  template <class Begin>
+  bool publish_core(const apireq::PublishReq& q, const Bus& b, Begin&& begin_call) {
+    apireq::MetaList meta = q.meta;
+    if (meta.size() > 1) {
+      std::stable_sort(meta.begin(), meta.end(), [](const auto& x, const auto& y) { return x.first < y.first; });
+      size_t n = 0;
+      for (size_t i = 0; i < meta.size(); ++i)
+        if (i + 1 == meta.size() || meta[i + 1].first != meta[i].first) meta[n++] = meta[i];
+      meta.resize(n);
+    }
+    auto meta_of = [&meta](std::string_view k) -> const std::string_view* {
+      for (auto& kv : meta)
+        if (kv.first == k) return &kv.second;
+      return nullptr;
+    };
+    const std::string_view ctype = q.ctype.empty() ? std::string_view("application/json") : q.ctype;
+    std::string base_buf;
+    std::string_view base = ctype;
+    if (ctype != "application/json") {
+      base_buf = lower(ctype.substr(0, ctype.find(';')));
+      while (!base_buf.empty() && base_buf.back() == ' ') base_buf.pop_back();
+      while (!base_buf.empty() && base_buf.front() == ' ') base_buf.erase(0, 1);
+      base = base_buf;
+    }
+    const std::string_view* rp = meta_of("rawPayload");
+    const bool raw = rp && ascii_ieq(*rp, "true");
     if (!raw && base == "application/cloudevents+json") return false;
-    bool is_json = base.find("json") != std::string::npos;
-    bool json_body = is_json && !m.body.empty() && valid_json(m.body);
-    bool as_string = !json_body && (is_json || base.rfind("text/", 0) == 0 || m.body.empty());
-    if (!raw && as_string && !valid_utf8(m.body)) return false;
-    auto d = begin(m, std::move(r), "publish", path);
-    d->attrs.emplace_back("topic", topic);
-    std::string body, out_ct, event_id;
-    if (raw) {
-      body = std::move(m.body);
-      out_ct = ctype;
-    } else {
-      std::string tp = d->span.traceparent();
-      event_id = uuid4();
-      body = "{\"specversion\":\"1.0\",\"id\":\"" + event_id + "\",\"source\":" + json_str(app_id_) +
-             ",\"type\":\"com.dapr.event.sent\",\"datacontenttype\":" + json_str(base.empty() ? "application/json" : base) +
-             ",\"topic\":" + json_str(topic) + ",\"pubsubname\":" + json_str(name) + ",\"time\":\"" + utc_now_iso() + "\"";
-      if (is_json) {
-        if (m.body.empty()) body += ",\"data\":null";
-        else if (json_body) body += ",\"data\":" + compact(m.body);
-        else body += ",\"data\":" + json_str(m.body);
-      } else if (base.rfind("text/", 0) == 0 || m.body.empty()) {
-        body += ",\"data\":" + json_str(m.body);
-      } else {
-        body += ",\"data_base64\":\"" + base64(m.body) + "\"";
-      }
-      body += ",\"traceparent\":\"" + tp + "\",\"traceid\":\"" + tp + "\"}";
-      out_ct = "application/cloudevents+json";
-    }
-    HeaderList h = b.auth;
-    h.emplace_back("content-type", out_ct);
-    std::string props;
+    const bool is_json = base.find("json") != std::string_view::npos;
+    const bool is_text = base.rfind("text/", 0) == 0;
+
+    const Uuid event_id = uuid4();
+    const std::string_view* pk = meta_of("partitionKey");
+    const size_t shard = b.shard_of(pk && !pk->empty() ? *pk : event_id.view());
+
+    std::string w;
+    w.reserve(b.post_line.size() + 3 * q.topic.size() + b.auth_tail[shard].size() + q.data.size() + q.data.size() / 2 +
+              2 * q.topic.size() + b.name.size() + ce_head_.size() + 512);
+    w += b.post_line;
+    quote_all_to(w, q.topic);
+    w += "/messages";
+    w += b.auth_tail[shard];
+    w += "content-type: ";
+    w += raw ? ctype : std::string_view("application/cloudevents+json");
+    w += "\r\n";
+    bool props = false;
     for (auto& kv : meta) {
       if (kv.first == "ttlInSeconds" || kv.first == "rawPayload") continue;
-      props += (props.empty() ? "{" : ",") + json_str(kv.first) + ":" + json_str(kv.second);
-    }
-    if (!props.empty()) h.emplace_back("x-tt-props", props + "}");
-    if (meta.count("ttlInSeconds")) {
-      long long ttl = (long long)(std::atof(meta["ttlInSeconds"].c_str()) * 1000);
-      if (ttl) h.emplace_back("x-tt-ttl-ms", std::to_string(ttl));
-    }
-    const std::string pkey = meta.count("partitionKey") && !meta["partitionKey"].empty() ? meta["partitionKey"]
-                             : event_id.empty()                                          ? uuid4()
-                                                                                         : event_id;
-    client_.request_pipelined(b.ep(pkey), "POST", "/servicebus/" + quote_all(b.ns) + "/topics/" + quote_all(topic) + "/messages", h,
-                    body, 60, [d, name, topic](ClientResult&& res) {
-                      if (res.err || res.resp.status >= 300) {
-                        d->error(500, "ERR_PUBSUB_PUBLISH_MESSAGE",
-                                 "error when publish to topic " + topic + " in pubsub " + name + ": " +
-                                     (res.err ? errno_text(res.err)
-                                              : "publish: HTTP " + std::to_string(res.resp.status) + " " +
-                                                    res.resp.body.substr(0, 200)));
-                        return;
-                      }
-                      d->send(204, {}, {});
-                    });
+      w += props ? "," : "x-tt-props: {";
+      props = true;
+      escape_to(w, kv.first);
+      w += ':';
+      escape_to(w, kv.second);
+    }
+    if (props) w += "}\r\n";
+    if (const std::string_view* t = meta_of("ttlInSeconds"))
+      if (long long ttl = apireq::ttl_ms_of(*t)) w.append("x-tt-ttl-ms: ").append(std::to_string(ttl)).append("\r\n");
+    const size_t body_at = body_begin(w);
+    if (raw) {
+      w += q.data;
+    } else {
+      w += "{\"specversion\":\"1.0\",\"id\":\"";
+      w += event_id.view();
+      w += ce_head_;
+      escape_to(w, base.empty() ? std::string_view("application/json") : base);
+      w += ",\"topic\":";
+      escape_to(w, q.topic);
+      w += ",\"pubsubname\":";
+      escape_to(w, b.name);
+      w += ",\"time\":\"";
+      w += utc_now_iso().view();
+      w += '"';
+      if (is_json && q.data.empty()) {
+        w += ",\"data\":null";
+      } else if (is_json || is_text || q.data.empty()) {
+        w += ",\"data\":";
+        if (!(is_json && compact_to(w, q.data))) {
+          if (!valid_utf8(q.data)) return false;
+          escape_to(w, q.data);
+        }
+      } else {
+        w += ",\"data_base64\":\"";
+        w += base64(q.data);
+        w += '"';
+      }
+    }
+    std::shared_ptr<Done> d = begin_call();
+    d->attrs.emplace_back("topic", std::string(q.topic));
+    if (!raw) {
+      char tp[55];
+      d->span.traceparent_to(tp);
+      w.append(",\"traceparent\":\"").append(tp, 55).append("\",\"traceid\":\"").append(tp, 55).append("\"}");
+    }
+    body_done(w, body_at);
+    client_.send_wire(b.ep(shard), std::move(w), 60, [d, bus = &b](ClientResult&& res) {
+      if (res.err || res.resp.status >= 300) {
+        d->error(500, "ERR_PUBSUB_PUBLISH_MESSAGE",
+                 "error when publish to topic " + d->attrs[0].second + " in pubsub " + bus->name + ": " +
+                     (res.err ? errno_text(res.err)
+                              : "publish: HTTP " + std::to_string(res.resp.status) + " " + res.resp.body.substr(0, 200)));
+        return;
+      }
+      d->send(204, {}, {});
+    }, true);
     return true;
   }
+  std::string ce_head_;
 
  public:
   h2::GrpcHandler grpc_handler() {
@@ -1846,10 +2111,9 @@
     r.error(grpc_code(status), what + ": " + msg, {{"dapr-http-status", std::to_string(status)}});
   }
   static std::string json_or_text(std::string_view raw) {
-    if (raw.empty()) return "null";
-    if (valid_json(raw)) return compact(raw);
-    if (valid_utf8(raw)) return json_str(raw);
-    return json_str(base64(raw));
+    std::string o;
+    apireq::json_or_text_to(o, raw);
+    return o;
   }
   static std::string meta_qs(const std::vector<std::pair<std::string, std::string>>& meta) {
     std::string qs;
@@ -1944,14 +2208,75 @@
     return o + "}";
   }
 
+  bool grpc_token_ok(const h2::GrpcCall& c, const h2::GrpcReply& r, const char* rpc) {
+    if (api_token_.empty()) return true;
+    for (auto& kv : c.metadata)
+      if (kv.first == "dapr-api-token") {
+        if (kv.second == api_token_) return true;
+        break;
+      }
+    grpc_fail(r, 401, error_json("ERR_API_TOKEN", "invalid api token"), rpc);
+    return false;
+  }
+
+  bool grpc_save(h2::GrpcCall& c, h2::GrpcReply& r) {
+    auto call = std::make_shared<SaveCall>();
+    call->src = std::move(c.message);
+    call->req.items.reserve(1);
+    if (!apireq::decode_save(call->src, call->req)) {
+      r.error(3, "SaveState: malformed request message");
+      return true;
+    }
+    if (!grpc_token_ok(c, r, "SaveState")) return true;
+    auto it = stores_.find(call->req.store);
+    if (it == stores_.end()) {
+      c.message = std::move(call->src);
+      return false;
+    }
+    call->s = &it->second;
+    call->d = begin_grpc(c, std::move(r), "SaveState", "state.save", it->second.grpc_save_name);
+    save_core(call);
+    return true;
+  }
+
+  bool grpc_publish(h2::GrpcCall& c, h2::GrpcReply& r) {
+    apireq::PublishReq q;
+    if (!apireq::decode_publish(c.message, q)) {
+      r.error(3, "PublishEvent: malformed request message");
+      return true;
+    }
+    if (!grpc_token_ok(c, r, "PublishEvent")) return true;
+    auto it = buses_.find(q.pubsub);
+    if (it == buses_.end() || q.topic.empty()) return false;
+    const Bus& b = it->second;
+    return publish_core(q, b, [&] {
+      std::string name = b.grpc_publish_prefix;
+      size_t i = 0;
+      while (true) {
+        size_t j = q.topic.find('/', i);
+        quote_all_to(name, q.topic.substr(i, j == std::string_view::npos ? std::string_view::npos : j - i));
+        if (j == std::string_view::npos) break;
+        name += '/';
+        i = j + 1;
+      }
+      name.resize(std::min<size_t>(name.size(), 80));
+      name.insert(0, "POST ");
+      return begin_grpc(c, std::move(r), "PublishEvent", "publish", name);
+    });
+  }
+
   void on_grpc(h2::GrpcCall&& c, h2::GrpcReply r) {
     static constexpr std::string_view kSvc = "/dapr.proto.runtime.v1.Dapr/";
     if (c.path.compare(0, kSvc.size(), kSvc) != 0) {
       r.error(12, "unknown service: " + c.path);
       return;
     }
-    std::string rpc = c.path.substr(kSvc.size());
-    counters_["app=\"" + app_id_ + "\",op=\"grpc." + rpc + "\",status=\"call\""]++;
+    const std::string_view rpc_name = std::string_view(c.path).substr(kSvc.size());
+    if (auto it = grpc_calls_.find(rpc_name); it != grpc_calls_.end()) ++it->second;
+    else grpc_calls_.emplace(std::string(rpc_name), 1);
+    if (rpc_name == "SaveState" && grpc_save(c, r)) return;
+    if (rpc_name == "PublishEvent" && grpc_publish(c, r)) return;
+    std::string rpc(rpc_name);
     pb::Reader rd(c.message);
     uint32_t f, wt;
     std::string_view v;
diff --git a/aca_dotnet_workshop_amd/native/src/evhttp.hpp b/aca_dotnet_workshop_amd/native/src/evhttp.hpp
--- a/aca_dotnet_workshop_amd/native/src/evhttp.hpp
+++ b/aca_dotnet_workshop_amd/native/src/evhttp.hpp
@@ -1026,7 +1026,7 @@
     w += ' ';
     w.append(target);
     w += " HTTP/1.1\r\nhost: ";
-    w += ep.unix_socket ? "localhost" : ep.host + ":" + std::to_string(ep.port);
+    w += host_of(ep);
     w += "\r\n";
     for (auto& h : headers) {
       if (is_hop_header(h.first)) continue;
@@ -1042,13 +1042,28 @@
     dispatch(ep, std::move(w), method == "HEAD", timeout_s, std::move(cb), retry_stale);
   }
 
+  static std::string host_of(const Endpoint& ep) {
+    return ep.unix_socket ? "localhost" : ep.host + ":" + std::to_string(ep.port);
+  }
+
+  void send_wire(const Endpoint& ep, std::string&& wire, double timeout_s, ClientCallback cb, bool pipelined) {
+    if (!pipelined || !pipelinable(ep)) {
+      dispatch(ep, std::move(wire), false, timeout_s, std::move(cb), !pipelined);
+      return;
+    }
+    double deadline = timeout_s > 0 ? now_s() + timeout_s : 0;
+    auto c = pipe_for(ep);
+    if (!c) {
+      dispatch(ep, std::move(wire), false, timeout_s, std::move(cb), false);
+      return;
+    }
+    c->send(std::move(wire), deadline, std::move(cb));
+    ++pipelined_;
+  }
+
   void request_pipelined(const Endpoint& ep, std::string_view method, std::string_view target,
                          const HeaderList& headers, std::string_view body, double timeout_s, ClientCallback cb) {
-    static const bool enabled = [] {
-      const char* v = std::getenv("TT_PIPELINE");
-      return !(v && v[0] == '0');
-    }();
-    if (!enabled || !ep.unix_socket || ep.tls || method == "HEAD") {
+    if (!pipelinable(ep) || method == "HEAD") {
       request(ep, method, target, headers, body, timeout_s, std::move(cb), false);
       return;
     }
@@ -1069,14 +1084,14 @@
     w += std::to_string(body.size());
     w += "\r\n\r\n";
     w.append(body);
-    double deadline = timeout_s > 0 ? now_s() + timeout_s : 0;
-    auto c = pipe_for(ep);
-    if (!c) {
-      dispatch(ep, std::move(w), false, timeout_s, std::move(cb), false);
-      return;
-    }
-    c->send(std::move(w), deadline, std::move(cb));
-    ++pipelined_;
+    send_wire(ep, std::move(w), timeout_s, std::move(cb), true);
+  }
+  static bool pipelinable(const Endpoint& ep) {
+    static const bool enabled = [] {
+      const char* v = std::getenv("TT_PIPELINE");
+      return !(v && v[0] == '0');
+    }();
+    return enabled && ep.unix_socket && !ep.tls;
   }
   void pipe_flushed(const std::string& key) {
     auto it = pipes_.find(key);
diff --git a/aca_dotnet_workshop_amd/native/src/json.hpp b/aca_dotnet_workshop_amd/native/src/json.hpp
--- a/aca_dotnet_workshop_amd/native/src/json.hpp
+++ b/aca_dotnet_workshop_amd/native/src/json.hpp
@@ -263,6 +263,7 @@
     ws();
     return p_ == e_;
   }
+  const char* prefix(int depth) { return value(depth) ? p_ : nullptr; }
 
  private:
   const char* p_;
@@ -470,6 +471,164 @@
     }
   }
   return o;
+}
+
+class Compactor {
+ public:
+  Compactor(std::string& out, std::string_view s) : out_(out), p_(s.data()), e_(s.data() + s.size()), run_(s.data()) {}
+  bool ok() {
+    if (!value(0)) return false;
+    ws();
+    if (p_ != e_) return false;
+    flush();
+    return true;
+  }
+  const char* prefix(int depth) {
+    if (!value(depth)) return nullptr;
+    flush();
+    return p_;
+  }
+
+ private:
+  std::string& out_;
+  const char* p_;
+  const char* e_;
+  const char* run_;
+  void flush() { out_.append(run_, (size_t)(p_ - run_)); }
+  void ws() {
+    if (p_ < e_ && (*p_ == ' ' || *p_ == '\n' || *p_ == '\r' || *p_ == '\t')) {
+      flush();
+      do ++p_;
+      while (p_ < e_ && (*p_ == ' ' || *p_ == '\n' || *p_ == '\r' || *p_ == '\t'));
+      run_ = p_;
+    }
+  }
+  bool value(int depth) {
+    if (depth > 256) return false;
+    ws();
+    if (p_ >= e_) return false;
+    switch (*p_) {
+      case '{': return object(depth);
+      case '[': return array(depth);
+      case '"': return str();
+      case 't': return lit("true", 4);
+      case 'f': return lit("false", 5);
+      case 'n': return lit("null", 4);
+      default: return num();
+    }
+  }
+  bool lit(const char* w, size_t n) {
+    if ((size_t)(e_ - p_) < n || std::memcmp(p_, w, n) != 0) return false;
+    p_ += n;
+    return true;
+  }
+  bool num() {
+    const char* s = p_;
+    if (p_ < e_ && (*p_ == '-' || *p_ == '+')) ++p_;
+    const char* d0 = p_;
+    while (p_ < e_ && *p_ >= '0' && *p_ <= '9') ++p_;
+    const char* d1 = p_;
+    while (p_ < e_ && ((*p_ >= '0' && *p_ <= '9') || *p_ == '.' || *p_ == 'e' || *p_ == 'E' || *p_ == '-' || *p_ == '+')) ++p_;
+    if (p_ == s) return false;
+    if (p_ == d1 && d1 > d0) return true;
+    char buf[64];
+    std::string big;
+    const size_t n = (size_t)(p_ - s);
+    const char* c;
+    if (n < sizeof buf) {
+      std::memcpy(buf, s, n);
+      buf[n] = 0;
+      c = buf;
+    } else {
+      big.assign(s, n);
+      c = big.c_str();
+    }
+    char* end = nullptr;
+    std::strtod(c, &end);
+    return end == c + n;
+  }
+  static bool is_hex(char c) { return (c >= '0' && c <= '9') || (c >= 'a' && c <= 'f') || (c >= 'A' && c <= 'F'); }
+  bool str() {
+    ++p_;
+    const __m128i q = _mm_set1_epi8('"'), bs = _mm_set1_epi8('\\');
+    while (true) {
+      while (e_ - p_ >= 16) {
+        __m128i x = _mm_loadu_si128(reinterpret_cast<const __m128i*>(p_));
+        int m = _mm_movemask_epi8(_mm_or_si128(_mm_cmpeq_epi8(x, q), _mm_cmpeq_epi8(x, bs)));
+        if (m) {
+          p_ += __builtin_ctz((unsigned)m);
+          break;
+        }
+        p_ += 16;
+      }
+      while (p_ < e_ && *p_ != '"' && *p_ != '\\') ++p_;
+      if (p_ >= e_) return false;
+      if (*p_ == '"') {
+        ++p_;
+        return true;
+      }
+      ++p_;
+      if (p_ >= e_) return false;
+      char x = *p_++;
+      switch (x) {
+        case '"': case '\\': case '/': case 'b': case 'f': case 'n': case 'r': case 't': break;
+        case 'u': {
+          if (e_ - p_ < 4) return false;
+          uint32_t cp = 0;
+          for (int i = 0; i < 4; ++i) {
+            char c = *p_++;
+            if (!is_hex(c)) return false;
+            cp = (cp << 4) | (uint32_t)(c <= '9' ? c - '0' : (c | 0x20) - 'a' + 10);
+          }
+          if (cp >= 0xD800 && cp < 0xDC00 && e_ - p_ >= 6 && p_[0] == '\\' && p_[1] == 'u') {
+            p_ += 2;
+            for (int i = 0; i < 4; ++i)
+              if (!is_hex(*p_++)) return false;
+          }
+          break;
+        }
+        default: return false;
+      }
+    }
+  }
+  bool array(int depth) {
+    ++p_;
+    ws();
+    if (p_ < e_ && *p_ == ']') { ++p_; return true; }
+    while (true) {
+      if (!value(depth + 1)) return false;
+      ws();
+      if (p_ >= e_) return false;
+      if (*p_ == ',') { ++p_; continue; }
+      if (*p_ == ']') { ++p_; return true; }
+      return false;
+    }
+  }
+  bool object(int depth) {
+    ++p_;
+    ws();
+    if (p_ < e_ && *p_ == '}') { ++p_; return true; }
+    while (true) {
+      ws();
+      if (p_ >= e_ || *p_ != '"' || !str()) return false;
+      ws();
+      if (p_ >= e_ || *p_ != ':') return false;
+      ++p_;
+      if (!value(depth + 1)) return false;
+      ws();
+      if (p_ >= e_) return false;
+      if (*p_ == ',') { ++p_; continue; }
+      if (*p_ == '}') { ++p_; return true; }
+      return false;
+    }
+  }
+};
+
+inline bool compact_to(std::string& out, std::string_view in) {
+  const size_t mark = out.size();
+  if (Compactor(out, in).ok()) return true;
+  out.resize(mark);
+  return false;
 }
 
 inline void escape_to(std::string& out, std::string_view s) {
diff --git a/aca_dotnet_workshop_amd/native/src/module.cpp b/aca_dotnet_workshop_amd/native/src/module.cpp
--- a/aca_dotnet_workshop_amd/native/src/module.cpp
+++ b/aca_dotnet_workshop_amd/native/src/module.cpp
@@ -598,6 +598,18 @@
       out.append(py::bytes(cur));
     }
     return out;
+  });
+
+  m.def("json_valid", [view](py::bytes text) { return tt::valid(view(text)); });
+  m.def("json_compact", [view](py::bytes text) { return py::bytes(tt::compact(view(text))); });
+  m.def("json_compact_to", [view](py::bytes text, py::bytes prefix) -> py::object {
+    std::string_view pre = view(prefix);
+    std::string out(pre);
+    if (!tt::compact_to(out, view(text))) {
+      if (out != pre) throw std::runtime_error("compact_to failed and left out changed");
+      return py::none();
+    }
+    return py::bytes(out);
   });
 
   m.def("task_model_name", [](py::bytes body) -> py::object {
diff --git a/aca_dotnet_workshop_amd/native/src/textutil.hpp b/aca_dotnet_workshop_amd/native/src/textutil.hpp
--- a/aca_dotnet_workshop_amd/native/src/textutil.hpp
+++ b/aca_dotnet_workshop_amd/native/src/textutil.hpp
@@ -32,9 +32,8 @@
   return o;
 }
 
-inline std::string quote_all(std::string_view s) {
+inline void quote_all_to(std::string& o, std::string_view s) {
   static const char* d = "0123456789ABCDEF";
-  std::string o;
   for (unsigned char c : s) {
     if (std::isalnum(c) || c == '_' || c == '.' || c == '-' || c == '~') {
       o += (char)c;
@@ -44,6 +43,11 @@
       o += d[c & 15];
     }
   }
+}
+
+inline std::string quote_all(std::string_view s) {
+  std::string o;
+  quote_all_to(o, s);
   return o;
 }
 
```

After: 96690. No clear change (-0.2%).
